# quadram-institute-bioscience/uvaia

Measured on AMD Instinct MI355X. Metric: ref-seqs scored/sec, higher is better.
Workload: dtype u32 bit-planes / int32 counts

## Files before the change

include/uvaia_gpu.h:

```cpp
#ifndef UVAIA_GPU_H
#define UVAIA_GPU_H

#include <stddef.h>
#include <stdint.h>

#ifdef __cplusplus
extern "C" {
#endif

#define UVAIA_GPU_NSCORE 6

enum {
  UVAIA_GPU_OK         =  0,
  UVAIA_GPU_EINVAL     = -1,
  UVAIA_GPU_ENODEV     = -2,
  UVAIA_GPU_ENOMEM     = -3,
  UVAIA_GPU_EHIP       = -4,
  UVAIA_GPU_EALPHABET  = -5,
  UVAIA_GPU_ESTATE     = -6
};

typedef struct uvaia_gpu_ctx uvaia_gpu_ctx;

typedef struct {
  int n_query;
  int nchar;
  const char *const *seq;
  const char *consensus;
  const size_t *idx_c, *idx_m, *idx;
  int n_idx_c, n_idx_m, n_idx;
  size_t trim;
  int acgt;
} uvaia_gpu_query;

int uvaia_gpu_open (uvaia_gpu_ctx **ctx, const uvaia_gpu_query *query, int heap_size, int device, size_t max_pool);

enum { UVAIA_GPU_SCAN_AUTO = 0,
       UVAIA_GPU_SCAN_PACKED = 1,
       UVAIA_GPU_SCAN_COMPRESSED = 2,
       UVAIA_GPU_SCAN_WIDE = 3 };
typedef struct {
  size_t subslice_refs;
  int rare_max;
  int scan;
  int serial;
  int scan_tiles_per_wave;
  int scan_waves_per_block;
  int rederive_streams;
  int ball_gather;
  int query_tables;
  int replay_extras;
  int replay_cus;
  int scan_streams;
  int pipeline;
  int head_scan;
} uvaia_gpu_tuning;
int uvaia_gpu_export_query_table (uvaia_gpu_ctx *ctx, int which, void *out, size_t cap, size_t *n_bytes);
int uvaia_gpu_open_tuned (uvaia_gpu_ctx **ctx, const uvaia_gpu_query *query, int heap_size, int device, size_t max_pool, const uvaia_gpu_tuning *tuning );
void uvaia_gpu_close (uvaia_gpu_ctx *ctx);
const char *uvaia_gpu_last_error (const uvaia_gpu_ctx *ctx);

int uvaia_gpu_push (uvaia_gpu_ctx *ctx, const char *const *seq, const int *non_n, int n_ref, int64_t ordinal0,
                    uint8_t *entered);

int uvaia_gpu_drain (uvaia_gpu_ctx *ctx, int *n_items, int *max_incompatible, int *scores, int64_t *ordinals);
int uvaia_gpu_heap_slots (const uvaia_gpu_ctx *ctx);
int uvaia_gpu_n_query (const uvaia_gpu_ctx *ctx);
int uvaia_gpu_reset (uvaia_gpu_ctx *ctx);

int uvaia_gpu_db_reserve (uvaia_gpu_ctx *ctx, size_t n_ref_capacity);
int uvaia_gpu_db_append (uvaia_gpu_ctx *ctx, const char *const *seq, const int *non_n, int n_ref);
int uvaia_gpu_db_append_block (uvaia_gpu_ctx *ctx, const char *rows, size_t pitch, const int *non_n, int n_ref);
size_t uvaia_gpu_db_size (const uvaia_gpu_ctx *ctx);
int uvaia_gpu_search_resident (uvaia_gpu_ctx *ctx, size_t pool, int64_t ordinal0, uint8_t *entered);
int uvaia_gpu_sync (uvaia_gpu_ctx *ctx);

size_t uvaia_gpu_state_bytes (const uvaia_gpu_ctx *ctx);
int uvaia_gpu_state_export (uvaia_gpu_ctx *ctx, void *dst);
int uvaia_gpu_state_import (uvaia_gpu_ctx *ctx, const void *src);
int uvaia_gpu_slice_scan (uvaia_gpu_ctx *ctx, size_t first, size_t n, int buf);
int uvaia_gpu_slice_replay (uvaia_gpu_ctx *ctx, int buf, int64_t ordinal0, int stripe_start);
int uvaia_gpu_slice_buffers (void);
size_t uvaia_gpu_state_range_bytes (const uvaia_gpu_ctx *ctx, int q0, int q1);
int uvaia_gpu_state_export_range (uvaia_gpu_ctx *ctx, void *dst, int q0, int q1);
int uvaia_gpu_state_import_range (uvaia_gpu_ctx *ctx, const void *src, int q0, int q1);
int uvaia_gpu_slice_replay_range (uvaia_gpu_ctx *ctx, int buf, int64_t ordinal0, int q0, int q1, int take_snapshot);
int uvaia_gpu_entered_flags (uvaia_gpu_ctx *ctx, uint8_t *out, int clear);

int uvaia_gpu_ball (uvaia_gpu_ctx *ctx, const char *const *seq, int n_ref, int radius, int *mindist);
int uvaia_gpu_ball_resident (uvaia_gpu_ctx *ctx, size_t first, size_t n, int radius, int *mindist);
int uvaia_gpu_ball_packed (uvaia_gpu_ctx *ctx, const void *planes, int n_ref, int radius, int *mindist);
int uvaia_gpu_unpack_rows (uvaia_gpu_ctx *ctx, const int *index, int n, char *rows, size_t pitch);
unsigned long long uvaia_gpu_ball_asked (uvaia_gpu_ctx *ctx, int reset);
void uvaia_gpu_ball_kernel_ms (uvaia_gpu_ctx *ctx, double out[3], int reset);

int uvaia_gpu_agree_on_polymorphic (uvaia_gpu_ctx *ctx, const char *const *seq, int n_seq, uint8_t *out);

int uvaia_gpu_query_columns (const char *const *seq, int n_query, int nchar, size_t trim, int acgt, int device, char *consensus, unsigned char *some_missing);

int uvaia_gpu_last_batch_scores (uvaia_gpu_ctx *ctx, int *out, int n_ref);
int uvaia_gpu_scan_stats (uvaia_gpu_ctx *ctx, double *ms, long long *launches, double *algorithmic_bytes, int reset);
int uvaia_gpu_replay_stats (uvaia_gpu_ctx *ctx, unsigned long long out[3], int reset);
int uvaia_gpu_replay_tiles_opened (uvaia_gpu_ctx *ctx, unsigned long long *out, int reset);
int uvaia_gpu_replay_timing (uvaia_gpu_ctx *ctx, unsigned long long out[12], int reset);
int uvaia_gpu_set_query_tile (uvaia_gpu_ctx *ctx, int qt);
int uvaia_gpu_set_active_queries (uvaia_gpu_ctx *ctx, int q0, int q1);
int uvaia_gpu_max_tolerance (uvaia_gpu_ctx *ctx, int *out);
int uvaia_gpu_search_resident_pool (uvaia_gpu_ctx *ctx, size_t first, size_t n, int64_t ordinal0, int snapshot);

int uvaia_gpu_db_set_shard (uvaia_gpu_ctx *ctx, int rank, int world, size_t piece_refs);
int uvaia_gpu_shard_rows (const uvaia_gpu_ctx *ctx);
size_t uvaia_gpu_shard_aux_bytes (const uvaia_gpu_ctx *ctx, size_t n_tiles);
int uvaia_gpu_shard_scan (uvaia_gpu_ctx *ctx, size_t first, size_t n, void *cnt, void *tmin, void *aux);
int uvaia_gpu_db_skip (uvaia_gpu_ctx *ctx, size_t n_ref);
int uvaia_gpu_shard_set_peer (uvaia_gpu_ctx *ctx, int rank, const void *planes, const void *side_rows);
const void *uvaia_gpu_shard_planes (const uvaia_gpu_ctx *ctx);
const void *uvaia_gpu_shard_side_rows (const uvaia_gpu_ctx *ctx);
int uvaia_gpu_shard_ipc_handle_bytes (void);
int uvaia_gpu_shard_ipc_handles (uvaia_gpu_ctx *ctx, void *out );
int uvaia_gpu_shard_ipc_open (uvaia_gpu_ctx *ctx, int rank, const void *handles);
int uvaia_gpu_shard_ipc_close (uvaia_gpu_ctx *ctx);
int uvaia_gpu_scan_wait (uvaia_gpu_ctx *ctx);
int uvaia_gpu_replay_wait (uvaia_gpu_ctx *ctx);
int uvaia_gpu_set_snapshot (uvaia_gpu_ctx *ctx, int snapshot);
enum { UVAIA_GPU_SCANS = 0, UVAIA_GPU_REPLAYS = 1 };
int uvaia_gpu_mark (uvaia_gpu_ctx *ctx, int what, int slot);
int uvaia_gpu_stream_wait_mark (uvaia_gpu_ctx *ctx, void *stream, int slot);
int uvaia_gpu_wait_stream (uvaia_gpu_ctx *ctx, int what, void *stream);
int uvaia_gpu_shard_replay (uvaia_gpu_ctx *ctx, const void *cnt, const void *tmin, const void *aux, int owner, size_t first, size_t n, int64_t ordinal0, int q0, int q1);

typedef struct uvaia_gpu_group uvaia_gpu_group;
int  uvaia_gpu_group_open (uvaia_gpu_group **group, const uvaia_gpu_query *query, int heap_size, const int *devices, int n_devices, size_t max_pool, size_t piece_refs);
void uvaia_gpu_group_close (uvaia_gpu_group *group);
const char *uvaia_gpu_group_last_error (const uvaia_gpu_group *group);
int  uvaia_gpu_group_size (const uvaia_gpu_group *group);
uvaia_gpu_ctx *uvaia_gpu_group_member (uvaia_gpu_group *group, int i);
int  uvaia_gpu_group_query_shard (const uvaia_gpu_group *group, int i, int *q0, int *q1);
int  uvaia_gpu_group_db_reserve (uvaia_gpu_group *group, size_t n_ref_capacity);
int  uvaia_gpu_group_db_append (uvaia_gpu_group *group, const char *const *seq, const int *non_n, int n_ref);
int  uvaia_gpu_group_db_append_packed (uvaia_gpu_group *group, const void *planes, const int *non_n, const int *side_rows, int n_ref);
int  uvaia_gpu_group_db_clear (uvaia_gpu_group *group);
int  uvaia_gpu_group_db_rederive (uvaia_gpu_group *group);
size_t uvaia_gpu_group_db_size (const uvaia_gpu_group *group);
int  uvaia_gpu_group_reset (uvaia_gpu_group *group);
int  uvaia_gpu_group_search_resident (uvaia_gpu_group *group, size_t pool, int64_t ordinal0, uint8_t *entered);
int  uvaia_gpu_group_push (uvaia_gpu_group *group, const char *const *seq, const int *non_n, int n_ref, int64_t ordinal0, uint8_t *entered);
int  uvaia_gpu_group_drain (uvaia_gpu_group *group, int *n_items, int *max_incompatible, int *scores, int64_t *ordinals);
int  uvaia_gpu_group_sync (uvaia_gpu_group *group);

size_t uvaia_gpu_db_tile_bytes (const uvaia_gpu_ctx *ctx);
int    uvaia_gpu_db_clear (uvaia_gpu_ctx *ctx);
int    uvaia_gpu_db_rederive (uvaia_gpu_ctx *ctx);
int    uvaia_gpu_db_side_row_ints (void);
int    uvaia_gpu_db_export (uvaia_gpu_ctx *ctx, size_t first_tile, size_t n_tiles, void *planes, int *non_n, int *side_rows);
int    uvaia_gpu_db_append_packed (uvaia_gpu_ctx *ctx, const void *planes, const int *non_n, const int *side_rows, int n_ref);

int uvaia_gpu_db_stage_reserve (uvaia_gpu_ctx *ctx, size_t n_tiles);
int uvaia_gpu_db_stage_packed (uvaia_gpu_ctx *ctx, int slot, const void *planes, const int *non_n, const int *side_rows, int n_tiles);
int uvaia_gpu_db_load_staged (uvaia_gpu_ctx *ctx, int slot, const int *sel, int n_ref);
int uvaia_gpu_db_stage_packed_at (uvaia_gpu_ctx *ctx, int slot, size_t tile_offset, const void *planes, const int *non_n, const int *side_rows, int n_tiles);
int uvaia_gpu_db_append_staged (uvaia_gpu_ctx *ctx, int slot, const int *sel, int n_ref);
int uvaia_gpu_db_unpack_rows (uvaia_gpu_ctx *ctx, const int *index, int n, char *rows, size_t pitch);
void uvaia_gpu_window_ms (uvaia_gpu_ctx *ctx, double out[3], int reset);
size_t uvaia_gpu_free_bytes (uvaia_gpu_ctx *ctx);

int uvaia_gpu_rows_census (uvaia_gpu_ctx *ctx, const void *d_rows, size_t pitch, int n, int *non_n, int *n_exc);
int uvaia_gpu_db_append_device (uvaia_gpu_ctx *ctx, const void *d_rows, size_t pitch, const int *row_index, int n_sel, const int *non_n);
int uvaia_gpu_rows_exceptions (uvaia_gpu_ctx *ctx, const void *d_rows, size_t pitch, const int *row_index, int n_sel, const uint64_t *offsets, void *exc_out);
int uvaia_gpu_db_drop_tiles (uvaia_gpu_ctx *ctx, size_t n_tiles);
void uvaia_gpu_rows_kernel_ms (uvaia_gpu_ctx *ctx, double out[3], int reset);
int uvaia_gpu_rows_set_run_cut (uvaia_gpu_ctx *ctx, unsigned cut);

size_t uvaia_gpu_scan_bytes_per_ref (const uvaia_gpu_ctx *ctx);
int uvaia_gpu_scan_variant (const uvaia_gpu_ctx *ctx);
size_t uvaia_gpu_derived_bytes_per_ref (const uvaia_gpu_ctx *ctx);
size_t uvaia_gpu_packed_bytes_per_ref (const uvaia_gpu_ctx *ctx);

#ifdef __cplusplus
}
#endif
#endif
```

uvaia_amd/capi.py:

```python
import ctypes as C
import os
import subprocess

import numpy as np

_HERE = os.path.dirname(os.path.abspath(__file__))
ROOT = os.path.dirname(_HERE)
_LIB = os.path.join(_HERE, "lib", "libuvaia_gpu.so")
NSCORE = 6

SYMBOLS = [
    "uvaia_gpu_open", "uvaia_gpu_open_tuned", "uvaia_gpu_close", "uvaia_gpu_last_error", "uvaia_gpu_push", "uvaia_gpu_drain",
    "uvaia_gpu_heap_slots", "uvaia_gpu_n_query", "uvaia_gpu_reset", "uvaia_gpu_db_reserve", "uvaia_gpu_db_append",
    "uvaia_gpu_db_append_block", "uvaia_gpu_db_size", "uvaia_gpu_search_resident", "uvaia_gpu_sync", "uvaia_gpu_ball", "uvaia_gpu_ball_resident", "uvaia_gpu_ball_packed", "uvaia_gpu_unpack_rows", "uvaia_gpu_ball_asked", "uvaia_gpu_ball_kernel_ms", "uvaia_gpu_export_query_table", "uvaia_gpu_agree_on_polymorphic", "uvaia_gpu_query_columns",
    "uvaia_gpu_last_batch_scores", "uvaia_gpu_scan_stats", "uvaia_gpu_replay_stats", "uvaia_gpu_replay_tiles_opened", "uvaia_gpu_replay_timing",
    "uvaia_gpu_state_bytes", "uvaia_gpu_state_export", "uvaia_gpu_state_import", "uvaia_gpu_slice_scan", "uvaia_gpu_slice_replay",
    "uvaia_gpu_entered_flags", "uvaia_gpu_state_range_bytes", "uvaia_gpu_state_export_range", "uvaia_gpu_state_import_range",
    "uvaia_gpu_slice_replay_range", "uvaia_gpu_slice_buffers", "uvaia_gpu_scan_bytes_per_ref", "uvaia_gpu_derived_bytes_per_ref", "uvaia_gpu_scan_variant", "uvaia_gpu_set_query_tile", "uvaia_gpu_packed_bytes_per_ref",
    "uvaia_gpu_db_tile_bytes", "uvaia_gpu_db_side_row_ints", "uvaia_gpu_db_export", "uvaia_gpu_db_append_packed", "uvaia_gpu_db_clear", "uvaia_gpu_db_rederive",
    "uvaia_gpu_set_active_queries", "uvaia_gpu_max_tolerance", "uvaia_gpu_search_resident_pool",
    "uvaia_gpu_db_set_shard", "uvaia_gpu_shard_rows", "uvaia_gpu_shard_scan", "uvaia_gpu_scan_wait", "uvaia_gpu_replay_wait", "uvaia_gpu_set_snapshot", "uvaia_gpu_shard_replay",
    "uvaia_gpu_mark", "uvaia_gpu_stream_wait_mark", "uvaia_gpu_wait_stream",
    "uvaia_gpu_shard_aux_bytes", "uvaia_gpu_db_skip", "uvaia_gpu_shard_set_peer", "uvaia_gpu_shard_planes", "uvaia_gpu_shard_side_rows",
    "uvaia_gpu_shard_ipc_handle_bytes", "uvaia_gpu_shard_ipc_handles", "uvaia_gpu_shard_ipc_open", "uvaia_gpu_shard_ipc_close",
    "uvaia_gpu_group_open", "uvaia_gpu_group_close", "uvaia_gpu_group_last_error", "uvaia_gpu_group_size", "uvaia_gpu_group_member", "uvaia_gpu_group_query_shard",
    "uvaia_gpu_group_db_reserve", "uvaia_gpu_group_db_append", "uvaia_gpu_group_db_append_packed", "uvaia_gpu_group_db_clear", "uvaia_gpu_group_db_rederive",
    "uvaia_gpu_group_db_size", "uvaia_gpu_group_reset", "uvaia_gpu_group_search_resident", "uvaia_gpu_group_push", "uvaia_gpu_group_drain", "uvaia_gpu_group_sync",
    "uvaia_gpu_rows_census", "uvaia_gpu_db_append_device", "uvaia_gpu_rows_exceptions", "uvaia_gpu_db_drop_tiles", "uvaia_gpu_rows_kernel_ms", "uvaia_gpu_rows_set_run_cut",
    "uvaia_gpu_db_stage_reserve", "uvaia_gpu_db_stage_packed", "uvaia_gpu_db_load_staged", "uvaia_gpu_db_unpack_rows", "uvaia_gpu_window_ms", "uvaia_gpu_free_bytes",
    "uvaia_gpu_db_stage_packed_at", "uvaia_gpu_db_append_staged",
]


class GpuError(RuntimeError):
    def __init__(self, code, msg):
        super().__init__("uvaia_gpu error %d: %s" % (code, msg))
        self.code = code


class Tuning(C.Structure):
    _fields_ = [("subslice_refs", C.c_size_t), ("rare_max", C.c_int), ("scan", C.c_int), ("serial", C.c_int),
                ("scan_tiles_per_wave", C.c_int), ("scan_waves_per_block", C.c_int), ("rederive_streams", C.c_int), ("ball_gather", C.c_int), ("query_tables", C.c_int), ("replay_extras", C.c_int), ("replay_cus", C.c_int), ("scan_streams", C.c_int), ("pipeline", C.c_int), ("head_scan", C.c_int)]

    SCAN = {"auto": 0, "packed": 1, "compressed": 2, "wide": 3}

    @classmethod
    def make(cls, tuning):
        if tuning is None or isinstance(tuning, cls):
            return tuning
        t = cls()
        for k, v in tuning.items():
            setattr(t, k, cls.SCAN[v] if k == "scan" and isinstance(v, str) else int(v))
        return t


class _Query(C.Structure):
    _fields_ = [
        ("n_query", C.c_int), ("nchar", C.c_int),
        ("seq", C.POINTER(C.c_char_p)), ("consensus", C.c_char_p),
        ("idx_c", C.POINTER(C.c_size_t)), ("idx_m", C.POINTER(C.c_size_t)), ("idx", C.POINTER(C.c_size_t)),
        ("n_idx_c", C.c_int), ("n_idx_m", C.c_int), ("n_idx", C.c_int),
        ("trim", C.c_size_t), ("acgt", C.c_int),
    ]


def library_path():
    return _LIB


def build_library(force=False):
    csrc = os.path.join(_HERE, "csrc")
    srcs = [os.path.join(csrc, f) for f in os.listdir(csrc) if f.endswith((".hip", ".inc"))] + [os.path.join(ROOT, "include", "uvaia_gpu.h")]
    if not force and os.path.exists(_LIB) and os.path.getmtime(_LIB) >= max(os.path.getmtime(f) for f in srcs):
        return _LIB
    subprocess.check_call(["make", "-C", os.path.join(_HERE, "csrc"), "-s"])
    return _LIB


_lib = None


def load_library():
    global _lib
    if _lib is not None:
        return _lib
    if not os.path.exists(_LIB):
        raise GpuError(-2, "HIP library %s is missing: run __graft_entry__.build() (no CPU fallback exists)" % _LIB)
    L = C.CDLL(_LIB)
    vp = C.c_void_p
    pp = C.POINTER(C.c_char_p)
    pi = C.POINTER(C.c_int)
    sig = {
        "uvaia_gpu_open": (C.c_int, [C.POINTER(vp), C.POINTER(_Query), C.c_int, C.c_int, C.c_size_t]),
        "uvaia_gpu_open_tuned": (C.c_int, [C.POINTER(vp), C.POINTER(_Query), C.c_int, C.c_int, C.c_size_t, C.POINTER(Tuning)]),
        "uvaia_gpu_close": (None, [vp]),
        "uvaia_gpu_last_error": (C.c_char_p, [vp]),
        "uvaia_gpu_push": (C.c_int, [vp, pp, pi, C.c_int, C.c_int64, C.POINTER(C.c_uint8)]),
        "uvaia_gpu_drain": (C.c_int, [vp, pi, pi, pi, C.POINTER(C.c_int64)]),
        "uvaia_gpu_heap_slots": (C.c_int, [vp]),
        "uvaia_gpu_n_query": (C.c_int, [vp]),
        "uvaia_gpu_reset": (C.c_int, [vp]),
        "uvaia_gpu_db_reserve": (C.c_int, [vp, C.c_size_t]),
        "uvaia_gpu_db_append": (C.c_int, [vp, pp, pi, C.c_int]),
        "uvaia_gpu_db_append_block": (C.c_int, [vp, C.c_void_p, C.c_size_t, pi, C.c_int]),
        "uvaia_gpu_db_size": (C.c_size_t, [vp]),
        "uvaia_gpu_search_resident": (C.c_int, [vp, C.c_size_t, C.c_int64, C.POINTER(C.c_uint8)]),
        "uvaia_gpu_sync": (C.c_int, [vp]),
        "uvaia_gpu_ball": (C.c_int, [vp, pp, C.c_int, C.c_int, pi]),
        "uvaia_gpu_ball_resident": (C.c_int, [vp, C.c_size_t, C.c_size_t, C.c_int, pi]),
        "uvaia_gpu_ball_packed": (C.c_int, [vp, C.c_void_p, C.c_int, C.c_int, pi]),
        "uvaia_gpu_unpack_rows": (C.c_int, [vp, pi, C.c_int, C.c_void_p, C.c_size_t]),
        "uvaia_gpu_ball_asked": (C.c_ulonglong, [vp, C.c_int]),
        "uvaia_gpu_ball_kernel_ms": (None, [vp, C.POINTER(C.c_double), C.c_int]),
        "uvaia_gpu_export_query_table": (C.c_int, [vp, C.c_int, vp, C.c_size_t, C.POINTER(C.c_size_t)]),
        "uvaia_gpu_agree_on_polymorphic": (C.c_int, [vp, pp, C.c_int, C.POINTER(C.c_uint8)]),
        "uvaia_gpu_query_columns": (C.c_int, [pp, C.c_int, C.c_int, C.c_size_t, C.c_int, C.c_int, C.c_char_p, C.POINTER(C.c_uint8)]),
        "uvaia_gpu_last_batch_scores": (C.c_int, [vp, pi, C.c_int]),
        "uvaia_gpu_scan_stats": (C.c_int, [vp, C.POINTER(C.c_double), C.POINTER(C.c_longlong), C.POINTER(C.c_double), C.c_int]),
        "uvaia_gpu_replay_stats": (C.c_int, [vp, C.POINTER(C.c_ulonglong), C.c_int]),
        "uvaia_gpu_replay_tiles_opened": (C.c_int, [vp, C.POINTER(C.c_ulonglong), C.c_int]),
        "uvaia_gpu_replay_timing": (C.c_int, [vp, C.POINTER(C.c_ulonglong), C.c_int]),
        "uvaia_gpu_state_bytes": (C.c_size_t, [vp]),
        "uvaia_gpu_state_export": (C.c_int, [vp, C.c_void_p]),
        "uvaia_gpu_state_import": (C.c_int, [vp, C.c_void_p]),
        "uvaia_gpu_slice_scan": (C.c_int, [vp, C.c_size_t, C.c_size_t, C.c_int]),
        "uvaia_gpu_slice_replay": (C.c_int, [vp, C.c_int, C.c_int64, C.c_int]),
        "uvaia_gpu_entered_flags": (C.c_int, [vp, C.POINTER(C.c_uint8), C.c_int]),
        "uvaia_gpu_state_range_bytes": (C.c_size_t, [vp, C.c_int, C.c_int]),
        "uvaia_gpu_state_export_range": (C.c_int, [vp, C.c_void_p, C.c_int, C.c_int]),
        "uvaia_gpu_state_import_range": (C.c_int, [vp, C.c_void_p, C.c_int, C.c_int]),
        "uvaia_gpu_slice_replay_range": (C.c_int, [vp, C.c_int, C.c_int64, C.c_int, C.c_int, C.c_int]),
        "uvaia_gpu_slice_buffers": (C.c_int, []),
        "uvaia_gpu_scan_bytes_per_ref": (C.c_size_t, [vp]),
        "uvaia_gpu_derived_bytes_per_ref": (C.c_size_t, [vp]),
        "uvaia_gpu_scan_variant": (C.c_int, [vp]),
        "uvaia_gpu_set_query_tile": (C.c_int, [vp, C.c_int]),
        "uvaia_gpu_packed_bytes_per_ref": (C.c_size_t, [vp]),
        "uvaia_gpu_set_active_queries": (C.c_int, [vp, C.c_int, C.c_int]),
        "uvaia_gpu_max_tolerance": (C.c_int, [vp, pi]),
        "uvaia_gpu_search_resident_pool": (C.c_int, [vp, C.c_size_t, C.c_size_t, C.c_int64, C.c_int]),
        "uvaia_gpu_db_tile_bytes": (C.c_size_t, [vp]),
        "uvaia_gpu_db_clear": (C.c_int, [vp]),
        "uvaia_gpu_db_rederive": (C.c_int, [vp]),
        "uvaia_gpu_db_side_row_ints": (C.c_int, []),
        "uvaia_gpu_db_export": (C.c_int, [vp, C.c_size_t, C.c_size_t, C.c_void_p, pi, pi]),
        "uvaia_gpu_db_append_packed": (C.c_int, [vp, C.c_void_p, pi, pi, C.c_int]),
        "uvaia_gpu_db_set_shard": (C.c_int, [vp, C.c_int, C.c_int, C.c_size_t]),
        "uvaia_gpu_shard_rows": (C.c_int, [vp]),
        "uvaia_gpu_shard_scan": (C.c_int, [vp, C.c_size_t, C.c_size_t, C.c_void_p, C.c_void_p, C.c_void_p]),
        "uvaia_gpu_shard_aux_bytes": (C.c_size_t, [vp, C.c_size_t]), "uvaia_gpu_db_skip": (C.c_int, [vp, C.c_size_t]),
        "uvaia_gpu_shard_set_peer": (C.c_int, [vp, C.c_int, C.c_void_p, C.c_void_p]),
        "uvaia_gpu_shard_planes": (C.c_void_p, [vp]), "uvaia_gpu_shard_side_rows": (C.c_void_p, [vp]),
        "uvaia_gpu_shard_ipc_handle_bytes": (C.c_int, []), "uvaia_gpu_shard_ipc_handles": (C.c_int, [vp, C.c_void_p]),
        "uvaia_gpu_shard_ipc_open": (C.c_int, [vp, C.c_int, C.c_void_p]), "uvaia_gpu_shard_ipc_close": (C.c_int, [vp]),
        "uvaia_gpu_scan_wait": (C.c_int, [vp]),
        "uvaia_gpu_replay_wait": (C.c_int, [vp]),
        "uvaia_gpu_set_snapshot": (C.c_int, [vp, C.c_int]),
        "uvaia_gpu_shard_replay": (C.c_int, [vp, C.c_void_p, C.c_void_p, C.c_void_p, C.c_int, C.c_size_t, C.c_size_t, C.c_int64, C.c_int, C.c_int]),
        "uvaia_gpu_mark": (C.c_int, [vp, C.c_int, C.c_int]), "uvaia_gpu_stream_wait_mark": (C.c_int, [vp, C.c_void_p, C.c_int]),
        "uvaia_gpu_wait_stream": (C.c_int, [vp, C.c_int, C.c_void_p]),
        "uvaia_gpu_group_open": (C.c_int, [C.POINTER(vp), C.POINTER(_Query), C.c_int, pi, C.c_int, C.c_size_t, C.c_size_t]),
        "uvaia_gpu_group_close": (None, [vp]),
        "uvaia_gpu_group_last_error": (C.c_char_p, [vp]),
        "uvaia_gpu_group_size": (C.c_int, [vp]),
        "uvaia_gpu_group_member": (vp, [vp, C.c_int]),
        "uvaia_gpu_group_query_shard": (C.c_int, [vp, C.c_int, pi, pi]),
        "uvaia_gpu_group_db_reserve": (C.c_int, [vp, C.c_size_t]),
        "uvaia_gpu_group_db_append": (C.c_int, [vp, pp, pi, C.c_int]),
        "uvaia_gpu_group_db_append_packed": (C.c_int, [vp, C.c_void_p, pi, pi, C.c_int]),
        "uvaia_gpu_group_db_clear": (C.c_int, [vp]),
        "uvaia_gpu_group_db_rederive": (C.c_int, [vp]),
        "uvaia_gpu_group_db_size": (C.c_size_t, [vp]),
        "uvaia_gpu_group_reset": (C.c_int, [vp]),
        "uvaia_gpu_group_search_resident": (C.c_int, [vp, C.c_size_t, C.c_int64, C.POINTER(C.c_uint8)]),
        "uvaia_gpu_group_push": (C.c_int, [vp, pp, pi, C.c_int, C.c_int64, C.POINTER(C.c_uint8)]),
        "uvaia_gpu_group_drain": (C.c_int, [vp, pi, pi, pi, C.POINTER(C.c_int64)]),
        "uvaia_gpu_group_sync": (C.c_int, [vp]),
        "uvaia_gpu_rows_census": (C.c_int, [vp, C.c_void_p, C.c_size_t, C.c_int, pi, pi]),
        "uvaia_gpu_db_append_device": (C.c_int, [vp, C.c_void_p, C.c_size_t, pi, C.c_int, pi]),
        "uvaia_gpu_rows_exceptions": (C.c_int, [vp, C.c_void_p, C.c_size_t, pi, C.c_int, C.POINTER(C.c_uint64), C.c_void_p]),
        "uvaia_gpu_db_drop_tiles": (C.c_int, [vp, C.c_size_t]),
        "uvaia_gpu_rows_kernel_ms": (None, [vp, C.POINTER(C.c_double), C.c_int]),
        "uvaia_gpu_rows_set_run_cut": (C.c_int, [vp, C.c_uint]),
        "uvaia_gpu_db_stage_reserve": (C.c_int, [vp, C.c_size_t]),
        "uvaia_gpu_db_stage_packed": (C.c_int, [vp, C.c_int, C.c_void_p, pi, pi, C.c_int]),
        "uvaia_gpu_db_load_staged": (C.c_int, [vp, C.c_int, pi, C.c_int]),
        "uvaia_gpu_db_stage_packed_at": (C.c_int, [vp, C.c_int, C.c_size_t, C.c_void_p, pi, pi, C.c_int]),
        "uvaia_gpu_db_append_staged": (C.c_int, [vp, C.c_int, pi, C.c_int]),
        "uvaia_gpu_db_unpack_rows": (C.c_int, [vp, pi, C.c_int, C.c_void_p, C.c_size_t]),
        "uvaia_gpu_window_ms": (None, [vp, C.POINTER(C.c_double), C.c_int]),
        "uvaia_gpu_free_bytes": (C.c_size_t, [vp]),
    }
    for name, (res, args) in sig.items():
        fn = getattr(L, name)
        fn.restype, fn.argtypes = res, args
    _lib = L
    return L


def _cstrs(strs):
    arr = (C.c_char_p * len(strs))()
    for i, s in enumerate(strs):
        arr[i] = s
    return arr


def _int_ptr(a):
    if a is None:
        return None, None
    arr = np.ascontiguousarray(a, dtype=np.int32)
    return arr, arr.ctypes.data_as(C.POINTER(C.c_int))


class Engine:

    def __init__(self, seqs, consensus, idx_c, idx_m, idx, trim=0, acgt=False, nbest=100, max_pool=4096, device=-1, tuning=None):
        self.L = load_library()
        self.nq, self.nchar = len(seqs), len(consensus)
        self._keep = [_cstrs(seqs), consensus,
                      (C.c_size_t * len(idx_c))(*[int(x) for x in idx_c]),
                      (C.c_size_t * len(idx_m))(*[int(x) for x in idx_m]),
                      (C.c_size_t * len(idx))(*[int(x) for x in idx])]
        q = _Query(self.nq, self.nchar, self._keep[0], consensus, self._keep[2], self._keep[3], self._keep[4],
                   len(idx_c), len(idx_m), len(idx), int(trim), int(bool(acgt)))
        self.ctx = C.c_void_p()
        tn = Tuning.make(tuning)
        rc = self.L.uvaia_gpu_open_tuned(C.byref(self.ctx), C.byref(q), int(nbest), int(device), int(max_pool), C.byref(tn) if tn is not None else None)
        if rc != 0:
            msg = self.L.uvaia_gpu_last_error(None)
            self.ctx = None
            raise GpuError(rc, msg.decode() if msg else "?")
        self.slots = self.L.uvaia_gpu_heap_slots(self.ctx)
        self.ordinal = 0

    @classmethod
    def from_query(cls, q, **kw):
        return cls(q.seqs, q.consensus, q.idx_c, q.idx_m, q.idx, trim=q.trim, acgt=q.acgt, **kw)

    def _chk(self, rc):
        if rc != 0:
            msg = self.L.uvaia_gpu_last_error(self.ctx)
            raise GpuError(rc, msg.decode() if msg else "?")

    def close(self):
        if getattr(self, "ctx", None):
            self.L.uvaia_gpu_close(self.ctx)
            self.ctx = None

    def __del__(self):
        try:
            self.close()
        except Exception:
            pass

    def __enter__(self):
        return self

    def __exit__(self, *a):
        self.close()

    def push(self, refs, non_n=None, ordinal0=None):
        n = len(refs)
        if ordinal0 is None:
            ordinal0 = self.ordinal
        self.ordinal = ordinal0 + n
        entered = np.zeros(n, dtype=np.uint8)
        if n == 0:
            return entered
        _k, nn = _int_ptr(non_n)
        self._chk(self.L.uvaia_gpu_push(self.ctx, _cstrs(refs), nn, n, ordinal0, entered.ctypes.data_as(C.POINTER(C.c_uint8))))
        return entered

    def last_batch_scores(self, n):
        out = np.zeros((n, self.nq, NSCORE), dtype=np.int32)
        self._chk(self.L.uvaia_gpu_last_batch_scores(self.ctx, out.ctypes.data_as(C.POINTER(C.c_int)), n))
        return out

    def drain(self):
        n = np.zeros(self.nq, dtype=np.int32)
        T = np.zeros(self.nq, dtype=np.int32)
        sc = np.zeros((self.nq, self.slots + 1, NSCORE), dtype=np.int32)
        od = np.zeros((self.nq, self.slots + 1), dtype=np.int64)
        pi = C.POINTER(C.c_int)
        self._chk(self.L.uvaia_gpu_drain(self.ctx, n.ctypes.data_as(pi), T.ctypes.data_as(pi), sc.ctypes.data_as(pi),
                                         od.ctypes.data_as(C.POINTER(C.c_int64))))
        return n, T, sc, od

    def reset(self):
        self.ordinal = 0
        self._chk(self.L.uvaia_gpu_reset(self.ctx))

    def db_reserve(self, n):
        self._chk(self.L.uvaia_gpu_db_reserve(self.ctx, int(n)))

    def db_append(self, refs, non_n=None):
        _k, nn = _int_ptr(non_n)
        self._chk(self.L.uvaia_gpu_db_append(self.ctx, _cstrs(refs), nn, len(refs)))

    def db_append_block(self, block, non_n=None):
        block = np.ascontiguousarray(block, dtype=np.uint8)
        _k, nn = _int_ptr(non_n)
        self._chk(self.L.uvaia_gpu_db_append_block(self.ctx, block.ctypes.data, block.shape[1], nn, block.shape[0]))

    def db_size(self):
        return self.L.uvaia_gpu_db_size(self.ctx)

    @staticmethod
    def _device_block(rows, pitch=None, n=None):
        if hasattr(rows, "data_ptr"):
            import torch
            if rows.dtype != torch.uint8 or rows.dim() != 2 or not rows.is_cuda or (rows.shape[0] > 0 and rows.shape[1] > 1 and rows.stride(1) != 1):
                raise GpuError(-1, "rows must be a 2-d torch.uint8 tensor in device memory with contiguous rows")
            torch.cuda.current_stream(rows.device).synchronize()
            return rows.data_ptr(), (rows.stride(0) if rows.shape[0] > 1 else rows.shape[1]), rows.shape[0], rows
        if pitch is None:
            raise GpuError(-1, "a raw device pointer needs its pitch")
        return int(rows), int(pitch), n, None

    def rows_census(self, rows, pitch=None, n=None):
        ptr, pitch, n, _keep = self._device_block(rows, pitch, n)
        non_n, n_exc = np.zeros(n, dtype=np.int32), np.zeros(n, dtype=np.int32)
        self._chk(self.L.uvaia_gpu_rows_census(self.ctx, ptr, pitch, n, non_n.ctypes.data_as(C.POINTER(C.c_int)), n_exc.ctypes.data_as(C.POINTER(C.c_int))))
        return non_n, n_exc

    def db_append_device(self, rows, row_index=None, non_n=None, pitch=None, n=None):
        ptr, pitch, n, _keep = self._device_block(rows, pitch, n)
        _k1, ri = _int_ptr(row_index)
        _k2, nn = _int_ptr(non_n)
        self._chk(self.L.uvaia_gpu_db_append_device(self.ctx, ptr, pitch, ri, n if row_index is None else len(row_index), nn))

    def rows_exceptions(self, rows, n_exc, row_index=None, pitch=None, n=None):
        ptr, pitch, n, _keep = self._device_block(rows, pitch, n)
        n_sel = n if row_index is None else len(row_index)
        off = np.zeros(n_sel + 1, dtype=np.uint64)
        off[1:] = np.cumsum(np.asarray(n_exc, dtype=np.uint64))
        out = np.zeros((int(off[-1]), 2), dtype=np.uint32)
        _k1, ri = _int_ptr(row_index)
        self._chk(self.L.uvaia_gpu_rows_exceptions(self.ctx, ptr, pitch, ri, n_sel, off.ctypes.data_as(C.POINTER(C.c_uint64)), out.ctypes.data))
        return off, out

    def db_drop_tiles(self, n_tiles):
        self._chk(self.L.uvaia_gpu_db_drop_tiles(self.ctx, int(n_tiles)))

    def rows_kernel_ms(self, reset=False):
        out = (C.c_double * 3)()
# ... 386 lines not shown
```

uvaia_amd/csrc/host_launch.inc:

```

namespace {

template <class F>
static void parallel_for(int n, F f)
{
  const unsigned nt = std::min<unsigned>(std::max(1u, std::thread::hardware_concurrency()), 64u);
  if (n < 32 || nt < 2) { for (int i = 0; i < n; i++) f(i); return; }
  std::atomic<int> next(0);
  std::vector<std::thread> th;
  for (unsigned t = 0; t < nt; t++) th.emplace_back([&]() { for (;;) { const int a = next.fetch_add(4); if (a >= n) break; for (int i = a; i < std::min(n, a + 4); i++) f(i); } });
  for (auto &x : th) x.join();
}

__global__ void mask_query_planes_kernel(const uint32_t *__restrict__ qp, const uint32_t *__restrict__ pmask, uint32_t *__restrict__ out, size_t n_words_total, int words_per_row, int nq_planes)
{
  const size_t i = (size_t)blockIdx.x * blockDim.x + threadIdx.x;
  if (i >= n_words_total) return;
  const int w = (int)((i / (size_t)nq_planes) % (size_t)words_per_row);
  out[i] = qp[i] & pmask[w];
}

int ensure_qpoly(uvaia_gpu_ctx *c)
{
  if (c->d_qpoly) return 0;
  HIPCHK(c, hipSetDevice(c->device));
  const size_t n = (size_t)c->nq_pad * c->W4 * 4 * c->NQ;
  uint32_t *d = nullptr;
  HIPCHK(c, hipMalloc(&d, n * 4));
  hipLaunchKernelGGL(mask_query_planes_kernel, dim3((unsigned)((n + 255) / 256)), dim3(256), 0, c->stream, c->d_qp, c->d_pmask, d, n, c->W4 * 4, c->NQ);
  hipError_t e = hipGetLastError();
  if (e == hipSuccess) e = hipStreamSynchronize(c->stream);
  if (e != hipSuccess) { hipFree(d); return fail(c, UVAIA_GPU_EHIP, "query planes on the polymorphic columns: %s", hipGetErrorString(e)); }
  c->d_qpoly = d;
  return 0;
}

int ensure_qgather(uvaia_gpu_ctx *c)
{
  if (c->d_qg) return 0;
  HIPCHK(c, hipSetDevice(c->device));
  const int NG = c->acgt ? 3 : 5, W = c->W4 * 4, n_idx = c->n_idx;
  constexpr int BALL_HOT_COLS = 256;
  std::vector<int> cols(c->idx_cols.begin(), c->idx_cols.begin() + n_idx), order;
  std::vector<uint32_t> masks((size_t)2 * W, 0u);
  int n_hot = 0;
  if (n_idx >= 2 * BALL_HOT_COLS) {
    int *d_score = nullptr;
    std::vector<int> score((size_t)n_idx);
    HIPCHK(c, hipMalloc(&d_score, (size_t)n_idx * sizeof(int)));
    if (c->acgt) hipLaunchKernelGGL((ball_column_diversity_kernel<true>), dim3((n_idx + 63) / 64), dim3(64), 0, c->stream, c->d_qp, c->nq, c->W4, c->d_idx_cols, n_idx, d_score);
    else         hipLaunchKernelGGL((ball_column_diversity_kernel<false>), dim3((n_idx + 63) / 64), dim3(64), 0, c->stream, c->d_qp, c->nq, c->W4, c->d_idx_cols, n_idx, d_score);
    hipError_t e = hipGetLastError();
    if (e == hipSuccess) e = hipMemcpyAsync(score.data(), d_score, (size_t)n_idx * sizeof(int), hipMemcpyDeviceToHost, c->stream);
    if (e == hipSuccess) e = hipStreamSynchronize(c->stream);
    hipFree(d_score);
    if (e != hipSuccess) return fail(c, UVAIA_GPU_EHIP, "diversity of the polymorphic columns: %s", hipGetErrorString(e));
    std::vector<int> by_score((size_t)n_idx);
    for (int i = 0; i < n_idx; i++) by_score[(size_t)i] = i;
    std::stable_sort(by_score.begin(), by_score.end(), [&](int a, int b) { return score[(size_t)a] > score[(size_t)b]; });
    n_hot = BALL_HOT_COLS;
    std::vector<uint8_t> is_hot((size_t)n_idx, 0);
    for (int i = 0; i < n_hot; i++) is_hot[(size_t)by_score[(size_t)i]] = 1;
    for (int i = 0; i < n_idx; i++) if (is_hot[(size_t)i]) order.push_back(cols[(size_t)i]);
    for (int i = 0; i < n_idx; i++) if (!is_hot[(size_t)i]) order.push_back(cols[(size_t)i]);
  } else order = cols;
  c->NH4 = n_hot / 128;
  c->NG4 = std::max(1, c->NH4 + (n_idx - n_hot + 127) / 128);
  for (int i = 0; i < n_idx; i++) { const int col = order[(size_t)i]; masks[(size_t)(col >> 7) * 8 + (i < n_hot ? 0 : 4) + ((col >> 5) & 3)] |= 1u << (col & 31); }
  order.resize(order.size() + 1, 0);
  uint32_t *d = nullptr, *dm = nullptr; int *dc = nullptr;
  const size_t n = (size_t)c->nq_pad * c->NG4 * 4 * NG;
  hipError_t e = hipMalloc(&d, n * 4);
  if (e == hipSuccess) e = hipMalloc(&dm, masks.size() * 4);
  if (e == hipSuccess) e = hipMalloc(&dc, order.size() * sizeof(int));
  if (e == hipSuccess) e = hipMemcpyAsync(dm, masks.data(), masks.size() * 4, hipMemcpyHostToDevice, c->stream);
  if (e == hipSuccess) e = hipMemcpyAsync(dc, order.data(), order.size() * sizeof(int), hipMemcpyHostToDevice, c->stream);
  if (e == hipSuccess) e = hipMemsetAsync(d, 0, n * 4, c->stream);
  dim3 grid((unsigned)((c->NG4 * 4 + 63) / 64), (unsigned)c->nq);
  if (e == hipSuccess) {
    if (c->acgt) hipLaunchKernelGGL((ball_gather_queries_kernel<true>), grid, dim3(64), 0, c->stream, c->d_qp, c->nq, c->W4, dc, n_idx, c->NG4, d);
    else         hipLaunchKernelGGL((ball_gather_queries_kernel<false>), grid, dim3(64), 0, c->stream, c->d_qp, c->nq, c->W4, dc, n_idx, c->NG4, d);
    e = hipGetLastError();
  }
  if (e == hipSuccess) e = hipStreamSynchronize(c->stream);
  hipFree(dc);
  if (e != hipSuccess) { hipFree(d); hipFree(dm); return fail(c, UVAIA_GPU_EHIP, "query planes on the polymorphic columns: %s", hipGetErrorString(e)); }
  c->d_qg = d; c->d_ball_masks = dm;
  return 0;
}

void store_free(TileStore &s)
{
  for (void *p : {(void *)s.planes, (void *)s.nonn, (void *)s.amb, (void *)s.tot, (void *)s.ev, (void *)s.poly, (void *)s.grp, (void *)s.tote}) hipFree(p);
  s = TileStore();
}
void slice_free(SliceBuf &b)
{
  for (void *p : {(void *)b.cnt, (void *)b.tmin, (void *)b.ext, (void *)b.rtp, (void *)b.tb8, (void *)b.rt, (void *)b.progress}) hipFree(p);
  for (hipEvent_t e : {b.scan_done, b.scan_started, b.replay_done}) if (e) hipEventDestroy(e);
  b = SliceBuf();
}

int store_alloc(uvaia_gpu_ctx *c, TileStore &s, size_t tiles)
{
  store_free(s);
  uint4 *planes = nullptr;
  const size_t refs = tiles * 64, tile_u4 = (size_t)c->W4 * c->P * 64;
  HIPCHK(c, hipMalloc(&s.nonn, refs * sizeof(int)));
  HIPCHK(c, hipMemset(s.nonn, 0, refs * sizeof(int)));
  HIPCHK(c, hipMalloc(&s.ev, tiles * (size_t)c->W4 * 2 * 64 * sizeof(uint4)));
  HIPCHK(c, hipMalloc(&s.grp, tiles * (size_t)c->W4 * 64 * sizeof(uint32_t)));
  HIPCHK(c, hipMalloc(&s.poly, tiles * (size_t)std::max(c->NP4 + c->NR4, 1) * 3 * 64 * sizeof(uint4)));
  HIPCHK(c, hipMalloc(&s.tote, refs * sizeof(int)));
  HIPCHK(c, hipMalloc(&s.tot, refs * sizeof(int)));
  HIPCHK(c, hipMemset(s.tot, 0, refs * sizeof(int)));
  HIPCHK(c, hipMalloc(&s.amb, refs * AMB_ROW * sizeof(int)));
  HIPCHK(c, hipMemset(s.amb, 0, refs * AMB_ROW * sizeof(int)));
  HIPCHK(c, hipMalloc(&planes, tiles * tile_u4 * sizeof(uint4)));
  HIPCHK(c, hipMemset(planes, 0, tiles * tile_u4 * sizeof(uint4)));
  s.planes = planes;
  return 0;
}

int ensure_batch_buffers(uvaia_gpu_ctx *c)
{
  if (c->batch.planes) return 0;
  HIPCHK(c, hipSetDevice(c->device));
  return store_alloc(c, c->batch, c->pool_pad / 64);
}

int pack_query_row(const uint8_t *code_tab, const char *row, int nchar, int lo, int hi, const uint8_t *keep, const uint8_t *is_poly,
                   bool acgt, int NQ, uint32_t *dst, int *bad_byte)
{
  for (int s = lo; s < hi; s++) {
    if (keep && !keep[s]) continue;
    const uint8_t code = code_tab[(unsigned char)row[s]];
    if (code == 0xFF) { *bad_byte = (unsigned char)row[s]; return -1; }
    if (!code) continue;
    const int w = s >> 5, b = s & 31;
    uint32_t *d = dst + (size_t)w * NQ;
    const bool one = (code & (code - 1)) == 0;
    if (acgt) {
      if (!one) continue;
      const uint32_t two = code == 2 ? 1u : code == 4 ? 2u : code == 8 ? 3u : 0u;
      d[0] |= (two & 1u) << b; d[1] |= (two >> 1) << b; d[2] |= 1u << b;
      if (is_poly && is_poly[s]) d[3] |= 1u << b;
    } else {
      for (int p = 0; p < 4; p++) d[p] |= (uint32_t)((code >> p) & 1u) << b;
      d[4] |= 1u << b;
      if (one) d[5] |= 1u << b;
    }
  }
  return 0;
}

int take_scan_events(uvaia_gpu_ctx *c, ScanEvt &ev)
{
  for (hipEvent_t *e : {&ev.a, &ev.b}) {
    if (!c->ev_pool.empty()) { *e = c->ev_pool.back(); c->ev_pool.pop_back(); }
    else HIPCHK(c, hipEventCreate(e));
  }
  return 0;
}

int launch_scan(uvaia_gpu_ctx *c, const TileStore &s, long long tile_first, int n_tiles, const uint32_t *qp, int n_rows, int4 *out, int ppad, double bytes)
{
  if (n_tiles <= 0) return 0;
  dim3 grid((unsigned)((n_rows + c->qt - 1) / c->qt), (unsigned)((n_tiles + 3) / 4)), block(256);
  ScanEvt ev{};
  if (c->profile) {
    { int rc_ = take_scan_events(c, ev); if (rc_) return rc_; }
    HIPCHK(c, hipEventRecord(ev.a, c->stream));
  }
#define LAUNCH(K, QT) hipLaunchKernelGGL((K<QT>), grid, block, 0, c->stream, s.planes, tile_first, n_tiles, c->W4, qp, out, ppad)
  if (c->acgt) { switch (c->qt) { case 8: LAUNCH(scan_acgt_kernel, 8); break; case 32: LAUNCH(scan_acgt_kernel, 32); break; default: LAUNCH(scan_acgt_kernel, 16); } }
  else         { switch (c->qt) { case 8: LAUNCH(scan_iupac_kernel, 8); break; case 32: LAUNCH(scan_iupac_kernel, 32); break; default: LAUNCH(scan_iupac_kernel, 16); } }
#undef LAUNCH
  HIPCHK(c, hipGetLastError());
  if (c->profile) { HIPCHK(c, hipEventRecord(ev.b, c->stream)); ev.bytes = bytes; c->evts.push_back(ev); }
  return 0;
}

int launch_pair_extras(uvaia_gpu_ctx *c, const TileStore &s, long long tile_first, int n_tiles, uint32_t *ext, int ppad, hipStream_t stream)
{
  if (n_tiles <= 0) return 0;
  hipLaunchKernelGGL(pair_extras_kernel, dim3((unsigned)n_tiles, (unsigned)((c->nq + 15) / 16)), dim3(256), 0, stream, s.planes, tile_first, n_tiles, c->W4,
                     s.amb, c->d_qp, c->d_amb_q, c->nq, ext, ppad);
  HIPCHK(c, hipGetLastError());
  return 0;
}

int launch_scan2(uvaia_gpu_ctx *c, const TileStore &s, long long tile_first, int n_tiles, uint32_t *out, int ppad, double bytes, hipStream_t stream,
                 int2 *tmin, int r_lo, int r_hi, int4 *rt, uint32_t *ext = nullptr , uint32_t *rtp = nullptr, uint4 *tb8 = nullptr,
                 unsigned *progress = nullptr )
{
  if (n_tiles <= 0) return 0;
  if (!stream) stream = c->stream;
  const bool cons = c->n_idx_c > 0;
  if (cons && !rt) return fail(c, UVAIA_GPU_ESTATE, "no buffer for the consensus pre-score");
  const uint4 *tiles = s.planes; const int *tot_tile0 = s.tot + tile_first * 64;
  const long long ptile_first = tile_first;
  auto consensus_rt = [&]() {
    if (!cons) return;
    if (c->acgt) hipLaunchKernelGGL((consensus_rt_kernel<true>), dim3((n_tiles + 3) / 4), dim3(256), 0, stream, tiles, ptile_first, n_tiles, c->W4, c->d_cp, rt);
    else         hipLaunchKernelGGL((consensus_rt_kernel<false>), dim3((n_tiles + 3) / 4), dim3(256), 0, stream, tiles, ptile_first, n_tiles, c->W4, c->d_cp, rt);
  };
  const int qt2 = c->qt != 8 ? 16 : c->nq <= 1 ? 1 : c->nq <= 2 ? 2 : c->nq <= 4 ? 4 : 8;
  const int n_qtiles = (c->nq + qt2 - 1) / qt2;
  dim3 grid(scan_grid_size(n_qtiles, n_tiles)), block(256);
  ScanEvt ev_{};
  if (c->profile) {
    { int rc_ = take_scan_events(c, ev_); if (rc_) return rc_; }
    HIPCHK(c, hipEventRecord(ev_.a, stream));
  }
  const uint32_t *qp = c->acgt ? c->d_qp : c->d_qp2;
  if (c->scan_variant == 2) {
    const int *tote = s.tote + tile_first * 64;
    constexpr int QS = 64;
    if (c->act_q0 % QS) return fail(c, UVAIA_GPU_ESTATE, "the scan works on super-tiles of %d queries: active queries start at a multiple of that", QS);
    const int st_first = c->act_q0 / QS, n_st = (c->act_q1 + QS - 1) / QS - st_first;
    const int R = c->scan_R;
    dim3 grid3(scan_grid_size(n_st, (n_tiles + R - 1) / R));
#define SCAN3_LAUNCH(NWW, A, RR) hipLaunchKernelGGL((scan3_kernel<NWW, A, RR>), grid3, dim3(64 * NWW), 0, stream, s.ev, s.poly, tile_first, n_tiles, c->W4, c->NP4, c->NP4 + c->NR4, c->d_qpl, c->d_stream, c->d_sdir, s.grp, tote, tot_tile0, out, ppad, n_st, tmin, r_lo, r_hi, st_first, progress)
#define SCAN3_NW(A, RR) { if (c->scan_NW == 8) SCAN3_LAUNCH(8, A, RR); else SCAN3_LAUNCH(4, A, RR); }
    if (progress) { consensus_rt(); HIPCHK(c, hipGetLastError()); }
    if (R == 4)      { if (c->acgt) SCAN3_LAUNCH(8, true, 4); else SCAN3_LAUNCH(8, false, 4); }
    else if (R == 2) { if (c->acgt) SCAN3_NW(true, 2) else SCAN3_NW(false, 2) }
    else             { if (c->acgt) SCAN3_NW(true, 1) else SCAN3_NW(false, 1) }
#undef SCAN3_NW
#undef SCAN3_LAUNCH
    HIPCHK(c, hipGetLastError());
    if (c->profile) { HIPCHK(c, hipEventRecord(ev_.b, stream)); ev_.bytes = bytes; c->evts.push_back(ev_); }
    if (!progress) consensus_rt();
    HIPCHK(c, hipGetLastError());
    if (tb8 && !c->acgt) {
      hipLaunchKernelGGL(tile_bounds_kernel, dim3((unsigned)n_tiles), dim3(256), 0, stream, out, ppad, n_tiles, c->nq, r_lo, r_hi, tb8, cons ? rt : (const int4 *)nullptr, rtp);
      HIPCHK(c, hipGetLastError());
      if (ext) { int rc_ = launch_pair_extras(c, s, ptile_first, n_tiles, ext, ppad, stream); if (rc_) return rc_; }
    }
    return 0;
  }
  const int *amb0 = s.amb;
#define LAUNCH(K, QT, CN) hipLaunchKernelGGL((K<QT, CN>), grid, block, 0, stream, tiles, tile_first, n_tiles, c->W4, qp, out, ppad, n_qtiles, tot_tile0, tmin, r_lo, r_hi, c->d_cp, rt)
#define LAUNCHX(K, QT, CN) hipLaunchKernelGGL((K<QT, CN>), grid, block, 0, stream, tiles, tile_first, n_tiles, c->W4, qp, out, ppad, n_qtiles, tot_tile0, tmin, r_lo, r_hi, c->d_cp, rt, ext, rtp, tb8, amb0, c->d_qp, c->d_amb_q, c->nq)
#define LAUNCH_QT(L, K, CN) switch (qt2) { case 1: L(K, 1, CN); break; case 2: L(K, 2, CN); break; case 4: L(K, 4, CN); break; case 8: L(K, 8, CN); break; default: L(K, 16, CN); }
  if (c->acgt) { if (cons) { LAUNCH_QT(LAUNCH, scan2_acgt_kernel, true) } else { LAUNCH_QT(LAUNCH, scan2_acgt_kernel, false) } }
  else         { if (cons) { LAUNCH_QT(LAUNCHX, scan2_iupac_kernel, true) } else { LAUNCH_QT(LAUNCHX, scan2_iupac_kernel, false) } }
#undef LAUNCH_QT
#undef LAUNCHX
#undef LAUNCH
  HIPCHK(c, hipGetLastError());
  if (c->profile) { HIPCHK(c, hipEventRecord(ev_.b, stream)); ev_.bytes = bytes; c->evts.push_back(ev_); }
  return 0;
}

size_t replay3_lds_bytes(const uvaia_gpu_ctx *c)
{ return (size_t)(c->k + 1) * HEAP_ENTRY * sizeof(int) + 128 + (size_t)16 * 1024 + (size_t)2 * c->replay_half * (c->n_idx_c > 0 ? 4 : 3) * 256; }
int ensure_cnt4(uvaia_gpu_ctx *c, size_t elems)
{
  if (c->cnt_cap >= elems) return 0;
  if (c->d_cnt) { HIPCHK(c, hipFree(c->d_cnt)); c->d_cnt = nullptr; c->cnt_cap = 0; }
  HIPCHK(c, hipMalloc(&c->d_cnt, elems * sizeof(int4)));
  c->cnt_cap = elems;
  return 0;
}

int collect_events(uvaia_gpu_ctx *c)
{
  for (auto &e : c->evts) {
    HIPCHK(c, hipEventSynchronize(e.b));
    float ms = 0; HIPCHK(c, hipEventElapsedTime(&ms, e.a, e.b));
    c->scan_ms += ms; c->scan_bytes += e.bytes; c->scan_launches++;
    c->ev_pool.push_back(e.a); c->ev_pool.push_back(e.b);
  }
  c->evts.clear();
  return 0;
}

struct ReplayLaunch {
  hipStream_t stream; int q0, q1;
  const uint32_t *cnt, *ext; int ppad; const int4 *rt; const uint32_t *rtp; const int2 *tmin; const uint4 *tb8;
  const uint4 *planes; long long tile_first; const int *nonn, *amb; uint8_t *entered;
  int rb, re; long long ord_base;
  const uint32_t *qpl; const uint4 *poly; int nr4; const uint32_t *qrare;
  int prefetch;
  const unsigned *progress; unsigned blocks_per_group; int scan_R; int *pipe_err;
};
int launch_replay(uvaia_gpu_ctx *c, const ReplayLaunch &L)
{
  const dim3 grid(L.q1 - L.q0), block(64);
  const size_t lds = (size_t)(c->k + 1) * HEAP_ENTRY * sizeof(int);
  if (c->fullscan) {
#define REPLAY(A) hipLaunchKernelGGL((replay_kernel<A>), grid, block, lds, L.stream, c->d_cnt, L.ppad, c->d_rt, c->d_tr, L.nonn, L.rb, L.re, L.ord_base, c->d_heap, c->d_n, c->d_T, c->d_snap, L.entered, c->k)
    if (c->acgt) REPLAY(true); else REPLAY(false);
#undef REPLAY
  } else if (L.ext) {
#define REPLAY3(B, H) hipLaunchKernelGGL((replay3_kernel<B, H>), grid, block, replay3_lds_bytes(c), L.stream, L.cnt, L.ext, L.ppad, L.rt, L.rtp, c->d_cp, L.nonn, L.amb, L.rb, L.re, L.ord_base, \
                                         c->d_heap, c->d_n, c->d_T, c->d_snap, L.entered, c->k, L.planes, L.tile_first, c->W4, c->d_qp, c->d_amb_q, c->d_stats, L.q0, L.tb8, c->replay_prio)
#define REPLAY3_HALF(B) { if (c->replay_half == 32) REPLAY3(B, 32); else if (c->replay_half == 16) REPLAY3(B, 16); else REPLAY3(B, 8); }
    if (c->n_idx_c > 0) REPLAY3_HALF(true) else REPLAY3_HALF(false)
#undef REPLAY3_HALF
#undef REPLAY3
  } else {
    const int lq_words = (c->replay_lq && !c->acgt && lds + (size_t)c->W4 * 4 * 6 * 4 + 128 <= 64 * 1024) ? c->W4 * 4 * 6 : 0;
    const int2 *tmin = (c->scan_variant == 2 || c->scan_variant == 0) ? L.tmin : nullptr;
#define REPLAY2(A, B, PF_) hipLaunchKernelGGL((replay2_kernel<A, B, PF_>), grid, block, lds + (size_t)lq_words * 4 + 128, L.stream, L.cnt, L.ppad, L.rt, c->d_cp, L.nonn, L.amb, L.rb, L.re, L.ord_base, \
                                              c->d_heap, c->d_n, c->d_T, c->d_snap, L.entered, c->k, L.planes, L.tile_first, c->W4, c->d_qp, c->d_amb_q, c->d_stats, L.q0, tmin, L.qpl, lq_words, c->replay_prio, \
                                              L.poly, c->NP4 + c->NR4, c->NP4, L.nr4, L.qrare, L.progress, L.blocks_per_group, L.scan_R, L.pipe_err)
#define REPLAY2_PF(A, B) { if (L.prefetch == 1) REPLAY2(A, B, 1); else if (L.prefetch == 2) REPLAY2(A, B, 2); else REPLAY2(A, B, 3); }
    if (c->acgt) { if (c->n_idx_c > 0) REPLAY2_PF(true, true) else REPLAY2_PF(true, false) }
    else         { if (c->n_idx_c > 0) REPLAY2_PF(false, true) else REPLAY2_PF(false, false) }
#undef REPLAY2_PF
#undef REPLAY2
  }
  HIPCHK(c, hipGetLastError());
  return 0;
}

int run_batch(uvaia_gpu_ctx *c, const TileStore &s, long long tile_first, int n_tiles, int r_begin, int r_end,
              long long ord_base, size_t cnt4_cols = 0 )
{
  if (r_end <= r_begin) return 0;
  const int ppad = n_tiles * 64;
  const SliceBuf &b = c->slice[0];
  hipLaunchKernelGGL(snapshot_kernel, dim3(1), dim3(256), 0, c->stream, c->d_T, c->nq, c->d_snap);
  if (c->n_idx_c > 0 && c->fullscan) {
    if (c->acgt) hipLaunchKernelGGL((consensus_kernel<true>), dim3((n_tiles + 3) / 4), dim3(256), 0, c->stream, s.planes, tile_first, n_tiles, c->W4, c->d_cp, c->d_snap, c->d_rt, c->d_tr);
    else         hipLaunchKernelGGL((consensus_kernel<false>), dim3((n_tiles + 3) / 4), dim3(256), 0, c->stream, s.planes, tile_first, n_tiles, c->W4, c->d_cp, c->d_snap, c->d_rt, c->d_tr);
  }
  HIPCHK(c, hipGetLastError());
  const double bytes = (double)(r_end - r_begin) * (double)c->W4 * 16.0 * c->P + (double)c->nq * (double)c->W4 * 16.0 * c->P;
  uint32_t *ext = c->use_ext ? b.ext : nullptr;
  int rc = 0;
  if (c->fullscan) {
    rc = ensure_cnt4(c, (size_t)c->nq_pad * (cnt4_cols ? std::max<size_t>(cnt4_cols, (size_t)ppad) : c->pool_pad)); if (rc) return rc;
    rc = launch_scan(c, s, tile_first, n_tiles, c->d_qp, c->nq, c->d_cnt, ppad, bytes);
  } else rc = launch_scan2(c, s, tile_first, n_tiles, b.cnt, ppad, bytes, nullptr, b.tmin, r_begin, r_end, b.rt, ext, b.rtp, b.tb8);
  if (rc) return rc;
  rc = launch_replay(c, {c->stream, 0, c->nq, b.cnt, ext, ppad, b.rt, b.rtp, b.tmin, b.tb8,
                             s.planes, tile_first, s.nonn + tile_first * 64, s.amb + tile_first * 64 * AMB_ROW, c->d_entered + tile_first * 64, r_begin, r_end, ord_base,
                             c->scan_variant == 2 ? c->d_qpl : nullptr, s.poly, c->NR4, c->d_qrare, 3, nullptr, 0, 2, nullptr});
  if (rc) return rc;
  c->last = {&s, tile_first, n_tiles, r_end - r_begin, r_begin, ppad, c->fullscan ? c->d_rt : b.rt};
  return 0;
}

int derive_rows(uvaia_gpu_ctx *c, const TileStore &s, long long slot0, int n_ref, hipStream_t st = nullptr, bool v_in_place = false)
{
  if (!st) st = c->stream;
  if (c->fullscan || c->scan_variant != 2 || n_ref <= 0 || !c->d_split) return 0;
  const long long a = slot0 / 64, t1 = (slot0 + n_ref - 1) / 64;
  const int nblk = (int)(t1 - a + 1);
#define DERIVE_ALL(A, V) hipLaunchKernelGGL((derive_all_kernel<A, V>), dim3(nblk), dim3(256), 0, st, s.planes, a, a, c->W4, c->d_cls, c->d_rmask, c->d_split, c->NP4, c->NR4, s.ev, s.tote, s.grp, s.poly)
  if (c->acgt) { if (v_in_place) DERIVE_ALL(true, false); else DERIVE_ALL(true, true); }
  else         { if (v_in_place) DERIVE_ALL(false, false); else DERIVE_ALL(false, true); }
#undef DERIVE_ALL
  HIPCHK(c, hipGetLastError());
  return 0;
}

int sync_scan_streams(uvaia_gpu_ctx *c) { for (hipStream_t st : c->scan_streams) if (st) HIPCHK(c, hipStreamSynchronize(st)); return 0; }
int sync_derive_streams(uvaia_gpu_ctx *c) { for (hipStream_t st : c->derive_streams) if (st) HIPCHK(c, hipStreamSynchronize(st)); return 0; }

template <class T> int regrow(uvaia_gpu_ctx *c, T *&p, size_t n) { if (p) hipFree(p); p = nullptr; HIPCHK(c, hipMalloc(&p, n * sizeof(T))); return 0; }

int slice_reserve(uvaia_gpu_ctx *c, SliceBuf &b, size_t need, size_t ppad)
{
  need = std::max(need, b.cap);
  if (need <= b.cap && b.tmin) return 0;
  if (int rc = sync_scan_streams(c)) return rc;
  HIPCHK(c, hipStreamSynchronize(c->stream));
  const size_t cap = std::max(need, (size_t)c->nq_pad * c->pool_pad), refs = std::max(cap / (size_t)c->nq_pad, ppad) + 64;
  if (cap > b.cap || !b.cnt) { if (int rc = regrow(c, b.cnt, cap)) return rc; }
  if (int rc = regrow(c, b.tmin, cap / 64)) return rc;
  if (c->use_ext) {
    if (int rc = regrow(c, b.ext, cap)) return rc;
    if (int rc = regrow(c, b.tb8, cap / 64)) return rc;
    if (int rc = regrow(c, b.rtp, refs)) return rc;
  }
  if (int rc = regrow(c, b.rt, refs)) return rc;
  b.cap = cap;
  return 0;
}

static int settle_derive(uvaia_gpu_ctx *c)
{
  if (c->derive_pending) { if (int rc = sync_derive_streams(c)) return rc; c->derive_pending = 0; }
  return 0;
}

int pack_rows(uvaia_gpu_ctx *c, const char *const *seq, const char *rows, size_t rows_pitch, const int *non_n, int n_ref, const TileStore &s, long long slot0)
{
  for (int done = 0, k = 0; done < n_ref; done += PACK_CHUNK, k ^= 1) {
    const int m = std::min(PACK_CHUNK, n_ref - done);
    if (c->stage_busy[k]) { HIPCHK(c, hipEventSynchronize(c->stage_free[k])); c->stage_busy[k] = false; }
    uint8_t *hs = c->h_stage + (size_t)k * PACK_CHUNK * c->pitch, *ds = c->d_stage + (size_t)k * PACK_CHUNK * c->pitch;
    for (int i = 0; i < m; i++) if (!(seq ? seq[done + i] : rows)) return fail(c, UVAIA_GPU_EINVAL, "NULL sequence at position %d", done + i);
    parallel_for(m, [&](int i) {
      const char *src = seq ? seq[done + i] : rows + (size_t)(done + i) * rows_pitch;
      memcpy(hs + (size_t)i * c->pitch, src, (size_t)c->nchar);
    });
    HIPCHK(c, hipMemcpyAsync(ds, hs, (size_t)m * c->pitch, hipMemcpyHostToDevice, c->stream));
    const long long s0 = slot0 + done, t0 = s0 / 64, t1 = (s0 + m - 1) / 64;
    const int nblk = (int)(t1 - t0 + 1);
    int *nn_out = non_n ? nullptr : s.nonn;
    if (c->acgt) hipLaunchKernelGGL((pack_refs_kernel<3>), dim3(nblk), dim3(256), 0, c->stream, ds, c->pitch, c->nchar, s0, m, c->W4, s.planes, t0, nn_out, (int *)nullptr, s.tot, c->d_err);
    else         hipLaunchKernelGGL((pack_refs_kernel<4>), dim3(nblk), dim3(256), 0, c->stream, ds, c->pitch, c->nchar, s0, m, c->W4, s.planes, t0, nn_out, s.amb, s.tot, c->d_err);
    HIPCHK(c, hipGetLastError());
    if (non_n) HIPCHK(c, hipMemcpyAsync(s.nonn + s0, non_n + done, (size_t)m * sizeof(int), hipMemcpyHostToDevice, c->stream));
    HIPCHK(c, hipEventRecord(c->stage_free[k], c->stream)); c->stage_busy[k] = true;
  }
  { int rc = derive_rows(c, s, slot0, n_ref); if (rc) return rc; }
  HIPCHK(c, hipStreamSynchronize(c->stream));
  int bad = 0;
  HIPCHK(c, hipMemcpy(&bad, c->d_err, sizeof(int), hipMemcpyDeviceToHost));
  if (bad) {
    HIPCHK(c, hipMemset(c->d_err, 0, sizeof(int)));
    return fail(c, UVAIA_GPU_EALPHABET, "a reference sequence holds a byte outside ACGT / MRWSYKVHDB / NX-?O.");
  }
  return 0;
}

}
```

uvaia_amd/csrc/host_open.inc:

```

extern "C" {

const char *uvaia_gpu_last_error(const uvaia_gpu_ctx *ctx) { return ctx ? ctx->err.c_str() : g_open_error.c_str(); }

void uvaia_gpu_close(uvaia_gpu_ctx *c)
{
  if (!c) return;
  if (c->stream) hipStreamSynchronize(c->stream);
  for (auto &e : c->evts) { hipEventDestroy(e.a); hipEventDestroy(e.b); }
  for (hipEvent_t e : c->ev_pool) hipEventDestroy(e);
  for (hipEvent_t e : c->rows_evs) hipEventDestroy(e);
  void *dev[] = {c->d_idx_cols, c->d_qg, c->d_ball_masks, c->d_ball_key, c->d_split, c->d_qrare, c->d_rmask, c->d_cls, c->d_qpl, c->d_stream, c->d_sdir, c->d_mindist, c->d_ball_list, c->d_ball_cdist, c->d_ball_n, c->d_ball_tiles, c->d_ball_ga,
                 c->d_qp2, c->d_amb_q, c->d_stats, c->d_qp, c->d_cp, c->d_cpm, c->d_qpoly, c->d_pmask, c->d_heap, c->d_n, c->d_T, c->d_snap, c->d_err, c->d_cnt, c->d_rt, c->d_tr, c->d_entered, c->d_stage, c->d_pipe_err, c->d_pk, c->d_rows, c->d_row_idx, c->d_rsel, c->d_rcnt, c->d_roff, c->d_rexc, c->d_wsel, c->d_win4};
  for (void *p : dev) if (p) hipFree(p);
  store_free(c->batch); store_free(c->db);
  for (SliceBuf &b : c->slice) slice_free(b);
  if (c->h_stage) hipHostFree(c->h_stage);
  for (int i = 0; i < 2; i++) if (c->stage_free[i]) hipEventDestroy(c->stage_free[i]);
  for (int i = 0; i < 16; i++) if (c->order_ev[i]) hipEventDestroy(c->order_ev[i]);
  for (int i = 0; i < 4; i++) if (c->ball_ev[i]) hipEventDestroy(c->ball_ev[i]);
  if (c->copy_stream) { hipStreamSynchronize(c->copy_stream); hipStreamDestroy(c->copy_stream); }
  for (auto &sl : c->wstage) { for (void *p : {(void *)sl.planes, (void *)sl.nonn, (void *)sl.side}) if (p) hipFree(p); for (hipEvent_t e : {sl.copied, sl.read}) if (e) hipEventDestroy(e); }
  for (int i = 0; i < 5; i++) if (c->win_ev[i]) hipEventDestroy(c->win_ev[i]);
  for (int i = 0; i < 64; i++) for (int j = 0; j < 2; j++) if (c->ipc_opened[i][j]) hipIpcCloseMemHandle(c->ipc_opened[i][j]);
  for (int i = 0; i < 8; i++) for (int j = 0; j < 3; j++) if (c->mark_ev[i][j]) hipEventDestroy(c->mark_ev[i][j]);
  for (int i_ = 0; i_ < 3; i_++) if (c->derive_streams[i_]) { hipStreamSynchronize(c->derive_streams[i_]); hipStreamDestroy(c->derive_streams[i_]); }
  for (auto &d : c->derive_chunks) hipEventDestroy(d.done);
  for (int i = 0; i < 4; i++) if (c->derive_fence[i]) hipEventDestroy(c->derive_fence[i]);
  if (c->scan_stream) hipStreamDestroy(c->scan_stream);
  for (int i = 1; i < 3; i++) if (c->scan_streams[i]) hipStreamDestroy(c->scan_streams[i]);
  if (c->stream) hipStreamDestroy(c->stream);
  if (c->rep_stream) { hipStreamSynchronize(c->rep_stream); hipStreamDestroy(c->rep_stream); }
  for (int i = 0; i < 2; i++) if (c->rep_ev[i]) hipEventDestroy(c->rep_ev[i]);
  delete c;
}

int uvaia_gpu_open(uvaia_gpu_ctx **out, const uvaia_gpu_query *q, int heap_size, int device, size_t max_pool)
{ return uvaia_gpu_open_tuned(out, q, heap_size, device, max_pool, nullptr); }

int uvaia_gpu_open_tuned(uvaia_gpu_ctx **out, const uvaia_gpu_query *q, int heap_size, int device, size_t max_pool, const uvaia_gpu_tuning *tune)
{
  uvaia_gpu_tuning tn;
  memset(&tn, 0, sizeof tn);
  if (tune) tn = *tune;
  if (tn.scan < 0 || tn.scan > UVAIA_GPU_SCAN_WIDE || tn.query_tables < 0 || tn.query_tables > 2 || (tn.scan_tiles_per_wave != 0 && tn.scan_tiles_per_wave != 1 && tn.scan_tiles_per_wave != 2 && tn.scan_tiles_per_wave != 4) ||
      (tn.scan_waves_per_block != 0 && tn.scan_waves_per_block != 4 && tn.scan_waves_per_block != 8) || (tn.subslice_refs != 0 && tn.subslice_refs < 64))
    return fail(nullptr, UVAIA_GPU_EINVAL, "bad tuning values");
  if (!out) return fail(nullptr, UVAIA_GPU_EINVAL, "ctx is NULL");
  *out = nullptr;
  if (!q || q->n_query < 1 || q->nchar < 1 || !q->seq || !q->consensus) return fail(nullptr, UVAIA_GPU_EINVAL, "empty or incomplete query set");
  if ((q->n_idx_c && !q->idx_c) || (q->n_idx_m && !q->idx_m) || (q->n_idx && !q->idx)) return fail(nullptr, UVAIA_GPU_EINVAL, "index arrays missing");
  if (max_pool < 1) return fail(nullptr, UVAIA_GPU_EINVAL, "max_pool must be >= 1");
  int ndev = 0;
  if (hipGetDeviceCount(&ndev) != hipSuccess || ndev < 1) return fail(nullptr, UVAIA_GPU_ENODEV, "no HIP device available: the MI355X engine has no CPU fallback");
  if (device < 0) { if (hipGetDevice(&device) != hipSuccess) device = 0; }
  if (device >= ndev) return fail(nullptr, UVAIA_GPU_ENODEV, "device %d out of range (%d devices)", device, ndev);
  if (hipSetDevice(device) != hipSuccess) return fail(nullptr, UVAIA_GPU_ENODEV, "hipSetDevice(%d) failed", device);

  uvaia_gpu_ctx *c = new uvaia_gpu_ctx();
  c->device = device;
  c->nq = q->n_query; c->act_q0 = 0; c->act_q1 = q->n_query; c->nchar = q->nchar; c->acgt = q->acgt ? 1 : 0; c->trim = q->trim; c->n_idx_c = q->n_idx_c; c->n_idx_m = q->n_idx_m;
  c->P = c->acgt ? 3 : 4; c->NQ = c->acgt ? 4 : 6;
  c->W = (c->nchar + 31) / 32; c->W4 = (c->W + 3) / 4;
  c->k = heap_size < 2 ? 2 : heap_size;
  c->qt = c->nq <= 8 ? 8 : 16;
  c->scan_variant = tn.scan == UVAIA_GPU_SCAN_PACKED ? 0 : tn.scan == UVAIA_GPU_SCAN_COMPRESSED ? 2 : (c->nq <= 32 ? 0 : 2);
  c->fullscan = tn.scan == UVAIA_GPU_SCAN_WIDE;
  c->serial = tn.serial != 0;
  if (tn.scan_tiles_per_wave) c->scan_R = tn.scan_tiles_per_wave;
  if (tn.scan_waves_per_block) c->scan_NW = tn.scan_waves_per_block;
  if (c->scan_R == 4 && c->scan_NW != 8) { delete c; return fail(nullptr, UVAIA_GPU_EINVAL, "four reference tiles per wave go with eight waves per block"); }
  if (tn.subslice_refs) { c->subslice = tn.subslice_refs; c->subslice_forced = true; }
  if (tn.scan_streams >= 1 && tn.scan_streams <= 3) c->scan_nstreams_forced = tn.scan_streams;
  if (tn.scan_streams > 100 && tn.scan_streams < 200) c->first_slice_pct = tn.scan_streams == 199 ? 0 : tn.scan_streams - 100;
  if (tn.pipeline == 2) c->pipeline = true;
  if (tn.head_scan == 2) c->head_full = true;
  if (tn.ball_gather == 1 || tn.ball_gather == 2) c->ball_fused = tn.ball_gather == 2;
  if (tn.rederive_streams >= 1 && tn.rederive_streams <= 3) { c->derive_nstreams = tn.rederive_streams; c->derive_forced = true; }
  if (c->nchar > 49000) c->fullscan = true;
  c->nq_pad = ((c->nq + 127) / 128) * 128;
  c->max_pool = max_pool; c->pool_pad = ((max_pool + 63) / 64) * 64 + 64;
  c->pitch = ((size_t)c->nchar + 63) / 64 * 64;
  if ((size_t)(c->k + 1) * HEAP_ENTRY * sizeof(int) + 128 > 160 * 1024) { delete c; return fail(nullptr, UVAIA_GPU_EINVAL, "nbest=%d does not fit the per-query LDS heap (max 5115)", heap_size); }

#define OPENCHK(call) HIP_TRY(call, { const int rc_ = fail(nullptr, code_, "%s failed: %s", #call, hipGetErrorString(e_)); uvaia_gpu_close(c); return rc_; })
  c->use_ext = !c->fullscan && !c->acgt && tn.replay_extras != 1 && (c->scan_variant == 0 || (c->scan_variant == 2 && c->nq <= 128 && tn.replay_extras == 2));
  {
    int prio_least = 0, prio_greatest = 0;
    OPENCHK(hipDeviceGetStreamPriorityRange(&prio_least, &prio_greatest));
    bool split = false;
    const int want_half = tn.replay_cus >= 1000 ? tn.replay_cus / 1000 : 0, want_cus = tn.replay_cus >= 1000 ? tn.replay_cus % 1000 : tn.replay_cus;
    c->replay_half = (want_half == 32 || want_half == 16 || want_half == 8) ? want_half : c->nq <= 8 ? 32 : c->nq <= 24 ? 16 : 8;
    int per_cu = (int)std::min<size_t>(4, (size_t)160 * 1024 / replay3_lds_bytes(c));
    while (c->use_ext && c->replay_half > 8 && per_cu * 8 < std::min(c->nq, 32)) { c->replay_half /= 2; per_cu = (int)std::min<size_t>(4, (size_t)160 * 1024 / replay3_lds_bytes(c)); }
    if (c->use_ext && replay3_lds_bytes(c) > (size_t)160 * 1024) c->use_ext = false;
    const int rep_cus = want_cus < 0 ? 0 : want_cus > 0 ? want_cus : (c->use_ext && per_cu > 0 ? std::max(8, ((c->nq + per_cu - 1) / per_cu + 7) / 8 * 8) : 0);
    hipDeviceProp_t prop;
    if (rep_cus > 0 && hipGetDeviceProperties(&prop, device) == hipSuccess && prop.multiProcessorCount >= 4 * rep_cus) {
      const int ncu = prop.multiProcessorCount, words = (ncu + 31) / 32;
      std::vector<uint32_t> m_rep((size_t)words, 0u), m_scan((size_t)words, 0u);
      for (int b = 0; b < ncu; b++) (b < rep_cus ? m_rep : m_scan)[(size_t)b >> 5] |= 1u << (b & 31);
      hipStream_t st[7] = {};
      bool ok = hipExtStreamCreateWithCUMask(&st[0], (uint32_t)words, m_rep.data()) == hipSuccess;
      for (int i = 1; i < 7 && ok; i++) ok = hipExtStreamCreateWithCUMask(&st[i], (uint32_t)words, m_scan.data()) == hipSuccess;
      if (ok) ok = hipEventCreateWithFlags(&c->rep_ev[0], hipEventDisableTiming) == hipSuccess && hipEventCreateWithFlags(&c->rep_ev[1], hipEventDisableTiming) == hipSuccess;
      if (ok) {
        c->rep_stream = st[0]; c->scan_stream = st[1]; c->scan_streams[0] = st[1]; c->scan_streams[1] = st[2]; c->scan_streams[2] = st[3];
        for (int i = 0; i < 3; i++) c->derive_streams[i] = st[4 + i];
        split = true; c->replay_cus = rep_cus;
      } else { (void)hipGetLastError(); for (int i = 0; i < 7; i++) if (st[i]) hipStreamDestroy(st[i]); }
    }
    OPENCHK(hipStreamCreateWithPriority(&c->stream, hipStreamNonBlocking, prio_greatest));
    if (!split) {
      OPENCHK(hipStreamCreateWithPriority(&c->scan_stream, hipStreamNonBlocking, prio_least));
      c->scan_streams[0] = c->scan_stream;
      for (int i = 1; i < 3; i++) OPENCHK(hipStreamCreateWithPriority(&c->scan_streams[i], hipStreamNonBlocking, prio_least));
      for (int i = 0; i < 3; i++) OPENCHK(hipStreamCreateWithPriority(&c->derive_streams[i], hipStreamNonBlocking, (prio_least + prio_greatest) / 2));
    }
    for (SliceBuf &b : c->slice) { OPENCHK(hipEventCreateWithFlags(&b.scan_done, hipEventDisableTiming)); OPENCHK(hipEventCreateWithFlags(&b.replay_done, hipEventDisableTiming)); }
    c->derive_stream = c->derive_streams[0];
  }
  uint8_t code_tab[256]; fill_code_table(code_tab);
  OPENCHK(hipMemcpyToSymbol(HIP_SYMBOL(c_code), code_tab, 256));

  const int lo = (int)std::min<size_t>(c->trim, (size_t)c->nchar), hi = std::max(lo, c->nchar - (int)c->trim);
  const size_t row_words = (size_t)c->W4 * 4 * c->NQ;
  std::vector<uint8_t> in_c(c->nchar, 0), in_m(c->nchar, 0), in_p(c->nchar, 0);
  for (int i = 0; i < q->n_idx_c; i++) if (q->idx_c[i] < (size_t)c->nchar) in_c[q->idx_c[i]] = 1;
  for (int i = 0; i < q->n_idx_m; i++) if (q->idx_m[i] < (size_t)c->nchar) in_m[q->idx_m[i]] = 1;
  for (int i = 0; i < q->n_idx; i++)   if (q->idx[i]   < (size_t)c->nchar) in_p[q->idx[i]] = 1;
  std::vector<uint32_t> cp(row_words, 0u), cpm(row_words, 0u);
  int bad = 0;
  for (int i = 0; i < c->nq; i++) if (!q->seq[i]) { uvaia_gpu_close(c); return fail(nullptr, UVAIA_GPU_EINVAL, "query %d is NULL", i); }
  if (pack_query_row(code_tab, q->consensus, c->nchar, 0, c->nchar, in_c.data(), nullptr, c->acgt, c->NQ, cp.data(), &bad) ||
      pack_query_row(code_tab, q->consensus, c->nchar, 0, c->nchar, in_m.data(), nullptr, c->acgt, c->NQ, cpm.data(), &bad)) {
    uvaia_gpu_close(c); return fail(nullptr, UVAIA_GPU_EALPHABET, "consensus holds byte 0x%02x outside the supported alphabet", bad);
  }
  {
    std::vector<uint32_t> pmask((size_t)c->W4 * 4, 0u);
    for (int sidx = lo; sidx < hi; sidx++) if (in_p[(size_t)sidx]) pmask[(size_t)sidx >> 5] |= 1u << (sidx & 31);
    OPENCHK(hipMalloc(&c->d_pmask, pmask.size() * 4)); OPENCHK(hipMemcpy(c->d_pmask, pmask.data(), pmask.size() * 4, hipMemcpyHostToDevice));
    std::vector<int> cols;
    for (int sidx = lo; sidx < hi; sidx++) if (in_p[(size_t)sidx]) cols.push_back(sidx);
    c->n_idx = (int)cols.size(); c->NG4 = std::max(1, ((c->n_idx + 31) / 32 + 3) / 4);
    c->idx_cols = cols;
    cols.resize(cols.size() + 1, 0);
    OPENCHK(hipMalloc(&c->d_idx_cols, cols.size() * sizeof(int))); OPENCHK(hipMemcpy(c->d_idx_cols, cols.data(), cols.size() * sizeof(int), hipMemcpyHostToDevice));
  }
  OPENCHK(hipMalloc(&c->d_stage, (size_t)2 * PACK_CHUNK * c->pitch));
  OPENCHK(hipHostMalloc(&c->h_stage, (size_t)2 * PACK_CHUNK * c->pitch, hipHostMallocDefault));
  memset(c->h_stage, 'N', (size_t)2 * PACK_CHUNK * c->pitch);
  for (int i = 0; i < 2; i++) OPENCHK(hipEventCreateWithFlags(&c->stage_free[i], hipEventDisableTiming));
  if (tn.query_tables == 1) { const int rc_ = build_query_tables_host(c, q, tn, code_tab, lo, hi, in_p); if (rc_) { uvaia_gpu_close(c); return rc_; } }
  else                      { const int rc_ = build_query_tables_device(c, q, tn, lo, hi);               if (rc_) { uvaia_gpu_close(c); return rc_; } }
  OPENCHK(hipMalloc(&c->d_cp, cp.size() * 4)); OPENCHK(hipMemcpy(c->d_cp, cp.data(), cp.size() * 4, hipMemcpyHostToDevice));
  OPENCHK(hipMalloc(&c->d_cpm, cpm.size() * 4)); OPENCHK(hipMemcpy(c->d_cpm, cpm.data(), cpm.size() * 4, hipMemcpyHostToDevice));

  OPENCHK(hipMalloc(&c->d_heap, (size_t)c->nq * (c->k + 1) * HEAP_ENTRY * sizeof(int)));
  OPENCHK(hipMalloc(&c->d_n, (size_t)c->nq * sizeof(int)));
  OPENCHK(hipMalloc(&c->d_T, (size_t)c->nq * sizeof(int)));
  OPENCHK(hipMalloc(&c->d_snap, sizeof(int)));
  OPENCHK(hipMalloc(&c->d_err, sizeof(int)));
  OPENCHK(hipMemset(c->d_err, 0, sizeof(int)));
  SliceBuf &b0 = c->slice[0];
  if (!c->fullscan) { OPENCHK(hipMalloc(&b0.cnt, (size_t)c->nq_pad * c->pool_pad * sizeof(uint32_t))); b0.cap = (size_t)c->nq_pad * c->pool_pad; }
  if (c->use_ext) {
    OPENCHK(hipMalloc(&b0.ext, (size_t)c->nq_pad * c->pool_pad * sizeof(uint32_t)));
    OPENCHK(hipMalloc(&b0.tb8, (size_t)c->nq_pad * (c->pool_pad / 64) * sizeof(uint4)));
    OPENCHK(hipMalloc(&b0.rtp, c->pool_pad * sizeof(uint32_t)));
    OPENCHK(hipMemset(b0.rtp, 0, c->pool_pad * sizeof(uint32_t)));
    const size_t l3 = replay3_lds_bytes(c);
    if (l3 > 160 * 1024) { uvaia_gpu_close(c); return fail(nullptr, UVAIA_GPU_EINVAL, "nbest=%d does not fit the LDS of the replay next to its staging buffers", heap_size); }
#define BIGLDS(K, N) OPENCHK(hipFuncSetAttribute(reinterpret_cast<const void *>(&K), hipFuncAttributeMaxDynamicSharedMemorySize, (int)(N)))
    BIGLDS((replay3_kernel<true, 32>), l3); BIGLDS((replay3_kernel<false, 32>), l3); BIGLDS((replay3_kernel<true, 16>), l3);
    BIGLDS((replay3_kernel<false, 16>), l3); BIGLDS((replay3_kernel<true, 8>), l3); BIGLDS((replay3_kernel<false, 8>), l3);
  }
  OPENCHK(hipMalloc(&b0.tmin, (size_t)c->nq_pad * (c->pool_pad / 64) * sizeof(int2)));
  OPENCHK(hipMalloc(&b0.rt, c->pool_pad * sizeof(int4)));
  OPENCHK(hipMemset(b0.rt, 0, c->pool_pad * sizeof(int4)));
  OPENCHK(hipMalloc(&c->d_stats, 16 * sizeof(unsigned long long)));
  OPENCHK(hipMemset(c->d_stats, 0, 16 * sizeof(unsigned long long)));
  OPENCHK(hipMalloc(&c->d_rt, c->pool_pad * sizeof(int4)));
  OPENCHK(hipMalloc(&c->d_tr, c->pool_pad * sizeof(int4)));
  OPENCHK(hipMemset(c->d_rt, 0, c->pool_pad * sizeof(int4)));
  OPENCHK(hipMemset(c->d_tr, 0, c->pool_pad * sizeof(int4)));
  OPENCHK(hipMalloc(&c->d_entered, c->pool_pad)); c->entered_cap = c->pool_pad;
  OPENCHK(hipMemset(c->d_entered, 0, c->pool_pad));
  const size_t lds = (size_t)(c->k + 1) * HEAP_ENTRY * sizeof(int) + 128;
  if (lds > 64 * 1024) {
    BIGLDS(replay_kernel<true>, lds); BIGLDS(replay_kernel<false>, lds);
#define BIGHEAP(PF_) BIGLDS((replay2_kernel<true, true, PF_>), lds); BIGLDS((replay2_kernel<true, false, PF_>), lds); BIGLDS((replay2_kernel<false, true, PF_>), lds); BIGLDS((replay2_kernel<false, false, PF_>), lds)
    BIGHEAP(1); BIGHEAP(2); BIGHEAP(3);
#undef BIGHEAP
  }
#undef BIGLDS
#undef OPENCHK
  int rc = uvaia_gpu_reset(c);
  if (rc) { g_open_error = c->err; uvaia_gpu_close(c); return rc; }
  *out = c;
  return UVAIA_GPU_OK;
}

int uvaia_gpu_export_query_table(uvaia_gpu_ctx *c, int which, void *out, size_t cap, size_t *n_bytes)
{
  if (!c || !n_bytes || which < 0 || which > 10) return UVAIA_GPU_EINVAL;
  if (which == 10) {
    const int v[11] = {c->NP, c->NR, c->NP4, c->NR4, c->rare_max, c->scan_variant, c->need_e_groups, c->need_v_groups, c->need_g_groups, c->need_r_groups, c->replay_lq};
    *n_bytes = sizeof v;
    if (out && cap >= sizeof v) memcpy(out, v, sizeof v);
    return UVAIA_GPU_OK;
  }
  *n_bytes = c->qtab[which].p ? c->qtab[which].n : 0;
  if (out && *n_bytes && cap >= *n_bytes) {
    HIPCHK(c, hipSetDevice(c->device));
    HIPCHK(c, hipStreamSynchronize(c->stream));
    HIPCHK(c, hipMemcpy(out, c->qtab[which].p, *n_bytes, hipMemcpyDeviceToHost));
  }
  return UVAIA_GPU_OK;
}

int uvaia_gpu_reset(uvaia_gpu_ctx *c)
{
  if (!c) return UVAIA_GPU_EINVAL;
  HIPCHK(c, hipMemsetAsync(c->d_heap, 0, (size_t)c->nq * (c->k + 1) * HEAP_ENTRY * sizeof(int), c->stream));
  hipLaunchKernelGGL(init_state_kernel, dim3((c->nq + 255) / 256), dim3(256), 0, c->stream, c->d_T, c->d_n, c->nq, c->nchar);
  HIPCHK(c, hipGetLastError());
  HIPCHK(c, hipMemcpyAsync(c->d_snap, &c->nchar, sizeof(int), hipMemcpyHostToDevice, c->stream));
  if (c->d_entered && c->db_n) HIPCHK(c, hipMemsetAsync(c->d_entered, 0, ((c->db_n + 63) / 64) * 64, c->stream));
  if (int rc = sync_scan_streams(c)) return rc;
  HIPCHK(c, hipStreamSynchronize(c->stream));
  return 0;
}

int uvaia_gpu_heap_slots(const uvaia_gpu_ctx *c) { return c ? c->k : 0; }
int uvaia_gpu_n_query(const uvaia_gpu_ctx *c) { return c ? c->nq : 0; }
size_t uvaia_gpu_packed_bytes_per_ref(const uvaia_gpu_ctx *c) { return c ? (size_t)c->W4 * 16 * c->P : 0; }
size_t uvaia_gpu_scan_bytes_per_ref(const uvaia_gpu_ctx *c)
{
  if (!c) return 0;
  return (c->fullscan || c->scan_variant != 2) ? (size_t)c->W4 * 16 * c->P
                                                : (size_t)(c->need_e_groups + c->need_v_groups) * 16 + (size_t)c->need_g_groups * 4 + (size_t)(c->NP4 + c->need_r_groups) * 16 * 3;
}

int uvaia_gpu_scan_variant(const uvaia_gpu_ctx *c)
{
  return !c ? -2 : c->fullscan ? -1 : c->scan_variant;
}

size_t uvaia_gpu_derived_bytes_per_ref(const uvaia_gpu_ctx *c)
{
  if (!c || c->fullscan || c->scan_variant != 2) return 0;
  return (size_t)c->W4 * 16 + (size_t)c->W4 * 4 + (size_t)(c->NP4 + c->NR4) * 48 + 4;
}

int uvaia_gpu_set_query_tile(uvaia_gpu_ctx *c, int qt)
{
  if (!c) return UVAIA_GPU_EINVAL;
  if (qt == 0) qt = 16;
  if (qt != 8 && qt != 16 && qt != 32) return fail(c, UVAIA_GPU_EINVAL, "query tile must be 8, 16 or 32");
  c->qt = qt;
  return 0;
}


}
```

uvaia_amd/csrc/host_qprep.inc:

```
namespace {

template <typename T>
int qprep_alloc(T **p, size_t n_elems, bool zero, hipStream_t s)
{
  hipError_t e = hipMalloc(p, std::max<size_t>(n_elems, 1) * sizeof(T));
  if (e == hipSuccess && zero) e = hipMemsetAsync(*p, 0, std::max<size_t>(n_elems, 1) * sizeof(T), s);
  if (e != hipSuccess) { *p = nullptr; return fail(nullptr, e == hipErrorOutOfMemory ? UVAIA_GPU_ENOMEM : UVAIA_GPU_EHIP, "query tables: %s", hipGetErrorString(e)); }
  return 0;
}

struct QprepScratch { std::vector<void *> p; ~QprepScratch() { for (void *x : p) if (x) hipFree(x); } };

int build_query_tables_device(uvaia_gpu_ctx *c, const uvaia_gpu_query *q, const uvaia_gpu_tuning &tn, int lo, int hi)
{
#define OPENCHK(call) HIP_TRY(call, return fail(nullptr, code_, "%s failed: %s", #call, hipGetErrorString(e_)))
#define QALLOC(ptr, n, zero) do { const int rc_ = qprep_alloc(&(ptr), (n), (zero), s); if (rc_) return rc_; } while (0)
  hipStream_t s = c->stream;
  const int Wp = c->W4 * 4, nq = c->nq;
  const size_t row_words = (size_t)Wp * c->NQ;
  QprepScratch tmp;
#define TALLOC(ptr, n, zero) do { const int rc_ = qprep_alloc(&(ptr), (n), (zero), s); if (rc_) return rc_; tmp.p.push_back(ptr); } while (0)

  QALLOC(c->d_qp, (size_t)c->nq_pad * row_words, true);
  c->qtab[0] = {c->d_qp, (size_t)c->nq_pad * row_words * 4};
  unsigned long long *d_bad = nullptr;
  TALLOC(d_bad, 1, false);
  OPENCHK(hipMemsetAsync(d_bad, 0xFF, sizeof(unsigned long long), s));
  for (int done = 0, k = 0; done < nq; done += PACK_CHUNK, k ^= 1) {
    const int m = std::min(PACK_CHUNK, nq - done);
    if (c->stage_busy[k]) { OPENCHK(hipEventSynchronize(c->stage_free[k])); c->stage_busy[k] = false; }
    uint8_t *hs = c->h_stage + (size_t)k * PACK_CHUNK * c->pitch, *ds = c->d_stage + (size_t)k * PACK_CHUNK * c->pitch;
    parallel_for(m, [&](int i) { memcpy(hs + (size_t)i * c->pitch, q->seq[done + i], (size_t)c->nchar); });
    OPENCHK(hipMemcpyAsync(ds, hs, (size_t)m * c->pitch, hipMemcpyHostToDevice, s));
    dim3 grid((unsigned)m, (unsigned)((Wp + 127) / 128));
    if (c->acgt) hipLaunchKernelGGL((qprep_pack_rows_kernel<true>), grid, dim3(128), 0, s, ds, c->pitch, m, done, c->nchar, lo, hi, c->d_pmask, Wp, c->d_qp, d_bad);
    else         hipLaunchKernelGGL((qprep_pack_rows_kernel<false>), grid, dim3(128), 0, s, ds, c->pitch, m, done, c->nchar, lo, hi, c->d_pmask, Wp, c->d_qp, d_bad);
    OPENCHK(hipGetLastError());
    OPENCHK(hipEventRecord(c->stage_free[k], s)); c->stage_busy[k] = true;
  }
  QALLOC(c->d_amb_q, (size_t)nq * AMB_STRIDE, true);
  c->qtab[2] = {c->d_amb_q, (size_t)nq * AMB_STRIDE * sizeof(int)};
  if (!c->acgt) {
    QALLOC(c->d_qp2, (size_t)c->nq_pad * Wp * 4, true);
    c->qtab[1] = {c->d_qp2, (size_t)c->nq_pad * Wp * 4 * 4};
    hipLaunchKernelGGL(qprep_recode_kernel, dim3((unsigned)nq), dim3(64), 0, s, c->d_qp, Wp, c->d_qp2, c->d_amb_q);
    OPENCHK(hipGetLastError());
  }
  const int n_shares = std::max(1, std::min(64, nq / 32)), per_share = (nq + n_shares - 1) / n_shares;
  uint32_t *d_acc = nullptr; int *d_cnt = nullptr;
  TALLOC(d_acc, (size_t)Wp * 5, true);
  QALLOC(c->d_cls, (size_t)Wp * 4, true);
  QALLOC(c->d_rmask, (size_t)Wp, true);
  c->qtab[3] = {c->d_cls, (size_t)Wp * 4 * 4}; c->qtab[4] = {c->d_rmask, (size_t)Wp * 4};
  {
    dim3 grid((unsigned)((Wp + 63) / 64), (unsigned)n_shares);
    if (c->acgt) hipLaunchKernelGGL((qprep_classes_kernel<true>), grid, dim3(64), 0, s, c->d_qp, nq, Wp, per_share, d_acc);
    else         hipLaunchKernelGGL((qprep_classes_kernel<false>), grid, dim3(64), 0, s, c->d_qp, nq, Wp, per_share, d_acc);
    hipLaunchKernelGGL(qprep_classes_finish_kernel, dim3((unsigned)((Wp + 63) / 64)), dim3(64), 0, s, d_acc, Wp, c->d_cls);
    OPENCHK(hipGetLastError());
  }
  c->rare_max = tn.rare_max > 0 ? tn.rare_max : tn.rare_max < 0 ? 0 : (nq < 64 ? 0 : std::min(64, std::max(4, nq / 64)));
  if (c->fullscan || c->scan_variant != 2) c->rare_max = 0;
  if (c->rare_max > 0) {
    TALLOC(d_cnt, (size_t)Wp * 32 * 4, true);
    dim3 grid((unsigned)((Wp * 32 + 63) / 64), (unsigned)n_shares);
    if (c->acgt) hipLaunchKernelGGL((qprep_rare_count_kernel<true>), grid, dim3(64), 0, s, c->d_qp, nq, Wp, per_share, c->d_cls, d_cnt);
    else         hipLaunchKernelGGL((qprep_rare_count_kernel<false>), grid, dim3(64), 0, s, c->d_qp, nq, Wp, per_share, c->d_cls, d_cnt);
    hipLaunchKernelGGL(qprep_rare_finish_kernel, dim3((unsigned)((Wp * 32 + 63) / 64)), dim3(64), 0, s, d_cnt, Wp, c->rare_max, c->d_cls, c->d_rmask);
    OPENCHK(hipGetLastError());
  }
  std::vector<uint32_t> cls((size_t)Wp * 4), rmask((size_t)Wp);
  unsigned long long bad = ~0ull;
  OPENCHK(hipMemcpyAsync(cls.data(), c->d_cls, cls.size() * 4, hipMemcpyDeviceToHost, s));
  OPENCHK(hipMemcpyAsync(rmask.data(), c->d_rmask, rmask.size() * 4, hipMemcpyDeviceToHost, s));
  OPENCHK(hipMemcpyAsync(&bad, d_bad, sizeof bad, hipMemcpyDeviceToHost, s));
  OPENCHK(hipStreamSynchronize(s));
  c->stage_busy[0] = c->stage_busy[1] = false;
  if (bad != ~0ull) return fail(nullptr, UVAIA_GPU_EALPHABET, "query %d holds byte 0x%02x outside the supported alphabet", (int)(bad >> 40), (unsigned)(bad & 0xFFu));
  std::vector<int> cols_p, cols_r;
  for (int w = 0; w < Wp; w++) {
    for (uint32_t m = cls[(size_t)w * 4 + 3]; m; m &= m - 1) cols_p.push_back(w * 32 + __builtin_ctz(m));
    for (uint32_t m = rmask[(size_t)w]; m; m &= m - 1) cols_r.push_back(w * 32 + __builtin_ctz(m));
  }
  c->NP = (int)cols_p.size(); c->NR = (int)cols_r.size();
  c->NP4 = ((c->NP + 31) / 32 + 3) / 4;
  c->NR4 = ((c->NR + 31) / 32 + 3) / 4;
  if (c->scan_variant == 2 && (size_t)c->NP4 * 128 + (size_t)c->NR4 * 128 > SCAN3_BIAS - 256) c->scan_variant = 0;
  {
    int split[15];
    for (int v = 0; v <= 4; v++) split[v] = (int)((long long)c->W4 * v / 4);
    for (int v = 0; v <= 4; v++) {
      int nd = 0, nr = 0;
      for (int w = 0; w < split[v] * 4; w++) { nd += __builtin_popcount(cls[(size_t)w * 4 + 3]); nr += __builtin_popcount(rmask[(size_t)w]); }
      split[5 + v] = nd; split[10 + v] = nr;
    }
    QALLOC(c->d_split, 15, false);
    OPENCHK(hipMemcpyAsync(c->d_split, split, sizeof split, hipMemcpyHostToDevice, s));
    OPENCHK(hipStreamSynchronize(s));
    c->qtab[9] = {c->d_split, sizeof split};
  }
  const size_t prow = (size_t)std::max(c->NP4, 1) * 16;
  QALLOC(c->d_qpl, (size_t)c->nq_pad * prow, true);
  QALLOC(c->d_qrare, (size_t)nq * std::max(c->NR4, 1) * 12, true);
  c->qtab[5] = {c->d_qpl, (size_t)c->nq_pad * prow * 4}; c->qtab[6] = {c->d_qrare, (size_t)nq * std::max(c->NR4, 1) * 12 * 4};
  int *d_cols = nullptr; uint32_t *d_qmin = nullptr;
  TALLOC(d_cols, cols_p.size() + cols_r.size(), false);
  TALLOC(d_qmin, (size_t)nq * std::max(c->NR4, 1) * 12, true);
  if (!cols_p.empty()) OPENCHK(hipMemcpyAsync(d_cols, cols_p.data(), cols_p.size() * sizeof(int), hipMemcpyHostToDevice, s));
  if (!cols_r.empty()) OPENCHK(hipMemcpyAsync(d_cols + cols_p.size(), cols_r.data(), cols_r.size() * sizeof(int), hipMemcpyHostToDevice, s));
  if (c->NP4 > 0) {
    dim3 grid((unsigned)nq, (unsigned)((c->NP4 * 4 + 63) / 64));
    if (c->acgt) hipLaunchKernelGGL((qprep_compress_kernel<true, false>), grid, dim3(64), 0, s, c->d_qp, nq, Wp, d_cols, c->NP, c->NP4 * 4, c->d_cls, c->d_qpl, prow, (uint32_t *)nullptr);
    else         hipLaunchKernelGGL((qprep_compress_kernel<false, false>), grid, dim3(64), 0, s, c->d_qp, nq, Wp, d_cols, c->NP, c->NP4 * 4, c->d_cls, c->d_qpl, prow, (uint32_t *)nullptr);
    OPENCHK(hipGetLastError());
  }
  if (c->NR4 > 0) {
    dim3 grid((unsigned)nq, (unsigned)((c->NR4 * 4 + 63) / 64));
    if (c->acgt) hipLaunchKernelGGL((qprep_compress_kernel<true, true>), grid, dim3(64), 0, s, c->d_qp, nq, Wp, d_cols + cols_p.size(), c->NR, c->NR4 * 4, c->d_cls, c->d_qrare, (size_t)0, d_qmin);
    else         hipLaunchKernelGGL((qprep_compress_kernel<false, true>), grid, dim3(64), 0, s, c->d_qp, nq, Wp, d_cols + cols_p.size(), c->NR, c->NR4 * 4, c->d_cls, c->d_qrare, (size_t)0, d_qmin);
    OPENCHK(hipGetLastError());
  }
  const int NWs = c->scan_NW, QS = 64, n_st = c->nq_pad / QS, NX = c->W4 + c->NR4;
  const uint32_t row_b = 256u * (uint32_t)c->scan_R;
  uint8_t *d_kind = nullptr; int *d_need = nullptr, *d_len = nullptr, *d_cost = nullptr;
  TALLOC(d_kind, (size_t)nq * c->W4, false);
  TALLOC(d_need, (size_t)c->W4, true);
  TALLOC(d_len, (size_t)n_st * NX, false);
  TALLOC(d_cost, (size_t)n_st * NX, false);
  {
    dim3 grid((unsigned)nq, (unsigned)((c->W4 + 63) / 64));
    if (c->acgt) hipLaunchKernelGGL((qprep_kinds_kernel<true>), grid, dim3(64), 0, s, c->d_qp, nq, Wp, c->d_cls, d_kind, d_need);
    else         hipLaunchKernelGGL((qprep_kinds_kernel<false>), grid, dim3(64), 0, s, c->d_qp, nq, Wp, c->d_cls, d_kind, d_need);
    hipLaunchKernelGGL(qprep_stream_sizes_kernel, dim3((unsigned)NX, (unsigned)n_st), dim3(64), 0, s, d_kind, d_qmin, nq, c->W4, c->NR4, d_len, d_cost);
    OPENCHK(hipGetLastError());
  }
  std::vector<int> need((size_t)c->W4), len((size_t)n_st * NX), cost((size_t)n_st * NX);
  OPENCHK(hipMemcpyAsync(need.data(), d_need, need.size() * sizeof(int), hipMemcpyDeviceToHost, s));
  OPENCHK(hipMemcpyAsync(len.data(), d_len, len.size() * sizeof(int), hipMemcpyDeviceToHost, s));
  OPENCHK(hipMemcpyAsync(cost.data(), d_cost, cost.size() * sizeof(int), hipMemcpyDeviceToHost, s));
  OPENCHK(hipStreamSynchronize(s));
  for (int g = 0; g < c->W4; g++) { c->need_e_groups += (need[(size_t)g] & 1) != 0; c->need_v_groups += (need[(size_t)g] & 2) != 0; c->need_g_groups += (need[(size_t)g] & 4) != 0; }
  if (c->replay_lq < 0) c->replay_lq = (nq < 256) ? 1 : 0;
  std::vector<long long> at((size_t)n_st * (NX + 1), 0);
  std::vector<uint32_t> sdir((size_t)n_st * 4 * NWs, 0u);
  std::vector<uint8_t> rare_group_used((size_t)std::max(c->NR4, 1), 0);
  size_t total = 0;
  struct Rec { size_t at; uint32_t cost; };
  auto shares = [NWs](const std::vector<Rec> &r, size_t base, size_t end_at, uint32_t *dir) {
    uint64_t tot = 0;
    for (const Rec &x : r) tot += x.cost;
    size_t i = 0; uint64_t done = 0;
    for (int w = 0; w < NWs; w++) {
      const size_t i0 = i;
      const uint64_t goal = tot * (uint64_t)(w + 1) / (uint64_t)NWs;
      while (i < r.size() && (w == NWs - 1 || done + r[i].cost / 2 < goal)) { done += r[i].cost; i++; }
      dir[2 * w] = (uint32_t)(base + (i0 < r.size() ? r[i0].at : end_at));
      dir[2 * w + 1] = (uint32_t)(i - i0);
    }
  };
  for (int st = 0; st < n_st; st++) {
    const size_t base = total;
    size_t pos = 0;
    std::vector<Rec> rec, rare;
    for (int x = 0; x < c->W4; x++) { const int L = len[(size_t)st * NX + x]; if (!L) continue; at[(size_t)st * (NX + 1) + x] = (long long)(base + pos); rec.push_back({pos, (uint32_t)cost[(size_t)st * NX + x]}); pos += (size_t)L; }
    const size_t groups_end = pos;
    at[(size_t)st * (NX + 1) + NX] = (long long)(base + pos); pos += 8;
    for (int x = c->W4; x < NX; x++) { const int L = len[(size_t)st * NX + x]; if (!L) continue; at[(size_t)st * (NX + 1) + x] = (long long)(base + pos); rare.push_back({pos, (uint32_t)cost[(size_t)st * NX + x]}); pos += (size_t)L; rare_group_used[(size_t)(x - c->W4)] = 1; }
    shares(rec, base, groups_end, &sdir[(size_t)st * 4 * NWs]);
    shares(rare, base, pos - 8, &sdir[(size_t)st * 4 * NWs + 2 * NWs]);
    total += pos;
  }
  for (uint8_t u : rare_group_used) c->need_r_groups += u;
  if (total + 64 > 0xFFFFFFFFull) return fail(nullptr, UVAIA_GPU_EINVAL, "item streams of %zu dwords", total);
  long long *d_at = nullptr;
  TALLOC(d_at, at.size(), false);
  QALLOC(c->d_stream, total + 64, true);
  QALLOC(c->d_sdir, sdir.size(), false);
  c->qtab[7] = {c->d_stream, (total + 64) * 4}; c->qtab[8] = {c->d_sdir, sdir.size() * 4};
  OPENCHK(hipMemcpyAsync(d_at, at.data(), at.size() * sizeof(long long), hipMemcpyHostToDevice, s));
  OPENCHK(hipMemcpyAsync(c->d_sdir, sdir.data(), sdir.size() * 4, hipMemcpyHostToDevice, s));
  {
    dim3 grid((unsigned)(NX + 1), (unsigned)n_st);
    if (c->acgt) hipLaunchKernelGGL((qprep_stream_fill_kernel<true>), grid, dim3(64), 0, s, c->d_qp, d_kind, d_qmin, c->d_cls, nq, Wp, c->NP4, c->NR4, d_len, d_at, row_b, c->d_stream);
    else         hipLaunchKernelGGL((qprep_stream_fill_kernel<false>), grid, dim3(64), 0, s, c->d_qp, d_kind, d_qmin, c->d_cls, nq, Wp, c->NP4, c->NR4, d_len, d_at, row_b, c->d_stream);
    OPENCHK(hipGetLastError());
  }
  OPENCHK(hipStreamSynchronize(s));
  return 0;
#undef TALLOC
#undef QALLOC
#undef OPENCHK
}

}
```

uvaia_amd/csrc/host_qtables.inc:

```
namespace {

int build_query_tables_host(uvaia_gpu_ctx *c, const uvaia_gpu_query *q, const uvaia_gpu_tuning &tn, const uint8_t *code_tab, int lo, int hi, const std::vector<uint8_t> &in_p)
{
#define OPENCHK(call) HIP_TRY(call, return fail(nullptr, code_, "%s failed: %s", #call, hipGetErrorString(e_)))
  const size_t row_words = (size_t)c->W4 * 4 * c->NQ;
  std::vector<uint32_t> qp((size_t)c->nq_pad * row_words, 0u);
  {
    std::atomic<int> first_bad(c->nq);
    std::vector<int> bad_byte((size_t)c->nq, 0);
    parallel_for(c->nq, [&](int i) {
      if (pack_query_row(code_tab, q->seq[i], c->nchar, lo, hi, nullptr, in_p.data(), c->acgt, c->NQ, qp.data() + (size_t)i * row_words, &bad_byte[(size_t)i])) {
        int cur = first_bad.load();
        while (i < cur && !first_bad.compare_exchange_weak(cur, i)) {}
      }
    });
    if (first_bad.load() < c->nq) {
      const int i = first_bad.load();
      return fail(nullptr, UVAIA_GPU_EALPHABET, "query %d holds byte 0x%02x outside the supported alphabet", i, bad_byte[(size_t)i]);
    }
  }
  OPENCHK(hipMalloc(&c->d_qp, qp.size() * 4)); OPENCHK(hipMemcpy(c->d_qp, qp.data(), qp.size() * 4, hipMemcpyHostToDevice));
  c->qtab[0] = {c->d_qp, qp.size() * 4};
  {
    std::vector<int> ambq((size_t)c->nq * AMB_STRIDE, 0);
    if (!c->acgt) {
      const size_t row2 = (size_t)c->W4 * 16;
      std::vector<uint32_t> qp2((size_t)c->nq_pad * row2, 0u);
      parallel_for(c->nq, [&](int i) { for (int w = 0; w < c->W4 * 4; w++) {
        const uint32_t *s6 = qp.data() + (size_t)i * row_words + (size_t)w * 6;
        uint32_t *d4 = qp2.data() + (size_t)i * row2 + (size_t)w * 4;
        const uint32_t one = s6[5];
        d4[0] = (s6[1] | s6[3]) & one; d4[1] = (s6[2] | s6[3]) & one; d4[2] = one; d4[3] = s6[4];
        if (s6[4] & ~one) { int &cnt = ambq[(size_t)i * AMB_STRIDE]; if (cnt < AMB_CAP) ambq[(size_t)i * AMB_STRIDE + 1 + cnt] = w; cnt++; }
      } });
      OPENCHK(hipMalloc(&c->d_qp2, qp2.size() * 4)); OPENCHK(hipMemcpy(c->d_qp2, qp2.data(), qp2.size() * 4, hipMemcpyHostToDevice));
      c->qtab[1] = {c->d_qp2, qp2.size() * 4};
    }
    {
      const int Wp = c->W4 * 4;
      auto QL = [&](int i, int w, int pl) -> uint32_t {
        if (c->acgt) { const uint32_t *s4 = qp.data() + (size_t)i * row_words + (size_t)w * 4; return pl == 3 ? s4[2] : s4[pl]; }
        const uint32_t *s6 = qp.data() + (size_t)i * row_words + (size_t)w * 6; const uint32_t one = s6[5];
        return pl == 0 ? ((s6[1] | s6[3]) & one) : pl == 1 ? ((s6[2] | s6[3]) & one) : pl == 2 ? one : s6[4];
      };
      std::vector<uint32_t> cls((size_t)Wp * 4, 0u);
      parallel_for(Wp, [&](int w) {
        uint32_t cL = 0, cH = 0, seen = 0, poly = 0;
        for (int i = 0; i < c->nq; i++) {
          const uint32_t qL = QL(i, w, 0), qH = QL(i, w, 1), qI = QL(i, w, 2);
          poly |= seen & qI & ((qL ^ cL) | (qH ^ cH));
          const uint32_t fresh = qI & ~seen;
          cL |= qL & fresh; cH |= qH & fresh; seen |= qI;
        }
        cls[(size_t)w * 4 + 0] = cL & ~poly; cls[(size_t)w * 4 + 1] = cH & ~poly; cls[(size_t)w * 4 + 2] = seen & ~poly; cls[(size_t)w * 4 + 3] = poly;
      });
      std::vector<uint32_t> rmask((size_t)Wp, 0u);
      {
        c->rare_max = tn.rare_max > 0 ? tn.rare_max : tn.rare_max < 0 ? 0 : (c->nq < 64 ? 0 : std::min(64, std::max(4, c->nq / 64)));
        if (c->fullscan || c->scan_variant != 2) c->rare_max = 0;
      }
      if (c->rare_max > 0) {
        parallel_for(Wp, [&](int w) {
          const uint32_t pm = cls[(size_t)w * 4 + 3];
          if (!pm) return;
          int cnt[32 * 4] = {0};
          for (int i = 0; i < c->nq; i++) {
            const uint32_t qL = QL(i, w, 0), qH = QL(i, w, 1);
            for (uint32_t m = QL(i, w, 2) & pm; m; m &= m - 1) { const int b = __builtin_ctz(m); cnt[(size_t)b * 4 + (((qL >> b) & 1u) | (((qH >> b) & 1u) << 1))]++; }
          }
          for (uint32_t m = pm; m; m &= m - 1) {
            const int b = __builtin_ctz(m);
            int major = 0, total = 0;
            for (int k = 0; k < 4; k++) { total += cnt[(size_t)b * 4 + k]; if (cnt[(size_t)b * 4 + k] > cnt[(size_t)b * 4 + major]) major = k; }
            if (total - cnt[(size_t)b * 4 + major] > c->rare_max) continue;
            const uint32_t bit = 1u << b;
            cls[(size_t)w * 4 + 0] = (cls[(size_t)w * 4 + 0] & ~bit) | ((major & 1) ? bit : 0u);
            cls[(size_t)w * 4 + 1] = (cls[(size_t)w * 4 + 1] & ~bit) | ((major & 2) ? bit : 0u);
            cls[(size_t)w * 4 + 2] |= bit; cls[(size_t)w * 4 + 3] &= ~bit; rmask[(size_t)w] |= bit;
          }
        });
      }
      for (int w = 0; w < Wp; w++) { c->NP += __builtin_popcount(cls[(size_t)w * 4 + 3]); c->NR += __builtin_popcount(rmask[(size_t)w]); }
      c->NP4 = ((c->NP + 31) / 32 + 3) / 4;
      c->NR4 = ((c->NR + 31) / 32 + 3) / 4;
      if (c->scan_variant == 2 && (size_t)c->NP4 * 128 + (size_t)c->NR4 * 128 > SCAN3_BIAS - 256) c->scan_variant = 0;
      struct RareWord { int word; uint32_t m, l, h; };
      std::vector<std::vector<RareWord>> rare_q((size_t)c->nq_pad);
      std::vector<uint32_t> qrare((size_t)c->nq * std::max(c->NR4, 1) * 12, 0u);
      const size_t prow = (size_t)std::max(c->NP4, 1) * 16, crow = (size_t)c->W4 * 8;
      std::vector<uint32_t> qpl((size_t)c->nq_pad * prow, 0u), qcv((size_t)c->nq_pad * crow, 0u), flg((size_t)(c->nq_pad / 16) * c->W4 * 2, 0u);
      parallel_for(c->nq_pad / 16, [&](int tile_) { for (int i = tile_ * 16; i < tile_ * 16 + 16; i++) {
        int k = 0, kr = 0;
        bool full = false;
        for (int w = 0; w < Wp; w++) {
          const bool real = i < c->nq;
          const uint32_t qL = real ? QL(i, w, 0) : 0u, qH = real ? QL(i, w, 1) : 0u, qI = real ? QL(i, w, 2) : 0u, qV = real ? QL(i, w, 3) : 0u;
          for (uint32_t m = cls[(size_t)w * 4 + 3]; m; m &= m - 1, k++) {
            const int b = __builtin_ctz(m);
            uint32_t *d = qpl.data() + (size_t)i * prow + (size_t)(k >> 7) * 16 + ((k >> 5) & 3);
            d[0] |= ((qL >> b) & 1u) << (k & 31); d[4] |= ((qH >> b) & 1u) << (k & 31); d[8] |= ((qI >> b) & 1u) << (k & 31);
          }
          const uint32_t eqb = qI & ~((qL ^ cls[(size_t)w * 4 + 0]) | (qH ^ cls[(size_t)w * 4 + 1]));
          const uint32_t nI = ~eqb & cls[(size_t)w * 4 + 2], nV = ~qV;
          for (uint32_t m = rmask[(size_t)w]; m; m &= m - 1, kr++) {
            const int b = __builtin_ctz(m);
            if (real) { uint32_t *d = qrare.data() + ((size_t)i * c->NR4 * 4 + (size_t)(kr >> 5)) * 3;
                        d[0] |= ((qL >> b) & 1u) << (kr & 31); d[1] |= ((qH >> b) & 1u) << (kr & 31); d[2] |= ((qI >> b) & 1u) << (kr & 31); }
            if (!real || !((qI >> b) & 1u) || ((eqb >> b) & 1u)) continue;
            if (rare_q[(size_t)i].empty() || rare_q[(size_t)i].back().word != (kr >> 5)) rare_q[(size_t)i].push_back({kr >> 5, 0u, 0u, 0u});
            RareWord &rw = rare_q[(size_t)i].back();
            rw.m |= 1u << (kr & 31); rw.l |= ((qL >> b) & 1u) << (kr & 31); rw.h |= ((qH >> b) & 1u) << (kr & 31);
          }
          qcv[(size_t)i * crow + (size_t)(w >> 2) * 8 + (w & 3)] = nI; qcv[(size_t)i * crow + (size_t)(w >> 2) * 8 + 4 + (w & 3)] = nV;
          uint32_t *fw = &flg[((size_t)(i / 16) * c->W4 + (w >> 2)) * 2];
          if (real && nI) fw[0] |= 1u << (i % 16);
          if (real && nV) fw[0] |= 0x10000u << (i % 16);
          if ((w & 3) == 0) full = real;
          full = full && nI == cls[(size_t)w * 4 + 2] && nV == 0xFFFFFFFFu;
          if ((w & 3) == 3 && full) { fw[0] &= ~(0x10001u << (i % 16)); fw[1] |= 1u << (i % 16); }
        }
      } });
      for (int g = 0; g < c->W4; g++) {
        uint32_t u = 0;
        uint32_t uy = 0;
        for (int t = 0; t < c->nq_pad / 16; t++) { u |= flg[((size_t)t * c->W4 + g) * 2]; uy |= flg[((size_t)t * c->W4 + g) * 2 + 1]; }
        c->need_e_groups += (u & 0xFFFFu) != 0; c->need_v_groups += (u >> 16) != 0; c->need_g_groups += uy != 0;
      }
      if (c->replay_lq < 0) c->replay_lq = (c->nq < 256) ? 1 : 0;
      OPENCHK(hipMalloc(&c->d_cls, cls.size() * 4)); OPENCHK(hipMemcpy(c->d_cls, cls.data(), cls.size() * 4, hipMemcpyHostToDevice));
      OPENCHK(hipMalloc(&c->d_qrare, qrare.size() * 4)); OPENCHK(hipMemcpy(c->d_qrare, qrare.data(), qrare.size() * 4, hipMemcpyHostToDevice));
      OPENCHK(hipMalloc(&c->d_rmask, rmask.size() * 4)); OPENCHK(hipMemcpy(c->d_rmask, rmask.data(), rmask.size() * 4, hipMemcpyHostToDevice));
      c->qtab[3] = {c->d_cls, cls.size() * 4}; c->qtab[4] = {c->d_rmask, rmask.size() * 4}; c->qtab[6] = {c->d_qrare, qrare.size() * 4};
      {
        int split[15];
        for (int v = 0; v <= 4; v++) split[v] = (int)((long long)c->W4 * v / 4);
        for (int v = 0; v <= 4; v++) {
          int nd = 0, nr = 0;
          for (int w = 0; w < split[v] * 4; w++) { nd += __builtin_popcount(cls[(size_t)w * 4 + 3]); nr += __builtin_popcount(rmask[(size_t)w]); }
          split[5 + v] = nd; split[10 + v] = nr;
        }
        OPENCHK(hipMalloc(&c->d_split, sizeof split)); OPENCHK(hipMemcpy(c->d_split, split, sizeof split, hipMemcpyHostToDevice));
        c->qtab[9] = {c->d_split, sizeof split};
      }
      OPENCHK(hipMalloc(&c->d_qpl, qpl.size() * 4)); OPENCHK(hipMemcpy(c->d_qpl, qpl.data(), qpl.size() * 4, hipMemcpyHostToDevice));
      c->qtab[5] = {c->d_qpl, qpl.size() * 4};
      const int NWs = c->scan_NW, QS = 64;
      const uint32_t row_b = 256u * (uint32_t)c->scan_R;
      struct Rec { size_t at; uint32_t cost; };
      struct TileStream { std::vector<uint32_t> u; std::vector<Rec> rec, rare; };
      const int n_st = c->nq_pad / QS;
      std::vector<TileStream> ts((size_t)n_st);
      std::vector<uint8_t> rare_groups_needed((size_t)std::max(c->NR4, 1), 0);
      parallel_for(n_st, [&](int st) {
        TileStream &S = ts[(size_t)st];
        std::vector<uint32_t> &strm = S.u;
        std::vector<int> full, gen, wrd[4];
        for (int g = 0; g < c->W4; g++) {
          full.clear(); gen.clear(); for (auto &w : wrd) w.clear();
          uint32_t wmask[64]; bool any_run = false;
          for (int ql = 0; ql < QS; ql++) {
            const int q = st * QS + ql, t = q / 16, b = q % 16;
            const uint32_t fx = flg[((size_t)t * c->W4 + g) * 2], fy = flg[((size_t)t * c->W4 + g) * 2 + 1];
            if ((fy >> b) & 1u) { full.push_back(ql); continue; }
            if (!(((fx | (fx >> 16)) >> b) & 1u)) continue;
            const uint32_t *src = qcv.data() + (size_t)q * crow + (size_t)g * 8;
            int n_part = 0, part = 0, last_full = 0;
            uint32_t fm = 0u;
            for (int j = 0; j < 4; j++) {
              if (!(src[j] | src[4 + j])) continue;
              if (src[4 + j] == 0xFFFFFFFFu && src[j] == cls[(size_t)(g * 4 + j) * 4 + 2]) { last_full = j; fm |= 0xFFu << (8 * j); }
              else { n_part++; part = j; }
            }
            int jsel = -1;
            if (n_part == 1) jsel = part;
            else if (n_part == 0) { jsel = last_full; fm &= ~(0xFFu << (8 * last_full)); }
            if (jsel >= 0) { wrd[jsel].push_back(ql); wmask[ql] = fm; any_run |= fm != 0u; } else gen.push_back(ql);
          }
          if (full.empty() && gen.empty() && wrd[0].empty() && wrd[1].empty() && wrd[2].empty() && wrd[3].empty()) continue;
          const size_t hdr = strm.size();
          const uint32_t n_full4 = (uint32_t)(full.size() + 3) / 4u;
          strm.push_back((uint32_t)g * 2048u | (any_run ? 1u : 0u));
          strm.push_back(n_full4 | (uint32_t)gen.size() << 16);
          strm.push_back((uint32_t)wrd[0].size() | (uint32_t)wrd[1].size() << 8 | (uint32_t)wrd[2].size() << 16 | (uint32_t)wrd[3].size() << 24);
          strm.push_back(0u);
          for (int ql : full) strm.push_back((uint32_t)ql * row_b);
          while (strm.size() & 3) strm.push_back((uint32_t)QS * row_b);
          for (int ql : gen) {
            const uint32_t *src = qcv.data() + (size_t)(st * QS + ql) * crow + (size_t)g * 8;
            strm.insert(strm.end(), src, src + 8);
            strm.push_back((uint32_t)ql * row_b); strm.push_back(0u); strm.push_back(0u); strm.push_back(0u);
          }
          for (int j = 0; j < 4; j++)
            for (int ql : wrd[j]) {
              const uint32_t *src = qcv.data() + (size_t)(st * QS + ql) * crow + (size_t)g * 8;
              strm.push_back(src[j]); strm.push_back(src[4 + j]); strm.push_back((uint32_t)ql * row_b); strm.push_back(wmask[ql]);
            }
          strm[hdr + 3] = (uint32_t)(strm.size() - hdr);
          S.rec.push_back({hdr, 60u + 4u * n_full4 + 30u * (uint32_t)gen.size() + 14u * (uint32_t)(wrd[0].size() + wrd[1].size() + wrd[2].size() + wrd[3].size())});
        }
        strm.push_back(0u); strm.push_back(0u); strm.push_back(0u); strm.push_back(4u);
        strm.push_back(0u); strm.push_back(0u); strm.push_back(0u); strm.push_back(4u);
        for (int r4 = 0; r4 < c->NR4; r4++) {
          uint32_t nw[4] = {0, 0, 0, 0};
          for (int ql = 0; ql < QS; ql++) for (const RareWord &rw : rare_q[(size_t)st * QS + ql]) if ((rw.word >> 2) == r4) nw[rw.word & 3]++;
          if (!(nw[0] | nw[1] | nw[2] | nw[3])) continue;
          S.rare.push_back({strm.size(), nw[0] + nw[1] + nw[2] + nw[3]});
          strm.push_back((uint32_t)(c->NP4 + r4) * 3072u); strm.push_back(nw[0] | nw[1] << 8 | nw[2] << 16 | nw[3] << 24); strm.push_back(0u); strm.push_back(0u);
          for (int j = 0; j < 4; j++)
            for (int ql = 0; ql < QS; ql++) for (const RareWord &rw : rare_q[(size_t)st * QS + ql]) if (rw.word == r4 * 4 + j) {
              strm.push_back(rw.m); strm.push_back(rw.l); strm.push_back(rw.h); strm.push_back((uint32_t)ql * row_b);
            }
          rare_groups_needed[(size_t)r4] = 1;
        }
      });
      std::vector<uint32_t> strm, sdir((size_t)n_st * 4 * NWs, 0u);
      auto split4 = [NWs](const std::vector<Rec> &r, size_t base, size_t end_at, uint32_t *dir) {
        uint64_t total = 0;
        for (const Rec &x : r) total += x.cost;
        size_t i = 0; uint64_t done = 0;
        for (int w = 0; w < NWs; w++) {
          const size_t i0 = i;
          const uint64_t goal = total * (uint64_t)(w + 1) / (uint64_t)NWs;
          while (i < r.size() && (w == NWs - 1 || done + r[i].cost / 2 < goal)) { done += r[i].cost; i++; }
          dir[2 * w] = (uint32_t)(base + (i0 < r.size() ? r[i0].at : end_at));
          dir[2 * w + 1] = (uint32_t)(i - i0);
        }
      };
      for (int st = 0; st < n_st; st++) {
        const TileStream &S = ts[(size_t)st];
        const size_t base = strm.size(), zero_hdr = S.rec.empty() ? 0 : 0;
        (void)zero_hdr;
        size_t end_at = S.u.size() - 8;
        for (const Rec &x : S.rare) { end_at = std::min(end_at, x.at - 8); break; }
        split4(S.rec, base, end_at, &sdir[(size_t)st * 4 * NWs]);
        split4(S.rare, base, S.u.size() - 8, &sdir[(size_t)st * 4 * NWs + 2 * NWs]);
        strm.insert(strm.end(), S.u.begin(), S.u.end());
      }
      for (uint8_t u : rare_groups_needed) c->need_r_groups += u;
      strm.resize(strm.size() + 64, 0u);
      OPENCHK(hipMalloc(&c->d_stream, strm.size() * 4)); OPENCHK(hipMemcpy(c->d_stream, strm.data(), strm.size() * 4, hipMemcpyHostToDevice));
      OPENCHK(hipMalloc(&c->d_sdir, sdir.size() * 4)); OPENCHK(hipMemcpy(c->d_sdir, sdir.data(), sdir.size() * 4, hipMemcpyHostToDevice));
      c->qtab[7] = {c->d_stream, strm.size() * 4}; c->qtab[8] = {c->d_sdir, sdir.size() * 4};
    }
    OPENCHK(hipMalloc(&c->d_amb_q, ambq.size() * sizeof(int))); OPENCHK(hipMemcpy(c->d_amb_q, ambq.data(), ambq.size() * sizeof(int), hipMemcpyHostToDevice));
    c->qtab[2] = {c->d_amb_q, ambq.size() * sizeof(int)};
  }
  return 0;
#undef OPENCHK
}

}
```

uvaia_amd/csrc/kernels_qprep.inc:

```

template <bool ACGT>
static __device__ __forceinline__ void qword_lhiv(const uint32_t *__restrict__ s, uint32_t &qL, uint32_t &qH, uint32_t &qI, uint32_t &qV)
{
  if (ACGT) { qL = s[0]; qH = s[1]; qI = s[2]; qV = s[2]; }
  else { const uint32_t one = s[5]; qL = (s[1] | s[3]) & one; qH = (s[2] | s[3]) & one; qI = one; qV = s[4]; }
}

template <bool ACGT>
__global__ void qprep_pack_rows_kernel(const uint8_t *__restrict__ raw, size_t pitch, int n_rows, int row0, int nchar, int lo, int hi, const uint32_t *__restrict__ pmask, int Wp,
                                       uint32_t *__restrict__ qp, unsigned long long *__restrict__ bad)
{
  constexpr int NQ = ACGT ? 4 : 6;
  const int w = blockIdx.y * blockDim.x + threadIdx.x, i = blockIdx.x;
  if (w >= Wp || i >= n_rows) return;
  const uint8_t *row = raw + (size_t)i * pitch;
  uint32_t d[NQ];
#pragma unroll
  for (int p = 0; p < NQ; p++) d[p] = 0u;
  for (int b = 0; b < 32; b++) {
    const int s = w * 32 + b;
    if (s < lo || s >= hi || s >= nchar) continue;
    const uint32_t byte = row[s], code = c_code[byte];
    if (code == 0xFFu) { atomicMin(bad, ((unsigned long long)(unsigned)(row0 + i) << 40) | ((unsigned long long)(unsigned)s << 8) | byte); continue; }
    if (!code) continue;
    const bool one = (code & (code - 1u)) == 0u;
    if (ACGT) {
      if (!one) continue;
      const uint32_t two = code == 2u ? 1u : code == 4u ? 2u : code == 8u ? 3u : 0u;
      d[0] |= (two & 1u) << b; d[1] |= (two >> 1) << b; d[2] |= 1u << b;
    } else {
#pragma unroll
      for (int p = 0; p < 4; p++) d[p] |= ((code >> p) & 1u) << b;
      d[4] |= 1u << b;
      if (one) d[5] |= 1u << b;
    }
  }
  if (ACGT) d[3] = d[2] & pmask[w];
  uint32_t *o = qp + ((size_t)(row0 + i) * Wp + w) * NQ;
#pragma unroll
  for (int p = 0; p < NQ; p++) o[p] = d[p];
}

__global__ __launch_bounds__(64) void qprep_recode_kernel(const uint32_t *__restrict__ qp, int Wp, uint32_t *__restrict__ qp2, int *__restrict__ ambq)
{
  const int i = blockIdx.x, lane = threadIdx.x;
  const uint32_t *row = qp + (size_t)i * Wp * 6;
  uint32_t *o = qp2 + (size_t)i * Wp * 4;
  int cnt = 0;
  for (int w0 = 0; w0 < Wp; w0 += 64) {
    const int w = w0 + lane;
    bool amb = false;
    if (w < Wp) {
      const uint32_t *s6 = row + (size_t)w * 6;
      const uint32_t one = s6[5];
      o[(size_t)w * 4 + 0] = (s6[1] | s6[3]) & one; o[(size_t)w * 4 + 1] = (s6[2] | s6[3]) & one; o[(size_t)w * 4 + 2] = one; o[(size_t)w * 4 + 3] = s6[4];
      amb = (s6[4] & ~one) != 0u;
    }
    const unsigned long long bal = __ballot(amb);
    const int pos = cnt + __popcll(bal & ((1ull << lane) - 1ull));
    if (amb && pos < AMB_CAP) ambq[(size_t)i * AMB_STRIDE + 1 + pos] = w;
    cnt += __popcll(bal);
  }
  if (lane == 0) ambq[(size_t)i * AMB_STRIDE] = cnt;
}

template <bool ACGT>
__global__ void qprep_classes_kernel(const uint32_t *__restrict__ qp, int nq, int Wp, int per_share, uint32_t *__restrict__ acc)
{
  constexpr int NQ = ACGT ? 4 : 6;
  const int w = blockIdx.x * blockDim.x + threadIdx.x;
  if (w >= Wp) return;
  const int i0 = blockIdx.y * per_share, i1 = min(nq, i0 + per_share);
  uint32_t l1 = 0, l0 = 0, h1 = 0, h0 = 0, seen = 0;
  for (int i = i0; i < i1; i++) {
    uint32_t qL, qH, qI, qV;
    qword_lhiv<ACGT>(qp + ((size_t)i * Wp + w) * NQ, qL, qH, qI, qV);
    l1 |= qI & qL; l0 |= qI & ~qL; h1 |= qI & qH; h0 |= qI & ~qH; seen |= qI;
  }
  uint32_t *a = acc + (size_t)w * 5;
  if (l1) atomicOr(a + 0, l1);
  if (l0) atomicOr(a + 1, l0);
  if (h1) atomicOr(a + 2, h1);
  if (h0) atomicOr(a + 3, h0);
  if (seen) atomicOr(a + 4, seen);
}
__global__ void qprep_classes_finish_kernel(const uint32_t *__restrict__ acc, int Wp, uint32_t *__restrict__ cls)
{
  const int w = blockIdx.x * blockDim.x + threadIdx.x;
  if (w >= Wp) return;
  const uint32_t *a = acc + (size_t)w * 5;
  const uint32_t poly = (a[0] & a[1]) | (a[2] & a[3]);
  cls[(size_t)w * 4 + 0] = a[0] & ~poly; cls[(size_t)w * 4 + 1] = a[2] & ~poly; cls[(size_t)w * 4 + 2] = a[4] & ~poly; cls[(size_t)w * 4 + 3] = poly;
}

template <bool ACGT>
__global__ void qprep_rare_count_kernel(const uint32_t *__restrict__ qp, int nq, int Wp, int per_share, const uint32_t *__restrict__ cls, int *__restrict__ cnt )
{
  constexpr int NQ = ACGT ? 4 : 6;
  const int col = blockIdx.x * blockDim.x + threadIdx.x;
  if (col >= Wp * 32) return;
  const int w = col >> 5, b = col & 31;
  if (!((cls[(size_t)w * 4 + 3] >> b) & 1u)) return;
  const int i0 = blockIdx.y * per_share, i1 = min(nq, i0 + per_share);
  int c0 = 0, c1 = 0, c2 = 0, c3 = 0;
  for (int i = i0; i < i1; i++) {
    uint32_t qL, qH, qI, qV;
    qword_lhiv<ACGT>(qp + ((size_t)i * Wp + w) * NQ, qL, qH, qI, qV);
    if (!((qI >> b) & 1u)) continue;
    const uint32_t code = ((qL >> b) & 1u) | ((qH >> b) & 1u) << 1;
    c0 += code == 0u; c1 += code == 1u; c2 += code == 2u; c3 += code == 3u;
  }
  int *o = cnt + (size_t)col * 4;
  if (c0) atomicAdd(o + 0, c0);
  if (c1) atomicAdd(o + 1, c1);
  if (c2) atomicAdd(o + 2, c2);
  if (c3) atomicAdd(o + 3, c3);
}
__global__ void qprep_rare_finish_kernel(const int *__restrict__ cnt, int Wp, int rare_max, uint32_t *__restrict__ cls, uint32_t *__restrict__ rmask)
{
  const int col = blockIdx.x * blockDim.x + threadIdx.x;
  if (col >= Wp * 32) return;
  const int w = col >> 5, b = col & 31;
  const uint32_t bit = 1u << b;
  if (!(cls[(size_t)w * 4 + 3] & bit)) return;
  const int *c = cnt + (size_t)col * 4;
  int major = 0, total = 0;
  for (int k = 0; k < 4; k++) { total += c[k]; if (c[k] > c[major]) major = k; }
  if (total - c[major] > rare_max) return;
  if (major & 1) atomicOr(&cls[(size_t)w * 4 + 0], bit); else atomicAnd(&cls[(size_t)w * 4 + 0], ~bit);
  if (major & 2) atomicOr(&cls[(size_t)w * 4 + 1], bit); else atomicAnd(&cls[(size_t)w * 4 + 1], ~bit);
  atomicOr(&cls[(size_t)w * 4 + 2], bit); atomicAnd(&cls[(size_t)w * 4 + 3], ~bit); atomicOr(&rmask[w], bit);
}

template <bool ACGT, bool RARE>
__global__ void qprep_compress_kernel(const uint32_t *__restrict__ qp, int nq, int Wp, const int *__restrict__ cols, int n_cols, int n_words, const uint32_t *__restrict__ cls,
                                      uint32_t *__restrict__ out, size_t out_row, uint32_t *__restrict__ qmin)
{
  constexpr int NQ = ACGT ? 4 : 6;
  const int kw = blockIdx.y * blockDim.x + threadIdx.x, i = blockIdx.x;
  if (kw >= n_words || i >= nq) return;
  uint32_t L = 0, H = 0, I = 0, M = 0;
  for (int b = 0; b < 32; b++) {
    const int k = kw * 32 + b;
    if (k >= n_cols) break;
    const int col = cols[k], w = col >> 5, cb = col & 31;
    uint32_t qL, qH, qI, qV;
    qword_lhiv<ACGT>(qp + ((size_t)i * Wp + w) * NQ, qL, qH, qI, qV);
    const uint32_t l = (qL >> cb) & 1u, h = (qH >> cb) & 1u, a = (qI >> cb) & 1u;
    L |= l << b; H |= h << b; I |= a << b;
    if (RARE) M |= (a & ((l ^ ((cls[(size_t)w * 4 + 0] >> cb) & 1u)) | (h ^ ((cls[(size_t)w * 4 + 1] >> cb) & 1u)))) << b;
  }
  if (RARE) {
    uint32_t *d = out + ((size_t)i * n_words + kw) * 3;
    d[0] = L; d[1] = H; d[2] = I;
    uint32_t *m = qmin + ((size_t)i * n_words + kw) * 3;
    m[0] = M; m[1] = L & M; m[2] = H & M;
  } else {
    uint32_t *d = out + (size_t)i * out_row + (size_t)(kw >> 2) * 16 + (kw & 3);
    d[0] = L; d[4] = H; d[8] = I;
  }
}

template <bool ACGT>
static __device__ __forceinline__ int qprep_dirty_words(const uint32_t *__restrict__ qp_row , const uint32_t *__restrict__ cls, int g, uint32_t (&nI)[4], uint32_t (&nV)[4],
                                                        uint32_t &fmask)
{
  constexpr int NQ = ACGT ? 4 : 6;
  bool full = true, anyI = false, anyV = false;
  int n_part = 0, part = 0, last_full = 0;
  uint32_t fm = 0u;
#pragma unroll
  for (int j = 0; j < 4; j++) {
    const int w = g * 4 + j;
    uint32_t qL, qH, qI, qV;
    qword_lhiv<ACGT>(qp_row + (size_t)w * NQ, qL, qH, qI, qV);
    const uint32_t c0 = cls[(size_t)w * 4 + 0], c1 = cls[(size_t)w * 4 + 1], c2 = cls[(size_t)w * 4 + 2];
    const uint32_t eqb = qI & ~((qL ^ c0) | (qH ^ c1));
    nI[j] = ~eqb & c2; nV[j] = ~qV;
    anyI |= nI[j] != 0u; anyV |= nV[j] != 0u;
    const bool fw = nI[j] == c2 && nV[j] == 0xFFFFFFFFu;
    full = full && fw;
    if (nI[j] | nV[j]) {
      if (fw) { last_full = j; fm |= 0xFFu << (8 * j); }
      else { n_part++; part = j; }
    }
  }
  fmask = 0u;
  if (full) return 1;
  if (!anyI && !anyV) return 0;
  if (n_part == 1) { fmask = fm; return 4 + part; }
  if (n_part == 0) { fmask = fm & ~(0xFFu << (8 * last_full)); return 4 + last_full; }
  return 2;
}

template <bool ACGT>
__global__ void qprep_kinds_kernel(const uint32_t *__restrict__ qp, int nq, int Wp, const uint32_t *__restrict__ cls, uint8_t *__restrict__ kind , int *__restrict__ need )
{
  constexpr int NQ = ACGT ? 4 : 6;
  const int W4 = Wp >> 2;
  const int g = blockIdx.y * blockDim.x + threadIdx.x, i = blockIdx.x;
  if (g >= W4 || i >= nq) return;
  uint32_t nI[4], nV[4], fmask;
  const int kd = qprep_dirty_words<ACGT>(qp + (size_t)i * Wp * NQ, cls, g, nI, nV, fmask);
  kind[(size_t)i * W4 + g] = (uint8_t)(kd | (fmask ? 8 : 0));
  if (kd == 1) atomicOr(&need[g], 4);
  else if (kd) atomicOr(&need[g], ((nI[0] | nI[1] | nI[2] | nI[3]) ? 1 : 0) | ((nV[0] | nV[1] | nV[2] | nV[3]) ? 2 : 0));
}

__global__ __launch_bounds__(64) void qprep_stream_sizes_kernel(const uint8_t *__restrict__ kind, const uint32_t *__restrict__ qmin, int nq, int W4, int NR4, int *__restrict__ len, int *__restrict__ cost)
{
  const int x = blockIdx.x, st = blockIdx.y, lane = threadIdx.x, q = st * 64 + lane;
  int L = 0, C = 0;
  if (x < W4) {
    const int kd = q < nq ? (kind[(size_t)q * W4 + x] & 7) : 0;
    const int n_full = __popcll(__ballot(kd == 1)), n_gen = __popcll(__ballot(kd == 2)), n_wrd = __popcll(__ballot(kd >= 4));
    if (n_full | n_gen | n_wrd) {
      const int n_full4 = (n_full + 3) / 4;
      L = 4 + 4 * n_full4 + 12 * n_gen + 4 * n_wrd;
      C = 60 + 4 * n_full4 + 30 * n_gen + 14 * n_wrd;
    }
  } else {
    const int r4 = x - W4;
    int n = 0;
#pragma unroll
    for (int j = 0; j < 4; j++) n += __popcll(__ballot(q < nq && qmin[((size_t)q * NR4 * 4 + r4 * 4 + j) * 3] != 0u));
    if (n) { L = 4 + 4 * n; C = n; }
  }
  if (lane == 0) { len[(size_t)st * (W4 + NR4) + x] = L; cost[(size_t)st * (W4 + NR4) + x] = C; }
}

template <bool ACGT>
__global__ __launch_bounds__(64) void qprep_stream_fill_kernel(const uint32_t *__restrict__ qp, const uint8_t *__restrict__ kind, const uint32_t *__restrict__ qmin, const uint32_t *__restrict__ cls,
                                                                int nq, int Wp, int NP4, int NR4, const int *__restrict__ len, const long long *__restrict__ at, uint32_t row_b,
                                                                uint32_t *__restrict__ strm)
{
  constexpr int NQ = ACGT ? 4 : 6;
  const int W4 = Wp >> 2;
  const int x = blockIdx.x, st = blockIdx.y, lane = threadIdx.x, q = st * 64 + lane;
  const size_t slot = (size_t)st * (W4 + NR4 + 1) + x;
  if (x == W4 + NR4) {
    if (lane < 8) strm[at[slot] + lane] = (lane & 3) == 3 ? 4u : 0u;
    return;
  }
  const int L = len[(size_t)st * (W4 + NR4) + x];
  if (!L) return;
  uint32_t *p = strm + at[slot];
  const unsigned long long lt = (1ull << lane) - 1ull;
  if (x < W4) {
    const int kd = q < nq ? (kind[(size_t)q * W4 + x] & 7) : 0;
    uint32_t nI[4] = {0u, 0u, 0u, 0u}, nV[4] = {0u, 0u, 0u, 0u}, fmask = 0u;
    if (kd >= 2) (void)qprep_dirty_words<ACGT>(qp + (size_t)q * Wp * NQ, cls, x, nI, nV, fmask);
    const bool any_run = __ballot(fmask != 0u) != 0ull;
    const unsigned long long b_full = __ballot(kd == 1), b_gen = __ballot(kd == 2);
    const unsigned long long b_w[4] = {__ballot(kd == 4), __ballot(kd == 5), __ballot(kd == 6), __ballot(kd == 7)};
    const int n_full = __popcll(b_full), n_full4 = (n_full + 3) / 4, n_gen = __popcll(b_gen);
    const int nw[4] = {(int)__popcll(b_w[0]), (int)__popcll(b_w[1]), (int)__popcll(b_w[2]), (int)__popcll(b_w[3])};
    if (lane == 0) { p[0] = (uint32_t)x * 2048u | (any_run ? 1u : 0u); p[1] = (uint32_t)n_full4 | (uint32_t)n_gen << 16; p[2] = (uint32_t)nw[0] | (uint32_t)nw[1] << 8 | (uint32_t)nw[2] << 16 | (uint32_t)nw[3] << 24; p[3] = (uint32_t)L; }
    if (kd == 1) p[4 + __popcll(b_full & lt)] = (uint32_t)lane * row_b;
    if (lane < n_full4 * 4 - n_full) p[4 + n_full + lane] = 64u * row_b;
    uint32_t *pg = p + 4 + 4 * n_full4;
    if (kd == 2) {
      uint32_t *d = pg + 12 * __popcll(b_gen & lt);
#pragma unroll
      for (int j = 0; j < 4; j++) { d[j] = nI[j]; d[4 + j] = nV[j]; }
      d[8] = (uint32_t)lane * row_b; d[9] = 0u; d[10] = 0u; d[11] = 0u;
    }
    uint32_t *pw = pg + 12 * n_gen;
#pragma unroll
    for (int j = 0; j < 4; j++) {
      if (kd == 4 + j) { uint32_t *d = pw + 4 * __popcll(b_w[j] & lt); d[0] = nI[j]; d[1] = nV[j]; d[2] = (uint32_t)lane * row_b; d[3] = fmask; }
      pw += 4 * nw[j];
    }
  } else {
    const int r4 = x - W4;
    uint32_t m[4], l[4], h[4];
    unsigned long long bw[4];
#pragma unroll
    for (int j = 0; j < 4; j++) {
      m[j] = l[j] = h[j] = 0u;
      if (q < nq) { const uint32_t *s = qmin + ((size_t)q * NR4 * 4 + r4 * 4 + j) * 3; m[j] = s[0]; l[j] = s[1]; h[j] = s[2]; }
      bw[j] = __ballot(m[j] != 0u);
    }
    const int nw[4] = {(int)__popcll(bw[0]), (int)__popcll(bw[1]), (int)__popcll(bw[2]), (int)__popcll(bw[3])};
    if (lane == 0) { p[0] = (uint32_t)(NP4 + r4) * 3072u; p[1] = (uint32_t)nw[0] | (uint32_t)nw[1] << 8 | (uint32_t)nw[2] << 16 | (uint32_t)nw[3] << 24; p[2] = 0u; p[3] = 0u; }
    uint32_t *pw = p + 4;
#pragma unroll
    for (int j = 0; j < 4; j++) {
      if (m[j]) { uint32_t *d = pw + 4 * __popcll(bw[j] & lt); d[0] = m[j]; d[1] = l[j]; d[2] = h[j]; d[3] = (uint32_t)lane * row_b; }
      pw += 4 * nw[j];
    }
  }
}
```

uvaia_amd/csrc/kernels_scan3.inc:

```


typedef uint32_t u32x4_nt __attribute__((ext_vector_type(4)));
static __device__ __forceinline__ void st_stream(uint4 *p, const uint4 &v)
{
  const u32x4_nt x = {v.x, v.y, v.z, v.w};
  __builtin_nontemporal_store(x, reinterpret_cast<u32x4_nt *>(p));
}
struct GatherStage { uint32_t bL, bH, bI; int fill, ow; };

static __device__ __forceinline__ int shared_slot(const int *__restrict__ bit, int word)
{
  for (int k = 1; k <= 3; k++) if ((bit[k] & 31) != 0 && (bit[k] >> 5) == word) return k;
  return 0;
}
static __device__ __forceinline__ uint32_t take_bit(uint32_t x, int b, int at, uint32_t acc)
{
  return (__builtin_amdgcn_ubfe(x, (uint32_t)b, 1u) << at) | acc;
}

template <bool ACGT, bool WRITE_V>
__global__ __launch_bounds__(256) __attribute__((amdgpu_waves_per_eu(8, 8)))
void derive_all_kernel(const uint4 *__restrict__ tiles, long long tile_base, long long dtile_base, int W4,
                       const uint32_t *__restrict__ cls, const uint32_t *__restrict__ rmask,
                       const int *__restrict__ split, int NP4, int NR4,
                       uint4 *__restrict__ ev, int *__restrict__ tot_e, uint32_t *__restrict__ grp, uint4 *__restrict__ poly)
{
  constexpr int P = ACGT ? 3 : 4;
  __shared__ int partial[4][64];
  __shared__ uint32_t shr[6][3][64];
  for (int i = threadIdx.x; i < 6 * 3 * 64; i += 256) (&shr[0][0][0])[i] = 0u;
  __syncthreads();
  const int lane = threadIdx.x & 63, wv = __builtin_amdgcn_readfirstlane(threadIdx.x >> 6);
  const long long ptile = tile_base + blockIdx.x, tile = dtile_base + blockIdx.x;
  const uint4 *t = tiles + (size_t)ptile * W4 * P * 64 + lane;
  uint4 *o = ev + (size_t)tile * W4 * 2 * 64 + lane;
  const int NG = NP4 + NR4;
  uint32_t *po = reinterpret_cast<uint32_t *>(poly + (size_t)tile * NG * 3 * 64 + lane);
  const int lo = split[wv], hi = split[wv + 1];
  const int *dbit = split + 5, *rbit = split + 10;

  GatherStage D, R;
  D.bL = D.bH = D.bI = 0u; D.fill = dbit[wv] & 31; D.ow = dbit[wv] >> 5;
  R.bL = R.bH = R.bI = 0u; R.fill = rbit[wv] & 31; R.ow = rbit[wv] >> 5;
  int sw[2][3];
#pragma unroll
  for (int sec = 0; sec < 2; sec++) {
    const int *bit = sec ? rbit : dbit;
#pragma unroll
    for (int k = 1; k <= 3; k++) sw[sec][k - 1] = (bit[k] & 31) != 0 ? (bit[k] >> 5) : -1;
  }
  auto push_word = [&](GatherStage &g, int sec) {
    const int k = (sw[sec][0] == g.ow) ? 1 : (sw[sec][1] == g.ow) ? 2 : (sw[sec][2] == g.ow) ? 3 : 0;
    if (k) {
      uint32_t (*dst)[64] = shr[sec * 3 + k - 1];
      if (g.bL) atomicOr(&dst[0][lane], g.bL);
      if (g.bH) atomicOr(&dst[1][lane], g.bH);
      if (g.bI) atomicOr(&dst[2][lane], g.bI);
    } else {
      uint32_t *d = po + (size_t)((sec ? NP4 : 0) + (g.ow >> 2)) * 3 * 256 + (g.ow & 3);
      d[0] = g.bL; d[256] = g.bH; d[512] = g.bI;
    }
    g.bL = g.bH = g.bI = 0u; g.fill = 0; g.ow++;
  };

  int te = 0;
  uint4 nxt[P];
#pragma unroll
  for (int p = 0; p < P; p++) nxt[p] = lo < hi ? ld_stream(t + (size_t)(lo * P + p) * 64) : make_uint4(0u, 0u, 0u, 0u);
  for (int w4 = lo; w4 < hi; w4++) {
    uint4 pl[P];
#pragma unroll
    for (int p = 0; p < P; p++) pl[p] = nxt[p];
    if (w4 + 1 < hi) {
#pragma unroll
      for (int p = 0; p < P; p++) nxt[p] = ld_stream(t + (size_t)((w4 + 1) * P + p) * 64);
    }
    uint32_t e[4], v[4];
    int ge = 0, gv = 0;
#pragma unroll
    for (int j = 0; j < 4; j++) {
      uint32_t rL, rH, rI, rV;
      if (ACGT) { rL = u4c(pl[0], j); rH = u4c(pl[1], j); rI = u4c(pl[2], j); rV = rI; }
      else {
        const uint32_t a = u4c(pl[0], j), cc = u4c(pl[1], j), g = u4c(pl[2], j), tt = u4c(pl[P - 1], j);
        const uint32_t par = a ^ cc ^ g ^ tt, three = (a & cc & (g | tt)) | (g & tt & (a | cc));
        rI = par & ~three; rL = (cc | tt) & rI; rH = (g | tt) & rI; rV = a | cc | g | tt;
      }
      const uint32_t *c4 = cls + (size_t)(w4 * 4 + j) * 4;
      const uint32_t diff = (rL ^ c4[0]) | (rH ^ c4[1]);
      e[j] = rI & c4[2] & (ACGT ? diff : ~diff);
      v[j] = rV;
      ge += __popc(e[j]); gv += __popc(v[j]);
      for (uint32_t m = c4[3]; m; m &= m - 1) {
        const int b = __ffs(m) - 1;
        D.bL = take_bit(rL, b, D.fill, D.bL); D.bH = take_bit(rH, b, D.fill, D.bH); D.bI = take_bit(rI, b, D.fill, D.bI);
        if (++D.fill == 32) push_word(D, 0);
      }
      for (uint32_t m = rmask[w4 * 4 + j]; m; m &= m - 1) {
        const int b = __ffs(m) - 1;
        R.bL = take_bit(rL, b, R.fill, R.bL); R.bH = take_bit(rH, b, R.fill, R.bH); R.bI = take_bit(rI, b, R.fill, R.bI);
        if (++R.fill == 32) push_word(R, 1);
      }
    }
    te += ge;
    __builtin_nontemporal_store((uint32_t)ge | ((uint32_t)gv << 16), grp + ((size_t)tile * W4 + w4) * 64 + lane);
    st_stream(o + (size_t)(w4 * 2 + 0) * 64, make_uint4(e[0], e[1], e[2], e[3]));
    if (WRITE_V) st_stream(o + (size_t)(w4 * 2 + 1) * 64, make_uint4(v[0], v[1], v[2], v[3]));
  }
  if (NP4 && D.fill > 0) push_word(D, 0);
  if (NR4 && R.fill > 0) push_word(R, 1);
  if (wv == 3) {
    for (int w = (dbit[4] + 31) >> 5; w < NP4 * 4; w++) { uint32_t *d = po + (size_t)(w >> 2) * 3 * 256 + (w & 3); d[0] = 0u; d[256] = 0u; d[512] = 0u; }
    for (int w = (rbit[4] + 31) >> 5; w < NR4 * 4; w++) { uint32_t *d = po + (size_t)(NP4 + (w >> 2)) * 3 * 256 + (w & 3); d[0] = 0u; d[256] = 0u; d[512] = 0u; }
  }
  partial[wv][lane] = te;
  __syncthreads();
  if (wv == 0) tot_e[tile * 64 + lane] = partial[0][lane] + partial[1][lane] + partial[2][lane] + partial[3][lane];
  else {
    for (int sec = 0; sec < 2; sec++) {
      const int *bit = sec ? rbit : dbit;
      if ((sec ? NR4 : NP4) == 0 || (bit[wv] & 31) == 0) continue;
      const int w = bit[wv] >> 5;
      if (shared_slot(bit, w) != wv) continue;
      const uint32_t (*src)[64] = shr[sec * 3 + wv - 1];
      uint32_t *d = po + (size_t)((sec ? NP4 : 0) + (w >> 2)) * 3 * 256 + (w & 3);
      d[0] = src[0][lane]; d[256] = src[1][lane]; d[512] = src[2][lane];
    }
  }
}

template <int R> struct Scan3Acc;
template <> struct Scan3Acc<1> { typedef uint32_t type; };
template <> struct Scan3Acc<2> { typedef unsigned long long type; };
struct Scan3Acc4 { unsigned long long a, b; };
template <> struct Scan3Acc<4> { typedef Scan3Acc4 type; };
static __device__ __forceinline__ uint32_t acc_part(uint32_t v, int) { return v; }
static __device__ __forceinline__ uint32_t acc_part(unsigned long long v, int rr) { return (uint32_t)(v >> (32 * rr)); }
static __device__ __forceinline__ uint32_t acc_part(const Scan3Acc4 &v, int rr) { return (uint32_t)((rr < 2 ? v.a : v.b) >> (32 * (rr & 1))); }
typedef __attribute__((address_space(3))) char scan3_lds_char;
static __device__ __forceinline__ void lds_counter_add(scan3_lds_char *p, uint32_t v)
{ __hip_atomic_fetch_add((__attribute__((address_space(3))) uint32_t *)p, v, __ATOMIC_RELAXED, __HIP_MEMORY_SCOPE_WORKGROUP); }
static __device__ __forceinline__ void lds_counter_add(scan3_lds_char *p, unsigned long long v)
{ __hip_atomic_fetch_add((__attribute__((address_space(3))) unsigned long long *)p, v, __ATOMIC_RELAXED, __HIP_MEMORY_SCOPE_WORKGROUP); }
static __device__ __forceinline__ void lds_counter_add(scan3_lds_char *p, const Scan3Acc4 &v)
{
  __hip_atomic_fetch_add((__attribute__((address_space(3))) unsigned long long *)p, v.a, __ATOMIC_RELAXED, __HIP_MEMORY_SCOPE_WORKGROUP);
  __hip_atomic_fetch_add((__attribute__((address_space(3))) unsigned long long *)(p + 8), v.b, __ATOMIC_RELAXED, __HIP_MEMORY_SCOPE_WORKGROUP);
}
template <class T> static __device__ __forceinline__ void lds_counter_store(scan3_lds_char *p, const T &v) { *(__attribute__((address_space(3))) T *)p = v; }
static __device__ __forceinline__ void lds_counter_store(scan3_lds_char *p, const Scan3Acc4 &v)
{ *(__attribute__((address_space(3))) unsigned long long *)p = v.a; *(__attribute__((address_space(3))) unsigned long long *)(p + 8) = v.b; }
template <class T> static __device__ __forceinline__ void lds_counter_load(scan3_lds_char *p, T &v) { v = *(__attribute__((address_space(3))) T *)p; }
static __device__ __forceinline__ void lds_counter_load(scan3_lds_char *p, Scan3Acc4 &v)
{ v.a = *(__attribute__((address_space(3))) unsigned long long *)p; v.b = *(__attribute__((address_space(3))) unsigned long long *)(p + 8); }
static __device__ __forceinline__ void lds_counter_sub(scan3_lds_char *p, uint32_t v)
{ __hip_atomic_fetch_sub((__attribute__((address_space(3))) uint32_t *)p, v, __ATOMIC_RELAXED, __HIP_MEMORY_SCOPE_WORKGROUP); }
static __device__ __forceinline__ void lds_counter_sub(scan3_lds_char *p, unsigned long long v)
{ __hip_atomic_fetch_sub((__attribute__((address_space(3))) unsigned long long *)p, v, __ATOMIC_RELAXED, __HIP_MEMORY_SCOPE_WORKGROUP); }
static __device__ __forceinline__ void lds_counter_sub(scan3_lds_char *p, const Scan3Acc4 &v)
{
  __hip_atomic_fetch_sub((__attribute__((address_space(3))) unsigned long long *)p, v.a, __ATOMIC_RELAXED, __HIP_MEMORY_SCOPE_WORKGROUP);
  __hip_atomic_fetch_sub((__attribute__((address_space(3))) unsigned long long *)(p + 8), v.b, __ATOMIC_RELAXED, __HIP_MEMORY_SCOPE_WORKGROUP);
}

template <int NW , bool ACGT, int R, int QS = 64 >
__global__ __launch_bounds__(64 * NW) __attribute__((amdgpu_waves_per_eu(4, 8))) void scan3_kernel(const uint4 *__restrict__ ev, const uint4 *__restrict__ poly, long long tile_first, int n_tiles,
                                                     int W4, int NP4, int NPT, const uint32_t *__restrict__ qpl, const uint32_t *__restrict__ stream,
                                                     const uint32_t *__restrict__ sdir, const uint32_t *__restrict__ grp,
                                                     const int *__restrict__ tot_e, const int *__restrict__ tot_v,
                                                     uint32_t *__restrict__ out, int ppad, int n_stiles, int2 *__restrict__ tmin, int r_lo, int r_hi,
                                                     int stile_first, unsigned *__restrict__ progress )
{
  constexpr int QT = QS / NW;
  static_assert((NW == 4 || NW == 8 || NW == 16) && (QS == 64 || QS == 128) && QT >= 4 && QT <= 16, "waves and queries of a super-tile");
  static_assert(R == 1 || R == 2 || R == 4, "one, two or four reference tiles per wave");
  typedef typename Scan3Acc<R>::type acc_t;
  constexpr uint32_t RARE_BIAS = SCAN3_BIAS;
  __shared__ acc_t lacc[QS + 1][64];
  const int lane = threadIdx.x & 63, wave = __builtin_amdgcn_readfirstlane(threadIdx.x >> 6);
  int stile, group;
  if (!scan_work_item(n_stiles, (n_tiles + R - 1) / R, stile, group)) return;
  const int trel0 = group * R;
  stile += stile_first;
  const int q0 = stile * QS + wave * QT;
  int trel[R]; bool live[R];
#pragma unroll
  for (int rr = 0; rr < R; rr++) { live[rr] = trel0 + rr < n_tiles; trel[rr] = live[rr] ? trel0 + rr : trel0; }
  scan3_lds_char *my = (scan3_lds_char *)&lacc[wave * QT][lane];
  auto pack_acc = [](const uint32_t (&v)[R]) -> acc_t {
    if constexpr (R == 1) return v[0];
    else if constexpr (R == 2) return (acc_t)v[0] | ((acc_t)v[1] << 32);
    else return acc_t{(unsigned long long)v[0] | ((unsigned long long)v[1] << 32), (unsigned long long)v[2] | ((unsigned long long)v[3] << 32)};
  };
  {
    int acc[R][QT];
#pragma unroll
    for (int rr = 0; rr < R; rr++)
#pragma unroll
      for (int q = 0; q < QT; q++) acc[rr][q] = 0;
    {
      const uint4 *t[R];
#pragma unroll
      for (int rr = 0; rr < R; rr++) t[rr] = poly + (size_t)(tile_first + trel[rr]) * NPT * 3 * 64 + lane;
      const size_t qstride = (size_t)NP4 * 16;
      const uint32_t *qb = qpl + (size_t)q0 * qstride;
      for (int p4 = 0; p4 < NP4; p4++) {
        uint4 pL[R], pH[R], pI[R];
#pragma unroll
        for (int rr = 0; rr < R; rr++) { pL[rr] = t[rr][(size_t)(p4 * 3 + 0) * 64]; pH[rr] = t[rr][(size_t)(p4 * 3 + 1) * 64]; pI[rr] = t[rr][(size_t)(p4 * 3 + 2) * 64]; }
        const uint32_t *s0 = qb + (size_t)p4 * 16;
        QWords<12> cur, nxt;
        load_qwords(cur, s0);
#pragma unroll
        for (int q = 0; q < QT; q++) {
          if (q + 1 < QT) load_qwords(nxt, s0 + (size_t)(q + 1) * qstride);
          __builtin_amdgcn_sched_barrier(0);
#pragma unroll
          for (int rr = 0; rr < R; rr++)
#pragma unroll
            for (int j = 0; j < 4; j++) {
              const uint32_t d = u4c(pL[rr], j) ^ cur.v[j];
              const uint32_t y = B3(u4c(pH[rr], j), cur.v[4 + j], d, (TT_A ^ TT_B) | TT_C);
              acc[rr][q] = bcnt_acc(ACGT ? B3(y, u4c(pI[rr], j), cur.v[8 + j], TT_A & TT_B & TT_C) : B3(y, u4c(pI[rr], j), cur.v[8 + j], ~(~TT_A & TT_B & TT_C)), acc[rr][q]);
            }
          __builtin_amdgcn_sched_barrier(0);
          if (q + 1 < QT) cur = nxt;
        }
      }
    }
#pragma unroll
    for (int q = 0; q < QT; q++) {
      uint32_t init[R];
#pragma unroll
      for (int rr = 0; rr < R; rr++) {
        if (ACGT) init[rr] = RARE_BIAS - (uint32_t)acc[rr][q];
        else init[rr] = (uint32_t)acc[rr][q] + RARE_BIAS;
      }
      lds_counter_store(my + (size_t)q * 64 * sizeof(acc_t), pack_acc(init));
    }
  }
  __syncthreads();
  {
    const uint4 *t[R]; const uint32_t *gt[R];
#pragma unroll
    for (int rr = 0; rr < R; rr++) { t[rr] = ev + (size_t)(tile_first + trel[rr]) * W4 * 2 * 64 + lane; gt[rr] = grp + (size_t)(tile_first + trel[rr]) * W4 * 64 + lane; }
    typedef __attribute__((address_space(4))) const uint32_t cst_u32;
    const cst_u32 *dir = (const cst_u32 *)(sdir + (size_t)stile * 4 * NW);
    const cst_u32 *sp = (const cst_u32 *)(stream + dir[2 * wave]);
    scan3_lds_char *myc = (scan3_lds_char *)&lacc[0][lane];
#define LDS_ADD(byte_off, val) lds_counter_add(myc + (byte_off), (val))
#define LDS_SUB(byte_off, val) lds_counter_sub(myc + (byte_off), (val))
#define TOUCH_ITEM(it) asm volatile("" ::"s"(it.v[0]), "s"(it.v[1]), "s"(it.v[2]), "s"(it.v[3]), "s"(it.v[4]), "s"(it.v[5]), "s"(it.v[6]), "s"(it.v[7]), "s"(it.v[8]))
#define TOUCH4(it) asm volatile("" ::"s"(it.v[0]), "s"(it.v[1]), "s"(it.v[2]), "s"(it.v[3]))
    struct Planes { uint4 E[R], V[R]; uint32_t g[R]; };
    Planes PA, PB;
    auto request = [&](Planes &P, uint32_t h0) {
#pragma unroll
      for (int rr = 0; rr < R; rr++) {
        const char *tg = reinterpret_cast<const char *>(t[rr]) + (h0 & ~1023u);
        P.E[rr] = *reinterpret_cast<const uint4 *>(tg);
        P.V[rr] = *reinterpret_cast<const uint4 *>(tg + 1024);
        P.g[rr] = *reinterpret_cast<const uint32_t *>(reinterpret_cast<const char *>(gt[rr]) + ((h0 & ~1023u) >> 3));
      }
    };
    QWords<4> h, hn, hnn;
    load_qwords(h, sp);
    const cst_u32 *sp_n = sp + h.v[3];
    load_qwords(hn, sp_n);
    request(PA, h.v[0]);
    const uint32_t n_rec = dir[2 * wave + 1];
#define RECORD(P, Pn)                                                                                                             \
    {                                                                                                                             \
      const uint32_t n_full4 = h.v[1] & 0xFFFFu, n_gen = h.v[1] >> 16, n_words = h.v[2];                                          \
      const cst_u32 *sp_nn = sp_n + hn.v[3];                                                                                      \
      load_qwords(hnn, sp_nn);                                                                                                    \
      request(Pn, hn.v[0]);                                                                                                       \
      sp += 4;                                                                                                                    \
                                   \
      const cst_u32 *ip = sp + n_full4 * 4u, *wp = ip + n_gen * 12u;                                                              \
      QWords<9> a, b;                                                                                                             \
      QWords<4> it, nx;                                                                                                           \
      load_qwords(a, ip);                                                                                                         \
      load_qwords(it, wp);                                                                                                        \
      if (n_full4) {     \
        const acc_t gg = pack_acc(P.g);                                                                                           \
        _Pragma("unroll 1") for (uint32_t k = 0; k < n_full4; k++, sp += 4) {       \
          QWords<4> o;                                                                                                            \
          load_qwords(o, sp);                                                                                                     \
          LDS_ADD(o.v[0], gg); LDS_ADD(o.v[1], gg); LDS_ADD(o.v[2], gg); LDS_ADD(o.v[3], gg);                                     \
        }                                                                                                                         \
      }                                                                                                                           \
      if (n_gen) {                                                                                                                \
         \
         \
                 \
        TOUCH_ITEM(a);                                                                                                            \
        for (uint32_t k = 0; k < n_gen; k += 2, ip += 24) {                                                                       \
          acc_t va, vb;                                                                                                           \
          load_qwords(b, ip + 12);                              \
          __builtin_amdgcn_sched_barrier(0);                                                                                      \
          ITEM_VALUE(P, a, va);                                                                                                   \
          const uint32_t off_a = a.v[8];                                                                                          \
          __builtin_amdgcn_sched_barrier(0);                                                                                      \
          TOUCH_ITEM(b);                                                                                                          \
          LDS_ADD(off_a, va);                                                                                                     \
          if (k + 1 < n_gen) {                                                                                                    \
            load_qwords(a, ip + 24);                                                                                              \
            __builtin_amdgcn_sched_barrier(0);                                                                                    \
            ITEM_VALUE(P, b, vb);                                                                                                 \
            const uint32_t off_b = b.v[8];                                                                                        \
            __builtin_amdgcn_sched_barrier(0);                                                                                    \
            TOUCH_ITEM(a);                                                                                                        \
            LDS_ADD(off_b, vb);                                                                                                   \
          }                                                                                                                       \
        }                                                                                                                         \
      }                                                                                                                           \
      if (n_words) {     \
                                                   \
        uint32_t wE[R], wV[R];       \
        _Pragma("unroll") for (int rr = 0; rr < R; rr++) { wE[rr] = 0u; wV[rr] = 0u; }                                            \
        if (h.v[0] & 1u) {                                                                                                        \
          _Pragma("unroll") for (int rr = 0; rr < R; rr++) {                                                                      \
            wE[rr] = (uint32_t)bcnt_acc(P.E[rr].x, 0) | (uint32_t)bcnt_acc(P.E[rr].y, 0) << 8 | (uint32_t)bcnt_acc(P.E[rr].z, 0) << 16 | (uint32_t)bcnt_acc(P.E[rr].w, 0) << 24; \
            wV[rr] = (uint32_t)bcnt_acc(P.V[rr].x, 0) | (uint32_t)bcnt_acc(P.V[rr].y, 0) << 8 | (uint32_t)bcnt_acc(P.V[rr].z, 0) << 16 | (uint32_t)bcnt_acc(P.V[rr].w, 0) << 24; \
          }                                                                                                                       \
        }                                                                                                                         \
        TOUCH4(it);                                                                                                               \
        WORD_ITEMS(P, 0) WORD_ITEMS(P, 1) WORD_ITEMS(P, 2) WORD_ITEMS(P, 3)                                                       \
      }                                                                                                                           \
      sp = sp_n; sp_n = sp_nn; h = hn; hn = hnn;                                                                                  \
    }
#define ITEM_VALUE(P, it, dst)                                                                                      \
    {                                                                                                               \
      uint32_t pk_[R];                                                                                              \
      _Pragma("unroll") for (int rr = 0; rr < R; rr++) {                                                            \
        int e_ = 0, v_ = 0;                                                                                         \
        _Pragma("unroll") for (int j = 0; j < 4; j++) e_ = bcnt_acc(u4c(P.E[rr], j) & it.v[j], e_);                 \
        _Pragma("unroll") for (int j = 0; j < 4; j++) v_ = bcnt_acc(u4c(P.V[rr], j) & it.v[4 + j], v_);             \
        pk_[rr] = (uint32_t)e_ | ((uint32_t)v_ << 16);                                                              \
      }                                                                                                             \
      dst = pack_acc(pk_);                                                                                          \
    }
         \
#define WORD_ITEM(P, J, cur, ahead)                                                                                               \
        {                                                                                                                         \
          __builtin_amdgcn_sched_barrier(0);                                                                                      \
          uint32_t pk_[R];                                                                                                        \
          _Pragma("unroll") for (int rr = 0; rr < R; rr++)                                                                        \
            pk_[rr] = (uint32_t)bcnt_acc(u4c(P.E[rr], J) & cur.v[0], 0) | ((uint32_t)bcnt_acc(u4c(P.V[rr], J) & cur.v[1], 0) << 16); \
          if (cur.v[3]) {      \
            _Pragma("unroll") for (int rr = 0; rr < R; rr++)                                                                      \
              pk_[rr] += __builtin_amdgcn_sad_u8(wE[rr] & cur.v[3], 0u, 0u) | (__builtin_amdgcn_sad_u8(wV[rr] & cur.v[3], 0u, 0u) << 16); \
          }                                                                                                                       \
          const uint32_t off_ = cur.v[2];                                                                                         \
          __builtin_amdgcn_sched_barrier(0);                                                                                      \
          TOUCH4(ahead);                                                                                                          \
          LDS_ADD(off_, pack_acc(pk_));                                                                                           \
        }
     \
     \
#define WORD_ITEMS(P, J)                                                                                                          \
        {                                                                                                                         \
          uint32_t k = (n_words >> (8 * J)) & 255u;                                                                               \
          _Pragma("unroll 1") for (; k >= 2; k -= 2) {                                                                            \
            load_qwords(nx, wp + 4);                                                                                              \
            WORD_ITEM(P, J, it, nx)                                                                                               \
            wp += 8;                                                                                                              \
            load_qwords(it, wp);                                                                                                  \
            WORD_ITEM(P, J, nx, it)                                                                                               \
          }                                                                                                                       \
          if (k) {                                                                                                                \
            wp += 4;                                                                                                              \
            load_qwords(nx, wp);                                                                                                  \
            WORD_ITEM(P, J, it, nx)                                                                                               \
            it = nx;                                                                                                              \
          }                                                                                                                       \
        }
    for (uint32_t rec = 0; rec < n_rec; rec += 2) {
      RECORD(PA, PB)
      if (rec + 1 < n_rec) RECORD(PB, PA)
    }
#undef RECORD
#undef ITEM_VALUE
#undef WORD_ITEMS
#undef WORD_ITEM
    {
      const char *tr[R];
#pragma unroll
      for (int rr = 0; rr < R; rr++) tr[rr] = reinterpret_cast<const char *>(poly + (size_t)(tile_first + trel[rr]) * NPT * 3 * 64 + lane);
      sp = (const cst_u32 *)(stream + dir[2 * NW + 2 * wave]);
      for (uint32_t rec = 0; rec < dir[2 * NW + 2 * wave + 1]; rec++) {
        QWords<2> hr;
        load_qwords(hr, sp);
        sp += 4;
        uint4 pL[R], pH[R], pI[R];
#pragma unroll
        for (int rr = 0; rr < R; rr++) {
          pL[rr] = *reinterpret_cast<const uint4 *>(tr[rr] + hr.v[0]); pH[rr] = *reinterpret_cast<const uint4 *>(tr[rr] + hr.v[0] + 1024);
          pI[rr] = *reinterpret_cast<const uint4 *>(tr[rr] + hr.v[0] + 2048);
        }
        const uint32_t n_words = hr.v[1];
        QWords<4> it, nx;
        load_qwords(it, sp);
        TOUCH4(it);
#define RARE_ITEM(J, cur, ahead)                                                                                                  \
        {                                                                                                                         \
          __builtin_amdgcn_sched_barrier(0);                                                                                      \
          uint32_t c_[R];                                                                                                         \
          _Pragma("unroll") for (int rr = 0; rr < R; rr++) {                                                                      \
            const uint32_t d_ = u4c(pL[rr], J) ^ cur.v[1];                                                                        \
            const uint32_t y_ = B3(u4c(pH[rr], J), cur.v[2], d_, (TT_A ^ TT_B) | TT_C);                                           \
            const uint32_t g_ = ACGT ? B3(y_, u4c(pI[rr], J), cur.v[0], TT_A & TT_B & TT_C) : B3(y_, u4c(pI[rr], J), cur.v[0], ~TT_A & TT_B & TT_C); \
            c_[rr] = (uint32_t)bcnt_acc(g_, 0);                                                                                   \
          }                                                                                                                       \
          const uint32_t off_ = cur.v[3];                                                                                         \
          __builtin_amdgcn_sched_barrier(0);                                                                                      \
          TOUCH4(ahead);                                                                                                          \
          LDS_SUB(off_, pack_acc(c_));                             \
        }
#define RARE_ITEMS(J)                                                                                                             \
        {                                                                                                                         \
          uint32_t k = (n_words >> (8 * J)) & 255u;                                                                               \
          _Pragma("unroll 1") for (; k >= 2; k -= 2) {                                                                            \
            load_qwords(nx, sp + 4);                                                                                              \
            RARE_ITEM(J, it, nx)                                                                                                  \
            sp += 8;                                                                                                              \
            load_qwords(it, sp);                                                                                                  \
            RARE_ITEM(J, nx, it)                                                                                                  \
          }                                                                                                                       \
          if (k) {                                                                                                                \
            sp += 4;                                                                                                              \
            load_qwords(nx, sp);                                                                                                  \
            RARE_ITEM(J, it, nx)                                                                                                  \
            it = nx;                                                                                                              \
          }                                                                                                                       \
        }
        RARE_ITEMS(0) RARE_ITEMS(1) RARE_ITEMS(2) RARE_ITEMS(3)
#undef RARE_ITEMS
#undef RARE_ITEM
      }
    }
#undef LDS_ADD
#undef LDS_SUB
#undef TOUCH_ITEM
#undef TOUCH4
  }
  __syncthreads();
  int te[R], tv[R]; bool in_batch[R]; size_t r[R];
#pragma unroll
  for (int rr = 0; rr < R; rr++) {
    r[rr] = (size_t)trel[rr] * 64 + lane;
    te[rr] = tot_e[r[rr]]; tv[rr] = tot_v[r[rr]];
    in_batch[rr] = ((int)r[rr] >= r_lo && (int)r[rr] < r_hi);
  }
#pragma unroll
  for (int q = 0; q < QT; q++) {
    acc_t pkk;
    lds_counter_load(my + (size_t)q * 64 * sizeof(acc_t), pkk);
#pragma unroll
    for (int rr = 0; rr < R; rr++) {
      if (!live[rr]) continue;
      const uint32_t pk = acc_part(pkk, rr);
      const int c0 = (ACGT ? te[rr] : te[rr] + NP4 * 128) - ((int)(pk & 0xFFFFu) - (int)RARE_BIAS), c1 = tv[rr] - (int)(pk >> 16);
#ifndef PIPE_PLAIN_STORES
      if (progress) __hip_atomic_store(out + (size_t)(q0 + q) * ppad + r[rr], (uint32_t)c0 | ((uint32_t)c1 << 16), __ATOMIC_RELAXED, __HIP_MEMORY_SCOPE_AGENT);
      else
#endif
      out[(size_t)(q0 + q) * ppad + r[rr]] = (uint32_t)c0 | ((uint32_t)c1 << 16);
      const int mm = ACGT ? c0 : c1 - c0, kk = ACGT ? c1 - c0 : c0;
      const uint32_t mx_m = wave_max_dpp(in_batch[rr] ? 65536u - (uint32_t)mm : 0u), mx_k = wave_max_dpp(in_batch[rr] ? (uint32_t)kk + 1u : 0u);
      const int m = mx_m ? (int)(65536u - mx_m) : 0x7fffffff, k = mx_k ? (int)(mx_k - 1u) : (int)0x80000000;
      if (lane == 0) {
        int2 *tp = tmin + (size_t)(q0 + q) * (ppad >> 6) + trel[rr];
        if (progress) __hip_atomic_store(reinterpret_cast<unsigned long long *>(tp), (unsigned long long)(unsigned)m | ((unsigned long long)(unsigned)k << 32), __ATOMIC_RELAXED, __HIP_MEMORY_SCOPE_AGENT);
        else *tp = make_int2(m, k);
      }
    }
    __builtin_amdgcn_sched_barrier(0);
  }
  if (progress) {
    asm volatile("s_waitcnt vmcnt(0)" ::: "memory");
    __syncthreads();
    if (threadIdx.x == 0) __hip_atomic_fetch_add(progress + (trel0 / SCAN_STRIPE_TILES), 1u, __ATOMIC_RELAXED, __HIP_MEMORY_SCOPE_AGENT);
  }
}
```

uvaia_amd/csrc/uvaia_gpu.hip:

```cpp
#include <hip/hip_runtime.h>

#include <algorithm>
#include <atomic>
#include <cstdarg>
#include <cstdint>
#include <cstdio>
#include <cstdlib>
#include <condition_variable>
#include <cstring>
#include <functional>
#include <mutex>
#include <string>
#include <thread>
#include <vector>

#include "../../include/uvaia_gpu.h"
#include "iupac_decode.h"

#define TT_A 0xF0u
#define TT_B 0xCCu
#define TT_C 0xAAu
#define B3(a, b, c, tt) __builtin_amdgcn_bitop3_b32((a), (b), (c), (tt) & 0xFFu)

static __device__ __forceinline__ uint32_t u4c(const uint4 &v, int j)
{
  return j == 0 ? v.x : j == 1 ? v.y : j == 2 ? v.z : v.w;
}

typedef uint32_t u32x4_ld __attribute__((ext_vector_type(4)));
static __device__ __forceinline__ uint4 ld_stream(const uint4 *p)
{
  const u32x4_ld v = __builtin_nontemporal_load(reinterpret_cast<const u32x4_ld *>(p));
  return make_uint4(v.x, v.y, v.z, v.w);
}

static __device__ __forceinline__ int bcnt_acc(uint32_t x, int acc)
{
  int r;
  asm("v_bcnt_u32_b32 %0, %1, %2" : "=v"(r) : "v"(x), "v"(acc));
  return r;
}

namespace {

constexpr int HEAP_ENTRY = 8;
constexpr int AMB_CAP = 11;
constexpr int AMB_STRIDE = AMB_CAP + 1;
constexpr int AMB_ROW = 64;
constexpr int PACK_CHUNK = 4096;
constexpr uint32_t SCAN3_BIAS = 16384u;
constexpr int SCAN_STRIPE_TILES = 64;
constexpr int NBUF = 4;

thread_local std::string g_open_error;

struct ScanEvt { hipEvent_t a, b; double bytes; };

struct TileStore {
  uint4 *planes = nullptr;
  int *nonn = nullptr;
  int *amb = nullptr;
  int *tot = nullptr;
  uint4 *ev = nullptr, *poly = nullptr;
  uint32_t *grp = nullptr;
  int *tote = nullptr;
};

struct SliceBuf {
  uint32_t *cnt = nullptr;
  int2 *tmin = nullptr;
  uint32_t *ext = nullptr;
  uint32_t *rtp = nullptr;
  uint4 *tb8 = nullptr;
  int4 *rt = nullptr;
  size_t cap = 0;
  int tiles = 0, rb = 0, re = 0; long long tf = 0;
  bool scanned = false, cons_done = false, piped = false;
  unsigned *progress = nullptr; size_t progress_cap = 0;
  hipEvent_t scan_done = nullptr, scan_started = nullptr, replay_done = nullptr;
  bool replay_recorded = false;
};

}

struct uvaia_gpu_ctx {
  int device = 0;
  hipStream_t stream = nullptr;
  hipStream_t scan_streams[3] = {};
  unsigned scan_rr = 0;
  int scan_nstreams = 1;
  int scan_nstreams_forced = 0;
  int first_slice_pct = 70;
  hipStream_t scan_stream = nullptr;
  struct DeriveChunk { long long t0, t1; hipEvent_t done; };
  hipStream_t derive_stream = nullptr;
  hipStream_t derive_streams[3] = {};
  int derive_nstreams = 3; bool derive_forced = false;
  std::vector<DeriveChunk> derive_chunks;
  hipEvent_t derive_fence[4] = {};
  size_t derive_pending = 0;
  bool pipeline = false, pipeline_now = false, pipe_used = false;
  int *d_pipe_err = nullptr;
  SliceBuf slice[NBUF];
  bool use_ext = false;
  size_t subslice = 25088;
  bool subslice_forced = false;
  int nq = 0, nq_pad = 0, nchar = 0, W = 0, W4 = 0, P = 4, NQ = 6, acgt = 0, k = 2, qt = 16, n_idx_c = 0, n_idx_m = 0;
  size_t trim = 0;
  size_t max_pool = 0, pool_pad = 0;
  uint32_t *d_qp = nullptr;
  uint32_t *d_qp2 = nullptr;
  int scan_variant = 2;
  uint32_t *d_cls = nullptr;
  uint32_t *d_qpl = nullptr;
  uint32_t *d_stream = nullptr;
  uint32_t *d_sdir = nullptr;
  int NP = 0, NP4 = 0;
  int NR = 0, NR4 = 0, rare_max = -1;
  uint32_t *d_rmask = nullptr;
  int *d_split = nullptr;
  int shard_rank = 0, shard_world = 1; long long shard_pt = 0;
  const uint4 *peer_db[64] = {}; const int *peer_amb[64] = {};
  void *ipc_opened[64][2] = {};
  uint32_t *d_qrare = nullptr;
  int need_e_groups = 0, need_v_groups = 0, need_g_groups = 0, need_r_groups = 0;
  int act_q0 = 0, act_q1 = 0;
  bool serial = false;
  int replay_lq = -1;
  int replay_prio = 1;
  bool head_full = false;
  int replay_half = 32;
  int replay_cus = 0;
  hipStream_t rep_stream = nullptr; hipEvent_t rep_ev[2] = {};
  int scan_R = 2;
  int scan_NW = 8;
  int *d_amb_q = nullptr;
  struct { const void *p; size_t n; } qtab[10] = {};
  unsigned long long *d_stats = nullptr;
  hipEvent_t order_ev[16] = {}; unsigned order_rr = 0;
  hipEvent_t mark_ev[8][3] = {}; bool mark_set[8][3] = {};
  bool fullscan = false;
  size_t cnt_cap = 0;
  uint32_t *d_cp = nullptr;
  uint32_t *d_cpm = nullptr;
  uint32_t *d_qpoly = nullptr;
  uint32_t *d_pmask = nullptr;
  int *d_mindist = nullptr, *d_ball_list = nullptr, *d_ball_cdist = nullptr, *d_ball_n = nullptr; size_t ball_cap = 0;
  uint4 *d_ball_tiles = nullptr; size_t ball_tiles_cap = 0; unsigned long long ball_asked = 0;
  bool ball_fused = true; uint4 *d_ball_ga = nullptr; size_t ball_ga_tiles = 0;
  hipEvent_t ball_ev[4] = {}; double ball_ms[3] = {0., 0., 0.};
  int *d_idx_cols = nullptr; int n_idx = 0, NG4 = 0;
  std::vector<int> idx_cols; uint32_t *d_ball_masks = nullptr; int NH4 = 0;
  uint32_t *d_qg = nullptr;
  unsigned long long *d_ball_key = nullptr;
  uint4 *d_pk = nullptr; int pk_n = 0;
  uint8_t *d_rows = nullptr; size_t rows_cap = 0;
  int *d_row_idx = nullptr; size_t row_idx_cap = 0;
  int *d_rsel = nullptr, *d_rcnt = nullptr; unsigned long long *d_roff = nullptr; uint2 *d_rexc = nullptr;
  size_t rsel_cap = 0, rcnt_cap = 0, roff_cap = 0, rexc_cap = 0;
  std::vector<int> rows_host; std::vector<uint2> rexc_host;
  uint32_t run_cut = 0xFFFFFFu;
  std::vector<hipEvent_t> rows_evs; double rows_ms[3] = {0., 0., 0.};
  struct StageSlot { uint4 *planes = nullptr; int *nonn = nullptr, *side = nullptr; int n_tiles = 0; hipEvent_t copied = nullptr, read = nullptr; bool read_recorded = false; };
  StageSlot wstage[2]; size_t wstage_tiles = 0;
  hipStream_t copy_stream = nullptr;
  int *d_wsel = nullptr; size_t wsel_cap = 0;
  uint4 *d_win4 = nullptr; size_t win4_tiles = 0; int win_n = 0;
  hipEvent_t win_ev[5] = {}; double win_ms[3] = {0., 0., 0.};
  int *d_heap = nullptr, *d_n = nullptr, *d_T = nullptr, *d_snap = nullptr, *d_err = nullptr;
  TileStore batch;
  int4 *d_cnt = nullptr;
  int4 *d_rt = nullptr, *d_tr = nullptr;
  uint8_t *d_entered = nullptr;
  size_t entered_cap = 0;
  uint8_t *d_stage = nullptr;
  uint8_t *h_stage = nullptr;
  hipEvent_t stage_free[2] = {}; bool stage_busy[2] = {};
  size_t pitch = 0;
  TileStore db;
  size_t db_cap = 0, db_n = 0, db_local_tiles = 0;
  struct { const TileStore *store = nullptr; long long tile_first = 0; int n_tiles = 0, n = 0, rbegin = 0, ppad = 0; const int4 *rt = nullptr; } last;
  std::vector<ScanEvt> evts;
  std::vector<hipEvent_t> ev_pool;
  double scan_ms = 0, scan_bytes = 0; long long scan_launches = 0;
  bool profile = true;
  std::string err;
};

namespace {

int fail(uvaia_gpu_ctx *c, int code, const char *fmt, ...)
{
  char buf[512];
  va_list ap; va_start(ap, fmt); vsnprintf(buf, sizeof buf, fmt, ap); va_end(ap);
  if (c) c->err = buf; else g_open_error = buf;
  return code;
}

#define HIP_TRY(call, on_fail) do { hipError_t e_ = (call); if (e_ != hipSuccess) { const int code_ = e_ == hipErrorOutOfMemory ? UVAIA_GPU_ENOMEM : UVAIA_GPU_EHIP; (void)code_; on_fail; } } while (0)
#define HIPCHK(c, call) HIP_TRY(call, return fail((c), code_, "%s failed: %s (%s:%d)", #call, hipGetErrorString(e_), __FILE__, __LINE__))

inline bool owns_tile(const uvaia_gpu_ctx *c, long long t) { return c->shard_world == 1 || (t / c->shard_pt) % c->shard_world == c->shard_rank; }
inline long long dtile_of(const uvaia_gpu_ctx *c, long long t)
{ return c->shard_world == 1 ? t : (t / (c->shard_pt * c->shard_world)) * c->shard_pt + t % c->shard_pt; }
template <class F> inline int for_owned_tiles(const uvaia_gpu_ctx *c, long long gt0, long long gt1, F f)
{
  if (c->shard_world == 1) return gt1 > gt0 ? f(gt0, gt0, gt1 - gt0) : 0;
  for (long long a = gt0; a < gt1;) {
    const long long b = std::min(gt1, (a / c->shard_pt + 1) * c->shard_pt);
    if (owns_tile(c, a)) { const int rc = f(a, dtile_of(c, a), b - a); if (rc) return rc; }
    a = b;
  }
  return 0;
}
inline size_t derived_tiles(const uvaia_gpu_ctx *c, size_t tiles)
{ return c->shard_world == 1 ? tiles : (size_t)((tiles + (size_t)(c->shard_pt * c->shard_world) - 1) / (size_t)(c->shard_pt * c->shard_world)) * (size_t)c->shard_pt; }

void fill_code_table(uint8_t *t)
{
  memset(t, 0xFF, 256);
  const char *inv = "NnXx-?Oo.";
  for (const char *p = inv; *p; p++) t[(unsigned char)*p] = 0;
  static const struct { char c; uint8_t m; } iu[] = {
    {'A',1},{'C',2},{'G',4},{'T',8},{'M',3},{'R',5},{'W',9},{'S',6},{'Y',10},{'K',12},{'V',7},{'H',11},{'D',13},{'B',14}};
  for (auto &e : iu) { t[(unsigned char)e.c] = e.m; t[(unsigned char)(e.c + 32)] = e.m; }
}

}

#include "kernels_pack.inc"
#include "kernels_rows.inc"
#include "kernels_consensus.inc"
#include "kernels_scan_history.inc"
#include "kernels_scan3.inc"
#include "kernels_replay.inc"
#include "kernels_ball.inc"
#include "kernels_qprep.inc"

#include "host_launch.inc"
#include "host_qtables.inc"
#include "host_qprep.inc"
#include "host_open.inc"
#include "host_batch.inc"
#include "host_resident.inc"
#include "host_rows.inc"
#include "host_shards.inc"
#include "host_ball.inc"
#include "host_window.inc"
```

Baseline: 33.18 million.

## Add LDS ring-buffer item streaming path to scan3 and udot4 run counts

Adds an optional RING variant of scan3_kernel that stages the per-wave item stream through a 512-byte LDS ring, refilled from global memory, instead of reading items through scalar constant loads. It is selected by a new scan_items tuning field and is off by default. The run-word encoding changes from 0xFF byte masks to 0x01 bytes so the run counts can be summed with udot4 instead of sad_u8 on the default path. The stream padding also grows to 512 dwords to cover ring prefetch overrun.

```diff
diff --git a/include/uvaia_gpu.h b/include/uvaia_gpu.h
--- a/include/uvaia_gpu.h
+++ b/include/uvaia_gpu.h
@@ -54,6 +54,7 @@
   int scan_streams;
   int pipeline;
   int head_scan;
+  int scan_items;
 } uvaia_gpu_tuning;
 int uvaia_gpu_export_query_table (uvaia_gpu_ctx *ctx, int which, void *out, size_t cap, size_t *n_bytes);
 int uvaia_gpu_open_tuned (uvaia_gpu_ctx **ctx, const uvaia_gpu_query *query, int heap_size, int device, size_t max_pool, const uvaia_gpu_tuning *tuning );
diff --git a/uvaia_amd/capi.py b/uvaia_amd/capi.py
--- a/uvaia_amd/capi.py
+++ b/uvaia_amd/capi.py
@@ -40,7 +40,7 @@
 
 class Tuning(C.Structure):
     _fields_ = [("subslice_refs", C.c_size_t), ("rare_max", C.c_int), ("scan", C.c_int), ("serial", C.c_int),
-                ("scan_tiles_per_wave", C.c_int), ("scan_waves_per_block", C.c_int), ("rederive_streams", C.c_int), ("ball_gather", C.c_int), ("query_tables", C.c_int), ("replay_extras", C.c_int), ("replay_cus", C.c_int), ("scan_streams", C.c_int), ("pipeline", C.c_int), ("head_scan", C.c_int)]
+                ("scan_tiles_per_wave", C.c_int), ("scan_waves_per_block", C.c_int), ("rederive_streams", C.c_int), ("ball_gather", C.c_int), ("query_tables", C.c_int), ("replay_extras", C.c_int), ("replay_cus", C.c_int), ("scan_streams", C.c_int), ("pipeline", C.c_int), ("head_scan", C.c_int), ("scan_items", C.c_int)]
 
     SCAN = {"auto": 0, "packed": 1, "compressed": 2, "wide": 3}
 
diff --git a/uvaia_amd/csrc/host_launch.inc b/uvaia_amd/csrc/host_launch.inc
--- a/uvaia_amd/csrc/host_launch.inc
+++ b/uvaia_amd/csrc/host_launch.inc
@@ -221,7 +221,8 @@
     const int st_first = c->act_q0 / QS, n_st = (c->act_q1 + QS - 1) / QS - st_first;
     const int R = c->scan_R;
     dim3 grid3(scan_grid_size(n_st, (n_tiles + R - 1) / R));
-#define SCAN3_LAUNCH(NWW, A, RR) hipLaunchKernelGGL((scan3_kernel<NWW, A, RR>), grid3, dim3(64 * NWW), 0, stream, s.ev, s.poly, tile_first, n_tiles, c->W4, c->NP4, c->NP4 + c->NR4, c->d_qpl, c->d_stream, c->d_sdir, s.grp, tote, tot_tile0, out, ppad, n_st, tmin, r_lo, r_hi, st_first, progress)
+#define SCAN3_LAUNCH_(NWW, A, RR, RG) hipLaunchKernelGGL((scan3_kernel<NWW, A, RR, QS, RG>), grid3, dim3(64 * NWW), 0, stream, s.ev, s.poly, tile_first, n_tiles, c->W4, c->NP4, c->NP4 + c->NR4, c->d_qpl, c->d_stream, c->d_sdir, s.grp, tote, tot_tile0, out, ppad, n_st, tmin, r_lo, r_hi, st_first, progress)
+#define SCAN3_LAUNCH(NWW, A, RR) do { if (c->scan_ring) SCAN3_LAUNCH_(NWW, A, RR, true); else SCAN3_LAUNCH_(NWW, A, RR, false); } while (0)
 #define SCAN3_NW(A, RR) { if (c->scan_NW == 8) SCAN3_LAUNCH(8, A, RR); else SCAN3_LAUNCH(4, A, RR); }
     if (progress) { consensus_rt(); HIPCHK(c, hipGetLastError()); }
     if (R == 4)      { if (c->acgt) SCAN3_LAUNCH(8, true, 4); else SCAN3_LAUNCH(8, false, 4); }
@@ -229,6 +230,7 @@
     else             { if (c->acgt) SCAN3_NW(true, 1) else SCAN3_NW(false, 1) }
 #undef SCAN3_NW
 #undef SCAN3_LAUNCH
+#undef SCAN3_LAUNCH_
     HIPCHK(c, hipGetLastError());
     if (c->profile) { HIPCHK(c, hipEventRecord(ev_.b, stream)); ev_.bytes = bytes; c->evts.push_back(ev_); }
     if (!progress) consensus_rt();
diff --git a/uvaia_amd/csrc/host_open.inc b/uvaia_amd/csrc/host_open.inc
--- a/uvaia_amd/csrc/host_open.inc
+++ b/uvaia_amd/csrc/host_open.inc
@@ -44,7 +44,7 @@
   memset(&tn, 0, sizeof tn);
   if (tune) tn = *tune;
   if (tn.scan < 0 || tn.scan > UVAIA_GPU_SCAN_WIDE || tn.query_tables < 0 || tn.query_tables > 2 || (tn.scan_tiles_per_wave != 0 && tn.scan_tiles_per_wave != 1 && tn.scan_tiles_per_wave != 2 && tn.scan_tiles_per_wave != 4) ||
-      (tn.scan_waves_per_block != 0 && tn.scan_waves_per_block != 4 && tn.scan_waves_per_block != 8) || (tn.subslice_refs != 0 && tn.subslice_refs < 64))
+      (tn.scan_waves_per_block != 0 && tn.scan_waves_per_block != 4 && tn.scan_waves_per_block != 8) || (tn.subslice_refs != 0 && tn.subslice_refs < 64) || tn.scan_items < 0 || tn.scan_items > 2)
     return fail(nullptr, UVAIA_GPU_EINVAL, "bad tuning values");
   if (!out) return fail(nullptr, UVAIA_GPU_EINVAL, "ctx is NULL");
   *out = nullptr;
@@ -69,6 +69,7 @@
   c->serial = tn.serial != 0;
   if (tn.scan_tiles_per_wave) c->scan_R = tn.scan_tiles_per_wave;
   if (tn.scan_waves_per_block) c->scan_NW = tn.scan_waves_per_block;
+  if (tn.scan_items) c->scan_ring = tn.scan_items == 2;
   if (c->scan_R == 4 && c->scan_NW != 8) { delete c; return fail(nullptr, UVAIA_GPU_EINVAL, "four reference tiles per wave go with eight waves per block"); }
   if (tn.subslice_refs) { c->subslice = tn.subslice_refs; c->subslice_forced = true; }
   if (tn.scan_streams >= 1 && tn.scan_streams <= 3) c->scan_nstreams_forced = tn.scan_streams;
diff --git a/uvaia_amd/csrc/host_qprep.inc b/uvaia_amd/csrc/host_qprep.inc
--- a/uvaia_amd/csrc/host_qprep.inc
+++ b/uvaia_amd/csrc/host_qprep.inc
@@ -171,12 +171,12 @@
     total += pos;
   }
   for (uint8_t u : rare_group_used) c->need_r_groups += u;
-  if (total + 64 > 0xFFFFFFFFull) return fail(nullptr, UVAIA_GPU_EINVAL, "item streams of %zu dwords", total);
+  if (total + SCAN3_STREAM_PAD > 0xFFFFFFFFull) return fail(nullptr, UVAIA_GPU_EINVAL, "item streams of %zu dwords", total);
   long long *d_at = nullptr;
   TALLOC(d_at, at.size(), false);
-  QALLOC(c->d_stream, total + 64, true);
+  QALLOC(c->d_stream, total + SCAN3_STREAM_PAD, true);
   QALLOC(c->d_sdir, sdir.size(), false);
-  c->qtab[7] = {c->d_stream, (total + 64) * 4}; c->qtab[8] = {c->d_sdir, sdir.size() * 4};
+  c->qtab[7] = {c->d_stream, (total + SCAN3_STREAM_PAD) * 4}; c->qtab[8] = {c->d_sdir, sdir.size() * 4};
   OPENCHK(hipMemcpyAsync(d_at, at.data(), at.size() * sizeof(long long), hipMemcpyHostToDevice, s));
   OPENCHK(hipMemcpyAsync(c->d_sdir, sdir.data(), sdir.size() * 4, hipMemcpyHostToDevice, s));
   {
diff --git a/uvaia_amd/csrc/host_qtables.inc b/uvaia_amd/csrc/host_qtables.inc
--- a/uvaia_amd/csrc/host_qtables.inc
+++ b/uvaia_amd/csrc/host_qtables.inc
@@ -168,12 +168,12 @@
             uint32_t fm = 0u;
             for (int j = 0; j < 4; j++) {
               if (!(src[j] | src[4 + j])) continue;
-              if (src[4 + j] == 0xFFFFFFFFu && src[j] == cls[(size_t)(g * 4 + j) * 4 + 2]) { last_full = j; fm |= 0xFFu << (8 * j); }
+              if (src[4 + j] == 0xFFFFFFFFu && src[j] == cls[(size_t)(g * 4 + j) * 4 + 2]) { last_full = j; fm |= 0x01u << (8 * j); }
               else { n_part++; part = j; }
             }
             int jsel = -1;
             if (n_part == 1) jsel = part;
-            else if (n_part == 0) { jsel = last_full; fm &= ~(0xFFu << (8 * last_full)); }
+            else if (n_part == 0) { jsel = last_full; fm &= ~(0x01u << (8 * last_full)); }
             if (jsel >= 0) { wrd[jsel].push_back(ql); wmask[ql] = fm; any_run |= fm != 0u; } else gen.push_back(ql);
           }
           if (full.empty() && gen.empty() && wrd[0].empty() && wrd[1].empty() && wrd[2].empty() && wrd[3].empty()) continue;
@@ -237,7 +237,7 @@
         strm.insert(strm.end(), S.u.begin(), S.u.end());
       }
       for (uint8_t u : rare_groups_needed) c->need_r_groups += u;
-      strm.resize(strm.size() + 64, 0u);
+      strm.resize(strm.size() + SCAN3_STREAM_PAD, 0u);
       OPENCHK(hipMalloc(&c->d_stream, strm.size() * 4)); OPENCHK(hipMemcpy(c->d_stream, strm.data(), strm.size() * 4, hipMemcpyHostToDevice));
       OPENCHK(hipMalloc(&c->d_sdir, sdir.size() * 4)); OPENCHK(hipMemcpy(c->d_sdir, sdir.data(), sdir.size() * 4, hipMemcpyHostToDevice));
       c->qtab[7] = {c->d_stream, strm.size() * 4}; c->qtab[8] = {c->d_sdir, sdir.size() * 4};
diff --git a/uvaia_amd/csrc/kernels_qprep.inc b/uvaia_amd/csrc/kernels_qprep.inc
--- a/uvaia_amd/csrc/kernels_qprep.inc
+++ b/uvaia_amd/csrc/kernels_qprep.inc
@@ -181,7 +181,7 @@
     const bool fw = nI[j] == c2 && nV[j] == 0xFFFFFFFFu;
     full = full && fw;
     if (nI[j] | nV[j]) {
-      if (fw) { last_full = j; fm |= 0xFFu << (8 * j); }
+      if (fw) { last_full = j; fm |= 0x01u << (8 * j); }
       else { n_part++; part = j; }
     }
   }
@@ -189,7 +189,7 @@
   if (full) return 1;
   if (!anyI && !anyV) return 0;
   if (n_part == 1) { fmask = fm; return 4 + part; }
-  if (n_part == 0) { fmask = fm & ~(0xFFu << (8 * last_full)); return 4 + last_full; }
+  if (n_part == 0) { fmask = fm & ~(0x01u << (8 * last_full)); return 4 + last_full; }
   return 2;
 }
 
diff --git a/uvaia_amd/csrc/kernels_scan3.inc b/uvaia_amd/csrc/kernels_scan3.inc
--- a/uvaia_amd/csrc/kernels_scan3.inc
+++ b/uvaia_amd/csrc/kernels_scan3.inc
@@ -163,7 +163,7 @@
   __hip_atomic_fetch_sub((__attribute__((address_space(3))) unsigned long long *)(p + 8), v.b, __ATOMIC_RELAXED, __HIP_MEMORY_SCOPE_WORKGROUP);
 }
 
-template <int NW , bool ACGT, int R, int QS = 64 >
+template <int NW , bool ACGT, int R, int QS = 64 , bool RING = false >
 __global__ __launch_bounds__(64 * NW) __attribute__((amdgpu_waves_per_eu(4, 8))) void scan3_kernel(const uint4 *__restrict__ ev, const uint4 *__restrict__ poly, long long tile_first, int n_tiles,
                                                      int W4, int NP4, int NPT, const uint32_t *__restrict__ qpl, const uint32_t *__restrict__ stream,
                                                      const uint32_t *__restrict__ sdir, const uint32_t *__restrict__ grp,
@@ -246,8 +246,9 @@
     for (int rr = 0; rr < R; rr++) { t[rr] = ev + (size_t)(tile_first + trel[rr]) * W4 * 2 * 64 + lane; gt[rr] = grp + (size_t)(tile_first + trel[rr]) * W4 * 64 + lane; }
     typedef __attribute__((address_space(4))) const uint32_t cst_u32;
     const cst_u32 *dir = (const cst_u32 *)(sdir + (size_t)stile * 4 * NW);
-    const cst_u32 *sp = (const cst_u32 *)(stream + dir[2 * wave]);
     scan3_lds_char *myc = (scan3_lds_char *)&lacc[0][lane];
+#define SCAN3_RUN_DOT(counts, ones) __builtin_amdgcn_udot4((counts), (ones), 0u, false)
+#define SCAN3_RUN_SUM(word, counts, ones) ((uint32_t)__builtin_popcount(word) + SCAN3_RUN_DOT(counts, ones))
 #define LDS_ADD(byte_off, val) lds_counter_add(myc + (byte_off), (val))
 #define LDS_SUB(byte_off, val) lds_counter_sub(myc + (byte_off), (val))
 #define TOUCH_ITEM(it) asm volatile("" ::"s"(it.v[0]), "s"(it.v[1]), "s"(it.v[2]), "s"(it.v[3]), "s"(it.v[4]), "s"(it.v[5]), "s"(it.v[6]), "s"(it.v[7]), "s"(it.v[8]))
@@ -263,6 +264,8 @@
         P.g[rr] = *reinterpret_cast<const uint32_t *>(reinterpret_cast<const char *>(gt[rr]) + ((h0 & ~1023u) >> 3));
       }
     };
+    if constexpr (!RING) {
+    const cst_u32 *sp = (const cst_u32 *)(stream + dir[2 * wave]);
     QWords<4> h, hn, hnn;
     load_qwords(h, sp);
     const cst_u32 *sp_n = sp + h.v[3];
@@ -315,7 +318,7 @@
           }                                                                                                                       \
         }                                                                                                                         \
       }                                                                                                                           \
-      if (n_words) {     \
+      if (n_words) {        \
                                                    \
         uint32_t wE[R], wV[R];       \
         _Pragma("unroll") for (int rr = 0; rr < R; rr++) { wE[rr] = 0u; wV[rr] = 0u; }                                            \
@@ -346,11 +349,18 @@
         {                                                                                                                         \
           __builtin_amdgcn_sched_barrier(0);                                                                                      \
           uint32_t pk_[R];                                                                                                        \
-          _Pragma("unroll") for (int rr = 0; rr < R; rr++)                                                                        \
-            pk_[rr] = (uint32_t)bcnt_acc(u4c(P.E[rr], J) & cur.v[0], 0) | ((uint32_t)bcnt_acc(u4c(P.V[rr], J) & cur.v[1], 0) << 16); \
-          if (cur.v[3]) {      \
+          if (cur.v[3]) {     \
+            \
+            \
+            uint32_t dE_[R], dV_[R], aE_[R], aV_[R];                                                                              \
+            _Pragma("unroll") for (int rr = 0; rr < R; rr++) { dE_[rr] = SCAN3_RUN_DOT(wE[rr], cur.v[3]); dV_[rr] = SCAN3_RUN_DOT(wV[rr], cur.v[3]); }\
+            _Pragma("unroll") for (int rr = 0; rr < R; rr++) { aE_[rr] = u4c(P.E[rr], J) & cur.v[0]; aV_[rr] = u4c(P.V[rr], J) & cur.v[1]; }\
+            __builtin_amdgcn_sched_barrier(0);                                                                                    \
             _Pragma("unroll") for (int rr = 0; rr < R; rr++)                                                                      \
-              pk_[rr] += __builtin_amdgcn_sad_u8(wE[rr] & cur.v[3], 0u, 0u) | (__builtin_amdgcn_sad_u8(wV[rr] & cur.v[3], 0u, 0u) << 16); \
+              pk_[rr] = ((uint32_t)__builtin_popcount(aE_[rr]) + dE_[rr]) | (((uint32_t)__builtin_popcount(aV_[rr]) + dV_[rr]) << 16);\
+          } else {            \
+            _Pragma("unroll") for (int rr = 0; rr < R; rr++)                                                                      \
+              pk_[rr] = (uint32_t)bcnt_acc(u4c(P.E[rr], J) & cur.v[0], 0) | ((uint32_t)bcnt_acc(u4c(P.V[rr], J) & cur.v[1], 0) << 16);\
           }                                                                                                                       \
           const uint32_t off_ = cur.v[2];                                                                                         \
           __builtin_amdgcn_sched_barrier(0);                                                                                      \
@@ -440,7 +450,196 @@
 #undef RARE_ITEM
       }
     }
+    } else {
+      constexpr uint32_t RING_B = 512u;
+      __shared__ __attribute__((aligned(16))) uint32_t ring_mem[NW][RING_B / 4];
+      typedef __attribute__((address_space(3))) uint32_t lds_u32;
+      typedef __attribute__((address_space(3))) const u32x4_ld lds_entry;
+      scan3_lds_char *rb = (scan3_lds_char *)&ring_mem[wave][0];
+      const uint32_t dg0 = dir[2 * wave], n_rec = dir[2 * wave + 1], dr0 = dir[2 * NW + 2 * wave], n_rare = dir[2 * NW + 2 * wave + 1];
+      asm volatile("" ::"s"(dg0), "s"(n_rec), "s"(dr0), "s"(n_rare));
+      uint32_t first = 0u, refill_at = 0u, stage = 0u, pos = 0u;
+      auto ring_start = [&](uint32_t share) {
+        first = share; pos = 0u; refill_at = 64u;
+        const uint32_t *g = stream + share;
+        const uint32_t c0 = g[lane], c1 = g[64 + lane];
+        stage = g[128 + lane];
+        *(lds_u32 *)(rb + lane * 4) = c0; *(lds_u32 *)(rb + 256 + lane * 4) = c1;
+      };
+      auto ring_refill = [&](uint32_t p) {
+        if (p >= refill_at) {
+          *(lds_u32 *)(rb + (((refill_at - 64u) & 64u) + (uint32_t)lane) * 4u) = stage;
+          stage = (stream + (first + refill_at + 128u))[lane];
+          refill_at += 64u;
+        }
+      };
+      auto ring_read = [&](uint32_t p) -> u32x4_ld { return *(lds_entry *)(rb + ((p * 4u) & (RING_B - 1u))); };
+      auto sgpr = [](uint32_t v) -> uint32_t { return (uint32_t)__builtin_amdgcn_readfirstlane((int)v); };
+      auto header_ahead = [&](uint32_t off) -> uint32_t { return (stream + off)[lane & 3]; };
+      auto lane_of = [](uint32_t v, int l) -> uint32_t { return (uint32_t)__builtin_amdgcn_readlane((int)v, l); };
+
+      ring_start(dg0);
+      uint32_t vh = header_ahead(dg0);
+      uint32_t h0 = lane_of(vh, 0), off_n = dg0 + lane_of(vh, 3);
+      vh = header_ahead(off_n);
+      uint32_t h0_n = lane_of(vh, 0), len_n = lane_of(vh, 3);
+      request(PA, h0);
+      u32x4_ld hd = ring_read(0u);
+#define ITEM_VALUE_R(P, mI, mV, dst)                                                                                \
+      {                                                                                                             \
+        uint32_t pk_[R];                                                                                            \
+        _Pragma("unroll") for (int rr = 0; rr < R; rr++) {                                                          \
+          int e_ = 0, v_ = 0;                                                                                       \
+          _Pragma("unroll") for (int j = 0; j < 4; j++) e_ = bcnt_acc(u4c(P.E[rr], j) & mI[j], e_);                 \
+          _Pragma("unroll") for (int j = 0; j < 4; j++) v_ = bcnt_acc(u4c(P.V[rr], j) & mV[j], v_);                 \
+          pk_[rr] = (uint32_t)e_ | ((uint32_t)v_ << 16);                                                            \
+        }                                                                                                           \
+        dst = pack_acc(pk_);                                                                                        \
+      }
+#define WORD_ITEM_R(P, J, cur)                                                                                                    \
+        {                                                                                                                         \
+          __builtin_amdgcn_sched_barrier(0);                                                                                      \
+          uint32_t pk_[R];                                                                                                        \
+          _Pragma("unroll") for (int rr = 0; rr < R; rr++)                                                                        \
+            pk_[rr] = SCAN3_RUN_SUM(u4c(P.E[rr], J) & cur.x, wE[rr], cur.w)                              \
+                      | (SCAN3_RUN_SUM(u4c(P.V[rr], J) & cur.y, wV[rr], cur.w) << 16);                   \
+          const uint32_t off_ = cur.z;                                                                                            \
+          __builtin_amdgcn_sched_barrier(0);                                                                                      \
+          LDS_ADD(off_, pack_acc(pk_));                                                                                           \
+        }
+#define WORD_ITEMS_R(P, J)                                                                                                        \
+        {                                                                                                                         \
+          uint32_t k = (n_words >> (8 * J)) & 255u;                                                                               \
+          _Pragma("unroll 1") for (; k >= 2; k -= 2) {                                                                            \
+            ring_refill(pos + 4u);                                                                                                \
+            nx = ring_read(pos + 4u);                                                                                             \
+            WORD_ITEM_R(P, J, it)                                                                                                 \
+            pos += 8u;                                                                                                            \
+            it = ring_read(pos);                                                                                                  \
+            WORD_ITEM_R(P, J, nx)                                                                                                 \
+          }                                                                                                                       \
+          if (k) {                                                                                                                \
+            pos += 4u;                                                                                                            \
+            ring_refill(pos);                                                                                                     \
+            nx = ring_read(pos);                                                                                                  \
+            WORD_ITEM_R(P, J, it)                                                                                                 \
+            it = nx;                                                                                                              \
+          }                                                                                                                       \
+        }
+#define RECORD_R(P, Pn)                                                                                                           \
+      {                                                                                                                           \
+        const uint32_t c1_ = sgpr(hd.y), n_words = sgpr(hd.z);                                                                    \
+        const uint32_t n_full4 = c1_ & 0xFFFFu, n_gen = c1_ >> 16;                                                                \
+        const uint32_t off_nn = off_n + len_n;                                                                                    \
+        vh = header_ahead(off_nn);                                                                                                \
+        request(Pn, h0_n);                                                                                                        \
+        pos += 4u;                                                                                                                \
+        ring_refill(pos);                                                                                                         \
+        u32x4_ld it = ring_read(pos), nx;                                                                                         \
+        if (n_full4) {                    \
+          const acc_t gg = pack_acc(P.g);                                                                                         \
+          _Pragma("unroll 1") for (uint32_t k = 0; k < n_full4; k++) {                                                            \
+            pos += 4u;                                                                                                            \
+            ring_refill(pos);                                                                                                     \
+            nx = ring_read(pos);                                                                                                  \
+            LDS_ADD(it.x, gg); LDS_ADD(it.y, gg); LDS_ADD(it.z, gg); LDS_ADD(it.w, gg);                                           \
+            it = nx;                                                                                                              \
+          }                                                                                                                       \
+        }                                                                                                                         \
+        if (n_gen) {                           \
+          _Pragma("unroll 1") for (uint32_t k = 0; k < n_gen; k++) {                                                              \
+            ring_refill(pos + 4u);                                                                                                \
+            const u32x4_ld mv_ = ring_read(pos + 4u), of_ = ring_read(pos + 8u);                                                  \
+            pos += 12u;                                                                                                           \
+            nx = ring_read(pos);                                                                                                  \
+            const uint32_t mI_[4] = {it.x, it.y, it.z, it.w}, mV_[4] = {mv_.x, mv_.y, mv_.z, mv_.w};                              \
+            acc_t va_;                                                                                                            \
+            ITEM_VALUE_R(P, mI_, mV_, va_);                                                                                       \
+            LDS_ADD(of_.x, va_);                                                                                                  \
+            it = nx;                                                                                                              \
+          }                                                                                                                       \
+        }                                                                                                                         \
+        if (n_words) {                                                                                                            \
+          uint32_t wE[R], wV[R];       \
+          _Pragma("unroll") for (int rr = 0; rr < R; rr++) { wE[rr] = 0u; wV[rr] = 0u; }                                          \
+          if (h0 & 1u) {                                                                                                          \
+            _Pragma("unroll") for (int rr = 0; rr < R; rr++) {                                                                    \
+              wE[rr] = (uint32_t)bcnt_acc(P.E[rr].x, 0) | (uint32_t)bcnt_acc(P.E[rr].y, 0) << 8 | (uint32_t)bcnt_acc(P.E[rr].z, 0) << 16 | (uint32_t)bcnt_acc(P.E[rr].w, 0) << 24; \
+              wV[rr] = (uint32_t)bcnt_acc(P.V[rr].x, 0) | (uint32_t)bcnt_acc(P.V[rr].y, 0) << 8 | (uint32_t)bcnt_acc(P.V[rr].z, 0) << 16 | (uint32_t)bcnt_acc(P.V[rr].w, 0) << 24; \
+            }                                                                                                                     \
+          }                                                                                                                       \
+          WORD_ITEMS_R(P, 0) WORD_ITEMS_R(P, 1) WORD_ITEMS_R(P, 2) WORD_ITEMS_R(P, 3)                                             \
+        }                                                                                                                         \
+        hd = it;                                                                                                                  \
+        h0 = h0_n; off_n = off_nn; h0_n = lane_of(vh, 0); len_n = lane_of(vh, 3);                                                 \
+      }
+      for (uint32_t rec = 0; rec < n_rec; rec += 2) {
+        RECORD_R(PA, PB)
+        if (rec + 1 < n_rec) RECORD_R(PB, PA)
+      }
+#undef RECORD_R
+#undef WORD_ITEMS_R
+#undef WORD_ITEM_R
+#undef ITEM_VALUE_R
+      if (n_rare) {
+        const char *tr[R];
+#pragma unroll
+        for (int rr = 0; rr < R; rr++) tr[rr] = reinterpret_cast<const char *>(poly + (size_t)(tile_first + trel[rr]) * NPT * 3 * 64 + lane);
+        ring_start(dr0);
+        u32x4_ld it = ring_read(0u), nx;
+        for (uint32_t rec = 0; rec < n_rare; rec++) {
+          const uint32_t hoff = sgpr(it.x), n_words = sgpr(it.y);
+          uint4 pL[R], pH[R], pI[R];
+#pragma unroll
+          for (int rr = 0; rr < R; rr++) {
+            pL[rr] = *reinterpret_cast<const uint4 *>(tr[rr] + hoff); pH[rr] = *reinterpret_cast<const uint4 *>(tr[rr] + hoff + 1024);
+            pI[rr] = *reinterpret_cast<const uint4 *>(tr[rr] + hoff + 2048);
+          }
+          pos += 4u;
+          ring_refill(pos);
+          it = ring_read(pos);
+#define RARE_ITEM_R(J, cur)                                                                                                       \
+          {                                                                                                                       \
+            __builtin_amdgcn_sched_barrier(0);                                                                                    \
+            uint32_t c_[R];                                                                                                       \
+            _Pragma("unroll") for (int rr = 0; rr < R; rr++) {                                                                    \
+              const uint32_t d_ = u4c(pL[rr], J) ^ cur.y;                                                                         \
+              const uint32_t y_ = B3(u4c(pH[rr], J), cur.z, d_, (TT_A ^ TT_B) | TT_C);                                            \
+              const uint32_t g_ = ACGT ? B3(y_, u4c(pI[rr], J), cur.x, TT_A & TT_B & TT_C) : B3(y_, u4c(pI[rr], J), cur.x, ~TT_A & TT_B & TT_C); \
+              c_[rr] = (uint32_t)bcnt_acc(g_, 0);                                                                                 \
+            }                                                                                                                     \
+            const uint32_t off_ = cur.w;                                                                                          \
+            __builtin_amdgcn_sched_barrier(0);                                                                                    \
+            LDS_SUB(off_, pack_acc(c_));                           \
+          }
+#define RARE_ITEMS_R(J)                                                                                                           \
+          {                                                                                                                       \
+            uint32_t k = (n_words >> (8 * J)) & 255u;                                                                             \
+            _Pragma("unroll 1") for (; k >= 2; k -= 2) {                                                                          \
+              ring_refill(pos + 4u);                                                                                              \
+              nx = ring_read(pos + 4u);                                                                                           \
+              RARE_ITEM_R(J, it)                                                                                                  \
+              pos += 8u;                                                                                                          \
+              it = ring_read(pos);                                                                                                \
+              RARE_ITEM_R(J, nx)                                                                                                  \
+            }                                                                                                                     \
+            if (k) {                                                                                                              \
+              pos += 4u;                                                                                                          \
+              ring_refill(pos);                                                                                                   \
+              nx = ring_read(pos);                                                                                                \
+              RARE_ITEM_R(J, it)                                                                                                  \
+              it = nx;                                                                                                            \
+            }                                                                                                                     \
+          }
+          RARE_ITEMS_R(0) RARE_ITEMS_R(1) RARE_ITEMS_R(2) RARE_ITEMS_R(3)
+#undef RARE_ITEMS_R
+#undef RARE_ITEM_R
+        }
+      }
+    }
 #undef LDS_ADD
+#undef SCAN3_RUN_SUM
+#undef SCAN3_RUN_DOT
 #undef LDS_SUB
 #undef TOUCH_ITEM
 #undef TOUCH4
diff --git a/uvaia_amd/csrc/uvaia_gpu.hip b/uvaia_amd/csrc/uvaia_gpu.hip
--- a/uvaia_amd/csrc/uvaia_gpu.hip
+++ b/uvaia_amd/csrc/uvaia_gpu.hip
@@ -49,6 +49,7 @@
 constexpr int AMB_ROW = 64;
 constexpr int PACK_CHUNK = 4096;
 constexpr uint32_t SCAN3_BIAS = 16384u;
+constexpr size_t SCAN3_STREAM_PAD = 512;
 constexpr int SCAN_STRIPE_TILES = 64;
 constexpr int NBUF = 4;
 
@@ -134,6 +135,7 @@
   hipStream_t rep_stream = nullptr; hipEvent_t rep_ev[2] = {};
   int scan_R = 2;
   int scan_NW = 8;
+  bool scan_ring = false;
   int *d_amb_q = nullptr;
   struct { const void *p; size_t n; } qtab[10] = {};
   unsigned long long *d_stats = nullptr;
```

New measurement: 33.19 million (median of 3 runs). Within noise of the previous version (+0.0%).
